# weibohuang0314/pixel_aware_gyro_aided_klt_feature_tracker

Hardware: AMD Instinct MI355X
Metric: tracked features/sec (21x21, 3-lvl, 30 iter) (higher is better)
Workload: dtype f32 sampling, f64 normal equations; 1 GPU; cfg1_euroc_752x480: 752x480 pair, 1000 keypoints (1000/GPU), gyro-predicted affine init, h=10, L=3, I=30 (synthetic stand-in for BASELINE configs[1]); mode=shard-weak, features_total=1000, features_active=1000, step_mode=graph

## Files before the change

### include/pagk.h

```cpp
#ifndef PAGK_H
#define PAGK_H

#include <stddef.h>
#include <stdint.h>

#ifdef __cplusplus
extern "C" {
#endif

#define PAGK_VERSION 303

#define PAGK_MAX_PYRAMIDS 8
#define PAGK_MAX_HALF_PATCH 15

enum {
    PAGK_OK = 0,
    PAGK_E_ARG = -1,
    PAGK_E_HIP = -2,
    PAGK_E_NOMEM = -3,
    PAGK_E_UNSUPPORTED = -4,
    PAGK_E_NODEVICE = -5,
    PAGK_E_NCCL = -6,
    PAGK_E_CAPACITY = -7
};
// ... 10 lines not shown
    int32_t iterations;
    int32_t pyramids;
    uint8_t has_gyro_predict_initial;
    uint8_t inverse;
    uint8_t consider_illumination;
    uint8_t consider_affine;
    uint8_t regularization_penalty;
    uint8_t calculate_ncc;
    uint8_t predict_method;
    uint8_t solver_variant;
    float lambda;
    float alpha;
    int32_t max_distance;
    float inv_log_max_dist;
    float fx, fy, cx, cy;
    float dist_coef[5];
    int32_t n_dist_coef;
} pagk_params;

typedef struct pagk_outputs {
    float *pt_un;
    float *pt_dist;
    uint8_t *status;
    double *pix_err;
    double *dist_pred;
    float *ncc;
    int32_t *iters;
} pagk_outputs;

typedef struct pagk_ctx pagk_ctx;

int pagk_version(void);
const char *pagk_strerror(int code);
const char *pagk_last_error(const pagk_ctx *ctx);

void pagk_params_default(pagk_params *p);
float pagk_inv_log_max_dist(float alpha, int32_t max_distance);

int pagk_create(pagk_ctx **out, int device);
void pagk_destroy(pagk_ctx *ctx);

int pagk_track(pagk_ctx *ctx, const pagk_params *params, const pagk_image *ref,
               const pagk_image *cur, int32_t n, const float *pt_ref_un,
               const float *pt_init_un, const float *affine, const uint8_t *status_in,
               const pagk_outputs *out);

int pagk_track_pyr(pagk_ctx *ctx, const pagk_params *params, int32_t n_levels,
                   const pagk_image *ref_levels, const pagk_image *cur_levels, int32_t n,
                   const float *pt_ref_un, const float *pt_init_un, const float *affine,
                   const uint8_t *status_in, const pagk_outputs *out);

int pagk_frame_upload(pagk_ctx *ctx, int32_t slot, const pagk_image *img, int32_t pyramids);
int pagk_frame_upload_pinned(pagk_ctx *ctx, int32_t slot, const pagk_image *img, int32_t pyramids);
int pagk_frame_set_device(pagk_ctx *ctx, int32_t slot, const void *d_data, int32_t width,
                          int32_t height, int64_t step, int32_t pyramids);
int pagk_frame_set_device_batch(pagk_ctx *const *ctxs, int32_t k, const int32_t *slot, const void *const *d_data,
                                const int32_t *width, const int32_t *height, const int64_t *step, int32_t pyramids);
int pagk_frame_download_level(pagk_ctx *ctx, int32_t slot, int32_t level, uint8_t *dst,
                              int32_t *width, int32_t *height);

int pagk_track_device(pagk_ctx *ctx, const pagk_params *params, int32_t slot_ref,
                      int32_t slot_cur, int32_t n, const float *d_pt_ref_un,
                      const float *d_pt_init_un, const float *d_affine,
                      const uint8_t *d_status_in, const pagk_outputs *d_out);
int pagk_track_device_fused(pagk_ctx *ctx, const pagk_params *params, int32_t slot_ref, int32_t slot_cur, int32_t n,
                            const float *d_pt_ref_un, const float *d_pt_init_un, const float *d_affine,
                            const uint8_t *d_status_in, const pagk_outputs *d_out, int32_t slot_next,
                            const void *d_next, int32_t width, int32_t height, int64_t step, int32_t pyramids);
int pagk_track_device_batch(pagk_ctx *const *ctxs, int32_t k, const pagk_params *params, const int32_t *slot_ref,
                            const int32_t *slot_cur, const int32_t *n, const float *const *d_pt_ref_un,
                            const float *const *d_pt_init_un, const float *const *d_affine,
                            const uint8_t *const *d_status_in, const pagk_outputs *d_out);
int pagk_sync(pagk_ctx *ctx);
int pagk_check_launch(pagk_ctx *ctx);
int pagk_set_stream(pagk_ctx *ctx, void *hip_stream);

int pagk_set_kernel(pagk_ctx *ctx, int32_t which);
int pagk_has_variant(int32_t which);
int pagk_last_variant(const pagk_ctx *ctx);

int pagk_last_handover(pagk_ctx *ctx);

int pagk_priority_threshold(pagk_ctx *ctx);

int pagk_set_concurrency(pagk_ctx *ctx, int32_t streams);

int pagk_last_kernel_ms(pagk_ctx *ctx, float *track_ms, float *pyramid_ms);

int pagk_gyro_predict_device(pagk_ctx *ctx, const pagk_params *params, int32_t width, int32_t height,
                             const float *KRKinv, const float *r3, int32_t n, const float *d_pt_ref_un,
                             float *d_pt_predict_un, float *d_pt_predict, uint8_t *d_status, float *d_affine);
int pagk_gyro_predict_device_rot(pagk_ctx *ctx, const pagk_params *params, int32_t width, int32_t height,
                                 const float *d_rot, int32_t n, const float *d_pt_ref_un, float *d_pt_predict_un,
                                 float *d_pt_predict, uint8_t *d_status, float *d_affine);

int pagk_post_filter(int32_t n, int32_t half_patch, const uint8_t *status_pm,
                     const double *pix_err, const double *dist_pred, const float *pt_pm,
                     const float *pt_pm_un, uint8_t *status_out, float *pt_predict,
                     float *pt_predict_un);
int pagk_post_filter_device(pagk_ctx *ctx, int32_t n, int32_t half_patch, const uint8_t *d_status_pm,
                            const double *d_pix_err, const double *d_dist_pred, const float *d_pt_pm,
                            const float *d_pt_pm_un, uint8_t *d_status_out, float *d_pt_predict,
                            float *d_pt_predict_un, int32_t *d_kept, double *d_thresholds );

int pagk_gyro_predict_device_live(pagk_ctx *ctx, const pagk_params *params, int32_t width, int32_t height,
                                  const float *d_rot, int32_t n, const float *d_pt_ref_un, const uint8_t *d_live,
                                  float *d_pt_predict_un, float *d_pt_predict, uint8_t *d_status, float *d_affine);

#define PAGK_HANDOVER_STATE_WORDS 8
int pagk_frame_handover_device(pagk_ctx *ctx, const pagk_params *params, int32_t width, int32_t height, int32_t cap,
                               int32_t target_n, double new_point_threshold, const uint8_t *d_status,
                               const float *d_pt_predict, const float *d_pt_predict_un, int32_t cand_cap,
                               const int32_t *d_n_cand, const float *d_cand_un, float *d_keys, float *d_keys_un,
                               float *d_keys_normal , int32_t *d_index_in_last, uint8_t *d_live,
                               uint8_t *d_mask , int32_t *d_state);
int pagk_frame_handover(pagk_ctx *ctx, const pagk_params *params, int32_t width, int32_t height, int32_t cap,
                        int32_t target_n, double new_point_threshold, const uint8_t *status, const float *pt_predict,
                        const float *pt_predict_un, int32_t cand_cap, const int32_t *n_cand, const float *cand_un,
                        float *keys, float *keys_un, float *keys_normal, int32_t *index_in_last, uint8_t *live,
                        uint8_t *mask, int32_t *state);

typedef struct pagk_detect_params {
    double quality_level;
    double min_distance;
    double harris_k;
    int32_t raw_cap;
} pagk_detect_params;
#define PAGK_DETECT_INFO_WORDS 8
void pagk_detect_params_default(pagk_detect_params *p);
int pagk_detect_corners_device(pagk_ctx *ctx, const pagk_detect_params *det, int32_t slot, const uint8_t *d_mask,
                               int32_t cap, const int32_t *d_max_corners, float *d_corners, int32_t *d_info);
int pagk_detect_corners(pagk_ctx *ctx, const pagk_detect_params *det, const pagk_image *img, const uint8_t *mask,
                        int32_t max_corners, float *corners, int32_t *info);
int pagk_frame_handover_detect_device(pagk_ctx *ctx, const pagk_params *params, int32_t width, int32_t height,
                                      int32_t cap, int32_t target_n, double new_point_threshold, const uint8_t *d_status,
                                      const float *d_pt_predict, const float *d_pt_predict_un,
                                      const pagk_detect_params *det, int32_t slot, float *d_keys, float *d_keys_un,
                                      float *d_keys_normal , int32_t *d_index_in_last, uint8_t *d_live,
                                      uint8_t *d_mask , int32_t *d_state, int32_t *d_info);
int pagk_frame_handover_detect(pagk_ctx *ctx, const pagk_params *params, int32_t width, int32_t height, int32_t cap,
                               int32_t target_n, double new_point_threshold, const uint8_t *status,
                               const float *pt_predict, const float *pt_predict_un, const pagk_detect_params *det,
                               const pagk_image *img, float *keys, float *keys_un, float *keys_normal,
                               int32_t *index_in_last, uint8_t *live, uint8_t *mask, int32_t *state, int32_t *info);
int pagk_selftest_corner_response(pagk_ctx *ctx, const pagk_image *img, float *R);

typedef struct pagk_fast_params {
    int32_t ini_threshold;
    int32_t min_threshold;
    int32_t n_features;
    int32_t n_levels;
} pagk_fast_params;
void pagk_fast_params_default(pagk_fast_params *p);
int pagk_fast_params_check(const pagk_fast_params *p);
int pagk_detect_fast_bounds(int32_t width, int32_t height, int32_t n_features, int32_t *raw_bound, int32_t *out_bound);
int pagk_detect_fast_device(pagk_ctx *ctx, const pagk_fast_params *params, int32_t slot, const uint8_t *d_mask, int32_t cap,
                            float *d_keypoints, float *d_response , int32_t *d_info);
int pagk_detect_fast(pagk_ctx *ctx, const pagk_fast_params *params, const pagk_image *img, const uint8_t *mask, int32_t cap,
                     float *keypoints, float *response, int32_t *info);
int pagk_frame_handover_fast_device(pagk_ctx *ctx, const pagk_params *params, int32_t width, int32_t height, int32_t cap,
                                    int32_t target_n, double new_point_threshold, const uint8_t *d_status,
                                    const float *d_pt_predict, const float *d_pt_predict_un, const pagk_fast_params *fast,
                                    int32_t slot, float *d_keys, float *d_keys_un, float *d_keys_normal ,
                                    int32_t *d_index_in_last, uint8_t *d_live, uint8_t *d_mask ,
                                    int32_t *d_state, int32_t *d_info);
int pagk_frame_handover_fast(pagk_ctx *ctx, const pagk_params *params, int32_t width, int32_t height, int32_t cap,
// ... 228 lines not shown
```

### pixel_aware_gyro_aided_klt_feature_tracker_amd/capi.py

```python
from __future__ import annotations

import ctypes as C
import os

import numpy as np

PKG_DIR = os.path.dirname(os.path.abspath(__file__))
LIB_PATH = os.environ.get("PAGK_LIB") or os.path.join(PKG_DIR, "libpagk_hip.so")

PAGK_OK = 0
PAGK_E_ARG = -1
PAGK_E_HIP = -2
PAGK_E_NOMEM = -3
PAGK_E_UNSUPPORTED = -4
PAGK_E_NODEVICE = -5
PAGK_E_NCCL = -6
PAGK_E_CAPACITY = -7


class Image(C.Structure):
    _fields_ = [("data", C.c_void_p), ("width", C.c_int32), ("height", C.c_int32), ("step", C.c_int64)]


class Params(C.Structure):
# ... 288 lines not shown
        lib.pagk_lk_params_check.argtypes = [_P(LkParams)]
        lib.pagk_lk_levels.restype = C.c_int
        lib.pagk_lk_levels.argtypes = [i32, i32, _P(LkParams)]
        lib.pagk_lk_pyramid_device.restype = C.c_int
        lib.pagk_lk_pyramid_device.argtypes = [vp, _P(LkParams), i32]
        lib.pagk_lk_track_device.restype = C.c_int
        lib.pagk_lk_track_device.argtypes = [vp, _P(LkParams), i32, i32, i32, vp, vp, vp, vp, vp, vp, vp, vp]
        lib.pagk_lk_track.restype = C.c_int
        lib.pagk_lk_track.argtypes = [vp, _P(LkParams), _P(Image), _P(Image), i32, vp, vp, vp, vp, vp, vp, vp]
        lib.pagk_selftest_lk_level.restype = C.c_int
        lib.pagk_selftest_lk_level.argtypes = [vp, i32, i32, vp, C.c_int64]
    f32 = C.c_float
    for name in ("pagk_graph_begin",):
        getattr(lib, name).restype = C.c_int
        getattr(lib, name).argtypes = [vp]
    lib.pagk_graph_end.restype = C.c_int
    lib.pagk_graph_end.argtypes = [vp, _P(i32)]
    lib.pagk_graph_launch.restype = C.c_int
    lib.pagk_graph_launch.argtypes = [vp, i32]
    lib.pagk_graph_destroy.restype = C.c_int
    lib.pagk_graph_destroy.argtypes = [vp, i32]
    lib.pagk_geometry_scores_device.restype = C.c_int
    lib.pagk_geometry_scores_device.argtypes = [vp, vp, vp, vp, i32, vp, vp, f32, vp, vp, vp]
    lib.pagk_geometry_scores.restype = C.c_int
    lib.pagk_geometry_scores.argtypes = [vp, vp, vp, vp, i32, vp, vp, f32, vp, vp, _P(f32), _P(f32)]
    lib.pagk_geometry_select.restype = C.c_int
    lib.pagk_geometry_select.argtypes = [f32, f32]
    lib.pagk_geometry_validation.restype = C.c_int
    lib.pagk_geometry_validation.argtypes = [vp, vp, vp, vp, i32, vp, vp, vp, f32, _P(f32)]
    if hasattr(lib, "pagk_search_klt_device"):
        ap, lp, f32_ = _P(AssocParams), _P(LkParams), C.c_float
        lib.pagk_assoc_params_default.restype = None
        lib.pagk_assoc_params_default.argtypes = [ap]
        lib.pagk_assoc_params_check.restype = C.c_int
        lib.pagk_assoc_params_check.argtypes = [ap]
        lib.pagk_match_features_device.restype = C.c_int
        lib.pagk_match_features_device.argtypes = [vp, ap, i32, i32, i32] + [vp] * 10
        lib.pagk_search_gyro_predict_device.restype = C.c_int
        lib.pagk_search_gyro_predict_device.argtypes = ([vp, ap, i32, i32, i32, i32, vp, vp, vp, vp, i32, vp, vp, vp, f32_, i32]
                                                        + [vp] * 11)
        lib.pagk_search_gyro_predict.restype = C.c_int
        lib.pagk_search_gyro_predict.argtypes = ([vp, ap, _P(Image), _P(Image), i32, i32, vp, vp, vp, vp, i32, vp, vp, f32_, i32]
                                                 + [vp] * 10)
        lib.pagk_search_klt_device.restype = C.c_int
        lib.pagk_search_klt_device.argtypes = [vp, lp, ap, i32, i32, i32, vp, vp, i32, vp, vp] + [vp] * 11
        lib.pagk_search_klt.restype = C.c_int
        lib.pagk_search_klt.argtypes = [vp, lp, ap, _P(Image), _P(Image), i32, vp, i32, vp] + [vp] * 10
    lib.pagk_fit_params_default.restype = None
    lib.pagk_fit_params_default.argtypes = [_P(FitParams)]
    lib.pagk_geometry_fit_device.restype = C.c_int
    lib.pagk_geometry_fit_device.argtypes = [vp, _P(FitParams), i32, vp, vp, vp, vp, vp, vp, vp, vp]
    lib.pagk_geometry_fit.restype = C.c_int
    lib.pagk_geometry_fit.argtypes = [vp, _P(FitParams), i32, vp, vp, vp, vp, vp, vp, vp, vp]
    lib.pagk_geometry_validation_device.restype = C.c_int
    lib.pagk_geometry_validation_device.argtypes = [vp, _P(FitParams), i32, vp, vp, vp, f32, vp, vp]
    lib.pagk_geometry_validation_fit.restype = C.c_int
    lib.pagk_geometry_validation_fit.argtypes = [vp, _P(FitParams), i32, vp, vp, vp, f32, _P(f32)]
    lib.pagk_selftest_fit_samples.restype = C.c_int
    lib.pagk_selftest_fit_samples.argtypes = [vp, C.c_uint64, i32, i32, i32, i32, vp]
    f64 = C.c_double
    lib.pagk_pose_params_default.restype = None
    lib.pagk_pose_params_default.argtypes = [_P(PoseParams)]
    lib.pagk_pose_params_check.restype = C.c_int
    lib.pagk_pose_params_check.argtypes = [_P(PoseParams)]
    lib.pagk_pose_2d2d_device.restype = C.c_int
    lib.pagk_pose_2d2d_device.argtypes = [vp, _P(PoseParams), f64, f64, f64, i32] + [vp] * 12
    lib.pagk_pose_from_matches_device.restype = C.c_int
    lib.pagk_pose_from_matches_device.argtypes = [vp, _P(PoseParams), f64, f64, f64, i32, vp, vp, i32] + [vp] * 12
    lib.pagk_pose_2d2d.restype = C.c_int
    lib.pagk_pose_2d2d.argtypes = [vp, _P(PoseParams), f64, f64, f64, i32] + [vp] * 12
    lib.pagk_near_neighbors_device.restype = C.c_int
    lib.pagk_near_neighbors_device.argtypes = [vp, i32, i32, i32, i32, vp, vp, vp, vp, i32, vp, vp, i32, f32, i32, i32,
                                               vp, vp, vp, vp]
    lib.pagk_find_near_neighbors.restype = C.c_int
    lib.pagk_find_near_neighbors.argtypes = [vp, _P(Image), _P(Image), i32, i32, vp, vp, vp, vp, i32, vp, vp, i32, f32,
                                             i32, i32, vp, vp, vp, vp]
    lib.pagk_ncc_free.restype = C.c_int
    lib.pagk_ncc_free.argtypes = [vp, _P(Image), _P(Image), i32, i32, vp, vp, vp, vp]
    if hasattr(lib, "pagk_selftest_divide"):
        lib.pagk_selftest_divide.restype = C.c_int
        lib.pagk_selftest_divide.argtypes = [vp, i32, vp, vp, vp, vp, vp, vp]
        lib.pagk_selftest_solve.restype = C.c_int
        lib.pagk_selftest_solve.argtypes = [vp, i32, vp, vp, C.c_uint32, vp, vp, vp, vp]
    if hasattr(lib, "pagk_priority_threshold"):
        lib.pagk_priority_threshold.restype = C.c_int
        lib.pagk_priority_threshold.argtypes = [vp]
    if hasattr(lib, "pagk_check_launch"):
        lib.pagk_check_launch.restype = C.c_int
        lib.pagk_check_launch.argtypes = [vp]
    if hasattr(lib, "pagk_selftest_repeat_sum"):
        lib.pagk_selftest_repeat_sum.restype = C.c_int
        lib.pagk_selftest_repeat_sum.argtypes = [vp, i32, vp, i32, vp, vp]
    if hasattr(lib, "pagk_selftest_sample"):
        lib.pagk_selftest_sample.restype = C.c_int
        lib.pagk_selftest_sample.argtypes = [vp, i32, i32, i32, i32, vp, vp]
    lib.pagk_match_features.restype = C.c_int
    lib.pagk_match_features.argtypes = [i32, i32, vp, vp, vp, vp, i32, vp, vp, vp, vp]
    lib.pagk_multi_create.restype = C.c_int
    lib.pagk_multi_create.argtypes = [_P(vp), _P(i32), i32]
    lib.pagk_multi_unique_id.restype = C.c_int
    lib.pagk_multi_unique_id.argtypes = [vp]
    lib.pagk_multi_create_rank.restype = C.c_int
    lib.pagk_multi_create_rank.argtypes = [_P(vp), vp, i32, i32, i32]
    lib.pagk_multi_destroy.restype = None
    lib.pagk_multi_destroy.argtypes = [vp]
    lib.pagk_multi_world.restype = i32
    lib.pagk_multi_world.argtypes = [vp]
    if hasattr(lib, "pagk_multi_comm_count"):
        lib.pagk_multi_comm_count.restype = i32
        lib.pagk_multi_comm_count.argtypes = [vp]
    lib.pagk_multi_local.restype = i32
    lib.pagk_multi_local.argtypes = [vp]
    lib.pagk_multi_ctx.restype = vp
    lib.pagk_multi_ctx.argtypes = [vp, i32]
    lib.pagk_multi_last_error.restype = C.c_char_p
    lib.pagk_multi_last_error.argtypes = [vp]
    lib.pagk_shard_range.restype = None
    lib.pagk_shard_range.argtypes = [i32, i32, i32, _P(i32), _P(i32)]
    lib.pagk_shard_layout.restype = C.c_size_t
    lib.pagk_shard_layout.argtypes = [i32, _P(C.c_size_t)]
    lib.pagk_multi_allgather.restype = C.c_int
    lib.pagk_multi_allgather.argtypes = [vp, _P(vp), _P(vp), C.c_size_t, _P(vp)]
    lib.pagk_track_sharded.restype = C.c_int
    lib.pagk_track_sharded.argtypes = [vp, _P(Params), _P(Image), _P(Image), i32, vp, vp, vp, vp, _P(Outputs)]


EXPORTED_SYMBOLS = [
    "pagk_version", "pagk_strerror", "pagk_last_error", "pagk_params_default", "pagk_inv_log_max_dist",
    "pagk_create", "pagk_destroy", "pagk_track", "pagk_track_pyr", "pagk_frame_upload", "pagk_frame_upload_pinned",
    "pagk_frame_set_device", "pagk_frame_download_level", "pagk_track_device", "pagk_track_device_fused", "pagk_sync",
    "pagk_set_stream", "pagk_set_kernel", "pagk_last_variant", "pagk_set_concurrency", "pagk_last_handover", "pagk_last_kernel_ms", "pagk_post_filter", "pagk_gyro_predict_device",
    "pagk_gyro_predict_device_rot",
    "pagk_geometry_scores_device", "pagk_geometry_scores", "pagk_geometry_select", "pagk_geometry_validation",
    "pagk_graph_begin", "pagk_graph_end", "pagk_graph_launch", "pagk_graph_destroy",
    "pagk_near_neighbors_device", "pagk_find_near_neighbors", "pagk_ncc_free", "pagk_match_features",
    "pagk_multi_create", "pagk_multi_unique_id", "pagk_multi_create_rank", "pagk_multi_destroy", "pagk_multi_world",
    "pagk_multi_local", "pagk_multi_ctx", "pagk_multi_last_error", "pagk_shard_range", "pagk_shard_layout",
    "pagk_multi_allgather", "pagk_track_sharded", "pagk_selftest_divide", "pagk_selftest_solve",
    "pagk_selftest_repeat_sum", "pagk_check_launch", "pagk_track_device_batch", "pagk_frame_set_device_batch", "pagk_priority_threshold",
    "pagk_multi_comm_count", "pagk_has_variant",
    "pagk_fit_params_default", "pagk_geometry_fit_device", "pagk_geometry_fit", "pagk_geometry_validation_device",
    "pagk_geometry_validation_fit", "pagk_selftest_fit_samples",
    "pagk_pose_params_default", "pagk_pose_params_check", "pagk_pose_2d2d_device", "pagk_pose_from_matches_device",
    "pagk_pose_2d2d",
    "pagk_post_filter_device", "pagk_gyro_predict_device_live", "pagk_frame_handover_device", "pagk_frame_handover",
    "pagk_detect_params_default", "pagk_detect_corners_device", "pagk_detect_corners",
    "pagk_frame_handover_detect_device", "pagk_frame_handover_detect", "pagk_selftest_corner_response",
    "pagk_fast_params_default", "pagk_fast_params_check", "pagk_detect_fast_bounds", "pagk_detect_fast_device",
    "pagk_detect_fast", "pagk_frame_handover_fast_device", "pagk_frame_handover_fast", "pagk_selftest_fast_cells",
    "pagk_rectify_params_default", "pagk_rectify_params_check", "pagk_rectify_set_maps", "pagk_frame_rectify_device",
    "pagk_frame_rectify_pinned", "pagk_rectify", "pagk_undistort_maps",
    "pagk_orb_params_default", "pagk_orb_params_check", "pagk_orb_pattern_check", "pagk_orb_set_pattern",
    "pagk_orb_describe_device", "pagk_orb_describe", "pagk_orb_match_device", "pagk_orb_match",
    "pagk_selftest_sample",
    "pagk_lk_params_default", "pagk_lk_params_check", "pagk_lk_levels", "pagk_lk_pyramid_device", "pagk_lk_track_device",
    "pagk_lk_track", "pagk_selftest_lk_level",
    "pagk_assoc_params_default", "pagk_assoc_params_check", "pagk_match_features_device", "pagk_search_gyro_predict_device",
    "pagk_search_gyro_predict", "pagk_search_klt_device", "pagk_search_klt",
]

HANDOVER_STATE_WORDS = 8
HANDOVER_STATE_FIELDS = ("total", "reach_flag", "survivors", "added", "rejected")


def fit_params_default(**overrides) -> FitParams:
    p = FitParams()
    load().pagk_fit_params_default(C.byref(p))
    for k, v in overrides.items():
        if k not in dict(FitParams._fields_):
            raise TypeError(f"pagk_fit_params has no field {k}")
        setattr(p, k, v)
    return p


def pose_params_default(**overrides) -> PoseParams:
    p = PoseParams()
    load().pagk_pose_params_default(C.byref(p))
    for k, v in overrides.items():
        if k not in dict(PoseParams._fields_):
            raise TypeError(f"pagk_pose_params has no field {k}")
        setattr(p, k, v)
    return p


def pose_params_check(p: PoseParams) -> int:
    return load().pagk_pose_params_check(C.byref(p))


def detect_params_default(**overrides) -> DetectParams:
    p = DetectParams()
    load().pagk_detect_params_default(C.byref(p))
    for k, v in overrides.items():
        if k not in dict(DetectParams._fields_):
            raise TypeError(f"pagk_detect_params has no field {k}")
        setattr(p, k, v)
    return p


def fast_params_default(**overrides) -> FastParams:
    p = FastParams()
    load().pagk_fast_params_default(C.byref(p))
    for k, v in overrides.items():
        if k not in dict(FastParams._fields_):
            raise TypeError(f"pagk_fast_params has no field {k}")
        setattr(p, k, v)
    return p


def fast_params_check(p: FastParams) -> int:
    return int(load().pagk_fast_params_check(C.byref(p)))


def detect_fast_bounds(width: int, height: int, n_features: int):
    raw, out = C.c_int32(0), C.c_int32(0)
    rc = load().pagk_detect_fast_bounds(int(width), int(height), int(n_features), C.byref(raw), C.byref(out))
    if rc != 0:
        raise PagkError(rc, "pagk_detect_fast_bounds")
    return raw.value, out.value


def orb_params_default(**overrides) -> OrbParams:
    p = OrbParams()
    load().pagk_orb_params_default(C.byref(p))
# ... 787 lines not shown
        info = np.zeros(ASSOC_INFO_WORDS, np.int32)
        ru = float(2 * half_patch) if radius_unit is None else float(radius_unit)
        rc = self.lib.pagk_search_gyro_predict(self.h, C.byref(ap), C.byref(ir), C.byref(ic), half_patch, n, _ptr(keys_ref),
                                               _ptr(pt_predict_un), _ptr(status), _ptr(affine), m, _ptr(keys_cur),
                                               _ptr(keys_cur_un), ru, cap, _ptr(count), _ptr(idx), _ptr(dist), _ptr(ncc),
                                               _ptr(q), _ptr(t), _ptr(md), _ptr(mc), _ptr(flows), _ptr(info))
        if rc < 0 and rc != PAGK_E_CAPACITY:
            self._check(rc, "pagk_search_gyro_predict")
        k = int(info[4])
        out = dict(rc=rc, n_matches=k, query=q[:k], train=t[:k], dist=md[:k], ncc=mc[:k], flows_err=flows[:n], count=count[:n],
                   idx=idx[:n], dist_lists=dist[:n], ncc_lists=ncc[:n], info=info)
        out.update(zip(ASSOC_MATCH_INFO_FIELDS, (int(v) for v in info[:6])))
        return out

    def search_klt_device(self, lk: LkParams, ap: AssocParams, slot_ref: int, slot_cur: int, cap: int, d_keys_ref, d_n, m: int,
                          d_keys_cur, d_m, d_pt_out, d_status, d_err, d_match_query, d_match_train, d_match_dist, d_disparity,
                          d_n_matches, d_stats, d_info, d_lk_info):
        self._check(self.lib.pagk_search_klt_device(
            self.h, C.byref(lk), C.byref(ap), slot_ref, slot_cur, cap, _ptr(d_keys_ref), _ptr(d_n), m, _ptr(d_keys_cur), _ptr(d_m),
            _ptr(d_pt_out), _ptr(d_status), _ptr(d_err), _ptr(d_match_query), _ptr(d_match_train), _ptr(d_match_dist),
            _ptr(d_disparity), _ptr(d_n_matches), _ptr(d_stats), _ptr(d_info), _ptr(d_lk_info)), "pagk_search_klt_device")

    def search_klt(self, img_ref, img_cur, keys_ref, keys_cur, lk: LkParams | None = None, ap: AssocParams | None = None) -> dict:
        lk = lk if lk is not None else lk_params_default()
        ap = ap if ap is not None else assoc_params_default()
        kr = np.ascontiguousarray(keys_ref, np.float32).reshape(-1, 2)
        kc = np.ascontiguousarray(keys_cur, np.float32).reshape(-1, 2)
        n, m = int(kr.shape[0]), int(kc.shape[0])
        nn = max(n, 1)
        ir, ic = image_view(img_ref), image_view(img_cur)
        pt_out, status, err = np.zeros((nn, 2), np.float32), np.zeros(nn, np.uint8), np.zeros(nn, np.float32)
        q, t = np.full(nn, -1, np.int32), np.full(nn, -1, np.int32)
        md, disp = np.zeros(nn, np.float32), np.zeros(nn, np.float64)
        stats = np.zeros(ASSOC_STATS_WORDS, np.float64)
        info, lk_info = np.zeros(ASSOC_INFO_WORDS, np.int32), np.zeros(LK_INFO_WORDS, np.int32)
        k = self.lib.pagk_search_klt(self.h, C.byref(lk), C.byref(ap), C.byref(ir), C.byref(ic), n, _ptr(kr) if n else None, m,
                                     _ptr(kc) if m else None, _ptr(pt_out), _ptr(status), _ptr(err), _ptr(q), _ptr(t), _ptr(md),
                                     _ptr(disp), _ptr(stats), _ptr(info), _ptr(lk_info))
        self._check(min(k, 0), "pagk_search_klt")
        out = dict(n_matches=k, query=q[:k], train=t[:k], dist=md[:k], disparity=disp[:k], pt_out=pt_out[:n], status=status[:n],
                   err=err[:n], stats=stats, info=info, lk_info=lk_info)
        out.update(zip(ASSOC_KLT_INFO_FIELDS, (int(v) for v in info)))
        out.update(zip(ASSOC_STATS_FIELDS, (float(v) for v in stats[:7])))
        return out

    def graph_begin(self):
        self._check(self.lib.pagk_graph_begin(self.h), "pagk_graph_begin")

    def graph_end(self) -> int:
        gid = C.c_int32(-1)
        self._check(self.lib.pagk_graph_end(self.h, C.byref(gid)), "pagk_graph_end")
        return gid.value

    def graph_launch(self, graph_id: int):
        self._check(self.lib.pagk_graph_launch(self.h, graph_id), "pagk_graph_launch")

    def graph_destroy(self, graph_id: int):
        self._check(self.lib.pagk_graph_destroy(self.h, graph_id), "pagk_graph_destroy")

    def sync(self):
        self._check(self.lib.pagk_sync(self.h), "pagk_sync")

    def check_launch(self):
        self._check(self.lib.pagk_check_launch(self.h), "pagk_check_launch")

    def set_stream(self, stream_ptr: int | None):
        self._check(self.lib.pagk_set_stream(self.h, stream_ptr), "pagk_set_stream")

    def set_kernel(self, which: int):
        self._check(self.lib.pagk_set_kernel(self.h, which), "pagk_set_kernel")

    VARIANT_NAMES = {0: "4-wave workgroup per feature, DPP row chains", 1: "one thread per feature (cross-check)",
                     2: "2-wave workgroup per feature, f64 MFMA chain", 3: "one wave per feature, f64 MFMA chain",
                     4: "relaxed order (experiment)", 5: "four features per wave, f64 MFMA blocks",
                     6: "four independent rows per wave + work queue",
                     7: "four features per wave, one pyramid level per wave"}

    def priority_threshold(self) -> int:
        rc = int(self.lib.pagk_priority_threshold(self.h))
        if rc < 0:
            self._check(rc, "pagk_priority_threshold")
        return rc

    def last_variant(self) -> int:
        return int(self.lib.pagk_last_variant(self.h))

    def last_handover(self) -> int:
        rc = int(self.lib.pagk_last_handover(self.h))
        if rc < 0:
            self._check(rc, "pagk_last_handover")
        return rc

    def set_concurrency(self, streams: int):
        self._check(self.lib.pagk_set_concurrency(self.h, streams), "pagk_set_concurrency")

    def last_kernel_ms(self):
        t, p = C.c_float(0), C.c_float(0)
        self._check(self.lib.pagk_last_kernel_ms(self.h, C.byref(t), C.byref(p)), "pagk_last_kernel_ms")
        return t.value, p.value


def post_filter(half_patch: int, status_pm, pix_err, dist_pred, pt_pm, pt_pm_un):
    lib = load()
    n = int(status_pm.shape[0])
    status = np.zeros(max(n, 1), np.uint8)
    pp = np.zeros((max(n, 1), 2), np.float32)
    ppu = np.zeros((max(n, 1), 2), np.float32)
    rc = lib.pagk_post_filter(n, half_patch, _ptr(status_pm), _ptr(pix_err), _ptr(dist_pred), _ptr(pt_pm),
                              _ptr(pt_pm_un), _ptr(status), _ptr(pp), _ptr(ppu))
    if rc < 0:
        raise PagkError(rc, "pagk_post_filter")
    return rc, status[:n], pp[:n], ppu[:n]


def geometry_select(score_H: float, score_F: float) -> bool:
    return bool(load().pagk_geometry_select(float(score_H), float(score_F)))


def match_features(count, idx, dist, ncc, use_ncc=True):
    n = int(count.shape[0])
    cap = int(idx.shape[1])
    q, t = np.zeros(max(n, 1), np.int32), np.zeros(max(n, 1), np.int32)
    d, c = np.zeros(max(n, 1), np.float32), np.zeros(max(n, 1), np.float32)
    count = np.ascontiguousarray(count, np.int32)
    idx, dist, ncc = np.ascontiguousarray(idx), np.ascontiguousarray(dist), np.ascontiguousarray(ncc)
    k = load().pagk_match_features(n, cap, _ptr(count), _ptr(idx), _ptr(dist), _ptr(ncc), int(use_ncc), _ptr(q), _ptr(t),
                                   _ptr(d), _ptr(c))
    if k < 0:
        raise PagkError(k, "pagk_match_features")
    return q[:k], t[:k], d[:k], c[:k]


def shard_range(n: int, rank: int, world: int) -> tuple[int, int]:
    lo, hi = C.c_int32(0), C.c_int32(0)
    load().pagk_shard_range(n, rank, world, C.byref(lo), C.byref(hi))
    return lo.value, hi.value


def shard_layout(m: int) -> tuple[list[int], int]:
    offs = (C.c_size_t * 7)()
    total = load().pagk_shard_layout(m, offs)
    return [int(v) for v in offs], int(total)


class Multi:

    def __init__(self, devices=None, *, uid: bytes | None = None, rank: int = 0, world: int = 1, device: int = 0):
        self.lib = load()
        self._lent = []
        h = C.c_void_p()
        if uid is None:
            if devices is None or len(devices) == 0 or any(int(d) < 0 for d in devices):
                raise ValueError("Multi(devices=[...]) needs a non-empty list of device indices (or uid=, rank=, world=)")
            devs = (C.c_int32 * len(devices))(*devices)
            rc = self.lib.pagk_multi_create(C.byref(h), devs, len(devices))
            where = "pagk_multi_create"
        else:
            if len(uid) != 128:
                raise ValueError("the RCCL unique id is 128 bytes")
            buf = (C.c_uint8 * 128).from_buffer_copy(uid)
            rc = self.lib.pagk_multi_create_rank(C.byref(h), buf, rank, world, device)
            where = "pagk_multi_create_rank"
        if rc != PAGK_OK:
            raise PagkError(rc, where)
        self.h = h
        self.world = self.lib.pagk_multi_world(h)
# ... 60 lines not shown
```

### pixel_aware_gyro_aided_klt_feature_tracker_amd/csrc/pagk_device.h

```cpp
#pragma once
#include <hip/hip_runtime.h>
#include <stdint.h>

namespace pagk {

constexpr int kMaxLevels = 8;

struct DevLevel {
    const uint32_t *quad;
    int cols, rows;
    float fcols, frows;
    float fcols_m1, frows_m1;
};

__device__ __forceinline__ int ld_agent(const int *p) { return __hip_atomic_load(p, __ATOMIC_RELAXED, __HIP_MEMORY_SCOPE_AGENT); }
__device__ __forceinline__ void st_agent(int *p, int v) { __hip_atomic_store(p, v, __ATOMIC_RELAXED, __HIP_MEMORY_SCOPE_AGENT); }

struct SuspState {
    int level;
    int iter;
    float dx, dy, dg, db, lastCost;
    int iters;
};

struct BatchStream {
    DevLevel l1[kMaxLevels], l2[kMaxLevels];
    const float *pt_ref, *pt_init, *affine;
    const uint8_t *status_in;
    float *pt_un, *pt_dist;
    uint8_t *status;
    double *pix_err, *dist_pred;
    float *ncc;
    int *iters;
    int n;
    int quad_base;
};

struct TrackArgs {
    DevLevel l1[kMaxLevels], l2[kMaxLevels];
    float scales[kMaxLevels];
    int n_levels;
    int n;
    const float *pt_ref;
    const float *pt_init;
    const float *affine;
    const uint8_t *status_in;
    float *pt_un;
    float *pt_dist;
    uint8_t *status;
    double *pix_err;
    double *dist_pred;
    float *ncc;
    int *iters;
    unsigned long long *dbg;
    float *ws;
    int iter_budget;
    int *susp_count;
    int *susp_list;
    SuspState *susp_state;
    int susp_lone;
    int susp_waves;
    int susp_polls;
    int *queue;
    int *lv_ready;
    float *lv_state;
    int *lv_error;
    int lv_shift;
    int lv_polls;
    const BatchStream *batch;
    int batch_k;
    int half, iterations;
    int prio_k;
    unsigned long long *prio_stats;
    const int *prio_kbuf;
    int has_gyro, illum, use_affine, penalty, calc_ncc;
    uint32_t solver;
    float lam_invlog;
    float lam_invlog_alpha;
    float alpha;
    double win_size_inv;
    int distort_on;
    float fx, fy, cx, cy, fx_inv, fy_inv, k1, k2, p1, p2, k3;
};

__device__ __forceinline__ DevLevel pin_level(const DevLevel &src) { return src; }

struct Coord {
    int i;
    float f;
    float omf;
};

template <bool CLAMP>
__device__ __forceinline__ Coord prep_coord(float x, float fmax, float fmax_m1)
{
    if (CLAMP) {
        x = fmaxf(x, 0.0f);
        x = (x >= fmax) ? fmax_m1 : x;
    }
    Coord c;
    c.i = (int)x;
    c.f = __builtin_amdgcn_fractf(x);
    c.omf = 1.0f - c.f;
    return c;
}

__device__ __forceinline__ float bilerp(uint32_t q, const Coord &cx, const Coord &cy)
{
    float d0 = (float)(q & 0xffu);
    float d1 = (float)((q >> 8) & 0xffu);
    float d2 = (float)((q >> 16) & 0xffu);
    float d3 = (float)(q >> 24);
    float top = cx.omf * d0 + cx.f * d1;
    float bot = cx.omf * d2 + cx.f * d3;
    return cy.omf * top + cy.f * bot;
}

#if !defined(PAGK_CLASSIC_SAMPLER)
#ifndef PAGK_PK_BILERP
#define PAGK_PK_BILERP
#endif
#ifndef PAGK_TYPED_TAPS
#define PAGK_TYPED_TAPS
#endif
#endif
typedef float pagk_f32x4 __attribute__((ext_vector_type(4)));
typedef float pagk_f32x2 __attribute__((ext_vector_type(2)));
typedef int pagk_i32x4 __attribute__((ext_vector_type(4)));

#ifdef PAGK_TYPED_TAPS
__device__ pagk_f32x4 pagk_buffer_load_format_xyzw(pagk_i32x4 rsrc, int vindex, int voffset, int soffset, int aux)
    __asm("llvm.amdgcn.struct.buffer.load.format.v4f32");

struct TapSrc {
    pagk_i32x4 rs;
};
__device__ __forceinline__ TapSrc tap_src(const DevLevel &L)
{
    const uint64_t base = (uint64_t)(uintptr_t)L.quad;
    TapSrc t;
    t.rs.x = (int)(uint32_t)base;
    t.rs.y = (int)((uint32_t)(base >> 32) & 0xffffu) | (4 << 16);
    t.rs.z = L.cols * L.rows;
    t.rs.w = 4 | (6 << 3) | (5 << 6) | (7 << 9) | (2 << 12) | (10 << 15);
    return t;
}
typedef pagk_f32x4 Taps;
__device__ __forceinline__ Taps load_taps(const TapSrc &t, int idx) { return pagk_buffer_load_format_xyzw(t.rs, idx, 0, 0, 0); }
__device__ __forceinline__ pagk_f32x4 taps_f32(Taps q) { return q; }
#else
struct TapSrc {
    const uint32_t *quad;
};
__device__ __forceinline__ TapSrc tap_src(const DevLevel &L) { return TapSrc{L.quad}; }
typedef uint32_t Taps;
__device__ __forceinline__ Taps load_taps(const TapSrc &t, int idx) { return t.quad[(uint32_t)idx]; }
__device__ __forceinline__ pagk_f32x4 taps_f32(Taps q)
// ... 607 lines not shown
```

### pixel_aware_gyro_aided_klt_feature_tracker_amd/csrc/pagk_handover_kernel.h

```cpp
#pragma once

#include <hip/hip_runtime.h>
#include <stdint.h>

namespace pagk {

constexpr int kHandoverStateWords = 8;
constexpr int kHandoverHalf = 7;

constexpr int kPfRound = 2048;

__device__ __forceinline__ double pf_chain256(double s, const double2 *b)
{
    double2 A[8], B[8];
#pragma unroll
    for (int j = 0; j < 8; j++) A[j] = b[j];
    for (int k = 0; k < 128; k += 16) {
#pragma unroll
        for (int j = 0; j < 8; j++) B[j] = b[k + 8 + j];
        __builtin_amdgcn_sched_barrier(0);
#pragma unroll
        for (int j = 0; j < 8; j++) {
            s = s + A[j].x;
            s = s + A[j].y;
// ... 10 lines not shown
        __builtin_amdgcn_sched_barrier(0);
    }
    return s;
}

__global__ void __launch_bounds__(1024) k_post_filter(int32_t n, int32_t half_patch, const uint8_t *status_pm,
                                                      const double *pix_err, const double *dist_pred, const float *pt_pm,
                                                      const float *pt_pm_un, uint8_t *status_out, float *pt_predict,
                                                      float *pt_predict_un, int32_t *kept_out, double *thresholds)
{
    __shared__ double s_sum;
    __shared__ __align__(16) double s_stage[2][kPfRound];
    __shared__ int32_t s_cnt[16], s_kept[16];
    const int tid = threadIdx.x, lane = tid & 63, wave = tid >> 6;
    int32_t cnt = 0;
    double s = 0.0;
    auto load = [&](int i, int32_t &c) -> double {
        if (i >= n) return 0.0;
        const double v = pix_err[i];
        const bool on = status_pm[i] != 0;
        c += on ? 1 : 0;
        return on ? v : 0.0;
    };
    double v0 = load(tid, cnt), v1 = load(1024 + tid, cnt);
    s_stage[0][tid] = v0, s_stage[0][1024 + tid] = v1;
    __syncthreads();
    for (int r0 = 0, g = 0; r0 < n; r0 += kPfRound, g ^= 1) {
        v0 = load(r0 + kPfRound + tid, cnt), v1 = load(r0 + kPfRound + 1024 + tid, cnt);
        if (wave == 0) {
            const int left = n - r0;
            const int groups = left >= kPfRound ? kPfRound / 256 : (left + 255) / 256;
            for (int q = 0; q < groups; q++) s = pf_chain256(s, reinterpret_cast<const double2 *>(&s_stage[g][q * 256]));
        }
        s_stage[g ^ 1][tid] = v0, s_stage[g ^ 1][1024 + tid] = v1;
        __syncthreads();
    }
    if (tid == 0) s_sum = s;
    for (int off = 32; off >= 1; off >>= 1) cnt += __shfl_down(cnt, off, 64);
    if (lane == 0) s_cnt[wave] = cnt;
    __syncthreads();
    int32_t total = 0;
    for (int w = 0; w < 16; w++) total += s_cnt[w];
    const double avg = s_sum / (double)total;
    const double th_pix = 4.0 * avg > (double)half_patch ? 4.0 * avg : (double)half_patch;
    const double th_dist = (double)half_patch * 4.0;
    int32_t kept = 0;
    for (int c0 = 0; c0 < n; c0 += 1024) {
        const int i = c0 + tid;
        if (i < n) {
            const bool ok = status_pm[i] && pix_err[i] < th_pix && dist_pred[i] < th_dist;
            status_out[i] = ok ? 1 : 0;
            if (ok) {
                if (pt_predict && pt_pm) pt_predict[2 * i] = pt_pm[2 * i], pt_predict[2 * i + 1] = pt_pm[2 * i + 1];
                if (pt_predict_un && pt_pm_un)
                    pt_predict_un[2 * i] = pt_pm_un[2 * i], pt_predict_un[2 * i + 1] = pt_pm_un[2 * i + 1];
                kept++;
            }
        }
    }
    for (int off = 32; off >= 1; off >>= 1) kept += __shfl_down(kept, off, 64);
    if (lane == 0) s_kept[wave] = kept;
    __syncthreads();
    if (tid == 0) {
        int32_t k = 0;
        for (int w = 0; w < 16; w++) k += s_kept[w];
        *kept_out = k;
        if (thresholds) thresholds[0] = th_pix, thresholds[1] = th_dist;
    }
}

struct HandoverArgs {
    int32_t cap, cand_cap, width, height, target_n;
    double new_point_threshold;
    float fx, fy, cx, cy, fx_inv, fy_inv, k1, k2, p1, p2, k3;
    int32_t distort_on;
    const uint8_t *status;
    const float *pt_predict, *pt_predict_un;
    const int32_t *n_cand;
    const float *cand_un;
    float *keys, *keys_un, *keys_normal;
    int32_t *index_in_last;
    uint8_t *live, *mask;
    int32_t *state;
};

__global__ void __launch_bounds__(256) k_handover_fill(uint8_t *mask, int64_t bytes)
{
    const int64_t t = (int64_t)blockIdx.x * 256 + threadIdx.x, o = t * 16;
    if (o + 16 <= bytes) {
        if ((reinterpret_cast<uintptr_t>(mask) & 15) == 0) {
            *reinterpret_cast<uint4 *>(mask + o) = make_uint4(0x01010101u, 0x01010101u, 0x01010101u, 0x01010101u);
        } else {
            for (int k = 0; k < 16; k++) mask[o + k] = 1;
        }
    } else {
        for (int64_t k = o; k < bytes; k++) mask[k] = 1;
    }
}

__device__ __forceinline__ int handover_hole_origin(float x, int extent)
{
    const int a = (int)x - kHandoverHalf;
    const int b = a > 0 ? a : 0;
    const int hi = extent - 2 * kHandoverHalf;
    return b < hi ? b : hi;
}

__global__ void __launch_bounds__(256) k_handover_holes(int32_t cap, int32_t width, int32_t height, const uint8_t *status,
                                                        const float *pt_predict_un, uint8_t *mask)
{
    const int t = blockIdx.x * 256 + threadIdx.x;
    const int i = t / (2 * kHandoverHalf), r = t - i * (2 * kHandoverHalf);
    if (i >= cap || !status[i]) return;
    const int x0 = handover_hole_origin(pt_predict_un[2 * i], width);
    const int y0 = handover_hole_origin(pt_predict_un[2 * i + 1], height);
    uint8_t *row = mask + (int64_t)(y0 + r) * width + x0;
    for (int k = 0; k < 2 * kHandoverHalf; k++) row[k] = 0;
}

__device__ __forceinline__ int32_t handover_scan(bool take, int32_t *wtot, int lane, int wave, int32_t &tot)
{
    const unsigned long long bal = __ballot(take);
    if (lane == 0) wtot[wave] = __popcll(bal);
    __syncthreads();
    int32_t off = 0;
    tot = 0;
    for (int w = 0; w < 16; w++) {
        off += w < wave ? wtot[w] : 0;
        tot += wtot[w];
    }
    __syncthreads();
    return off + __popcll(bal & ((1ull << lane) - 1ull));
}

__device__ __forceinline__ bool handover_accepts(const HandoverArgs &a, float x, float y)
{
    if (!(x > -1.0f && x < (float)a.width && y > -1.0f && y < (float)a.height)) return false;
    return a.mask[(int64_t)(int)y * a.width + (int)x] != 0;
}

__global__ void __launch_bounds__(1024) k_handover_keys(HandoverArgs a)
{
    __shared__ int32_t wtot[16];
    const int tid = threadIdx.x, lane = tid & 63, wave = tid >> 6;
    int32_t m = 0;
    for (int c0 = 0; c0 < a.cap; c0 += 1024) {
        const int i = c0 + tid;
        const bool take = i < a.cap && a.status[i] != 0;
        int32_t tot;
        const int32_t o = m + handover_scan(take, wtot, lane, wave, tot);
        if (take) {
            const float xu = a.pt_predict_un[2 * i], yu = a.pt_predict_un[2 * i + 1];
            a.keys[2 * o] = a.pt_predict[2 * i], a.keys[2 * o + 1] = a.pt_predict[2 * i + 1];
            a.keys_un[2 * o] = xu, a.keys_un[2 * o + 1] = yu;
            if (a.keys_normal) a.keys_normal[2 * o] = (xu - a.cx) * a.fx_inv, a.keys_normal[2 * o + 1] = (yu - a.cy) * a.fy_inv;
            a.index_in_last[o] = i;
        }
        m += tot;
    }
    const int32_t reach = a.state[1];
    int32_t n_cand = *a.n_cand;
    n_cand = n_cand < 0 ? 0 : (n_cand > a.cand_cap ? a.cand_cap : n_cand);
    __syncthreads();
    const int32_t n_new = a.target_n - m;
    const bool topup = ((double)m < a.new_point_threshold || !reach) && n_new > 0;
    int32_t seen = 0;
    for (int c0 = 0; c0 < n_cand; c0 += 1024) {
        const int j = c0 + tid;
        float x = 0.0f, y = 0.0f;
        if (j < n_cand) x = a.cand_un[2 * j], y = a.cand_un[2 * j + 1];
        const bool ok = j < n_cand && handover_accepts(a, x, y);
        int32_t tot;
        const int32_t r = seen + handover_scan(ok, wtot, lane, wave, tot);
        if (topup && ok && r < n_new) {
            const int32_t q = m + r;
            a.keys_un[2 * q] = x, a.keys_un[2 * q + 1] = y;
            const float xn = (x - a.cx) * a.fx_inv, yn = (y - a.cy) * a.fy_inv;
            if (a.keys_normal) a.keys_normal[2 * q] = xn, a.keys_normal[2 * q + 1] = yn;
            float ox = x, oy = y;
            if (a.distort_on) {
                const float r2 = xn * xn + yn * yn;
                const float r4 = r2 * r2;
                const float r6 = r4 * r2;
                const float xd = xn * (1 + a.k1 * r2 + a.k2 * r4 + a.k3 * r6) + 2 * a.p1 * xn * yn + a.p2 * (r2 + 2 * xn * xn);
                const float yd = yn * (1 + a.k1 * r2 + a.k2 * r4 + a.k3 * r6) + a.p1 * (r2 + 2 * yn * yn) + 2 * a.p2 * xn * yn;
                ox = a.fx * xd + a.cx;
                oy = a.fy * yd + a.cy;
            }
            a.keys[2 * q] = ox, a.keys[2 * q + 1] = oy;
            a.index_in_last[q] = -1;
        }
        seen += tot;
    }
    const int32_t added = topup ? (seen < n_new ? seen : n_new) : 0;
    const int32_t total = m + added;
    for (int i = tid; i < a.cap; i += 1024) {
        a.live[i] = i < total ? 1 : 0;
        if (i >= total) {
            a.keys[2 * i] = a.keys[2 * i + 1] = 0.0f;
            a.keys_un[2 * i] = a.keys_un[2 * i + 1] = 0.0f;
            if (a.keys_normal) a.keys_normal[2 * i] = a.keys_normal[2 * i + 1] = 0.0f;
            a.index_in_last[i] = -1;
        }
    }
    if (tid == 0) {
        a.state[0] = total;
        a.state[1] = topup ? (total == a.target_n ? 1 : 0) : reach;
        a.state[2] = m;
        a.state[3] = added;
        a.state[4] = n_cand - seen;
        a.state[5] = a.state[6] = a.state[7] = 0;
    }
}

}
```

### pixel_aware_gyro_aided_klt_feature_tracker_amd/csrc/pagk_hip.hip

```cpp
#include <hip/hip_runtime.h>

#include <algorithm>
#include <array>
#include <cmath>
#include <cstdio>
#include <cstdlib>
#include <cstring>
#include <new>
#include <utility>
#include <vector>

#include "../../include/pagk.h"
#include "pagk_kernels.h"
#include "pagk_associate_kernel.h"
#include "pagk_pose_kernel.h"
#include "pagk_layout.h"
#include "pagk_select.h"

using namespace pagk;

namespace {

constexpr int kSlots = 6;
constexpr int kUserSlots = 4;

struct DevBuf {
    void *ptr = nullptr;
    size_t bytes = 0;
    void *host = nullptr;
    bool mirrored = false;
};

struct FrameSlot {
    int w = 0, h = 0, L = 0;
    int wrap0 = 1;
    int pad0 = 0;
    uint8_t *u8[kMaxLevels] = {};
    uint32_t *quad[kMaxLevels] = {};
    const uint8_t *img0 = nullptr;
    int64_t pitch0 = 0;
    DevBuf block;
    bool valid = false;
};

}

struct pagk_ctx {
    int device = 0;
    hipStream_t own_stream = nullptr;
    hipStream_t stream = nullptr;
    FrameSlot slots[kSlots];
    enum Buf {
        FEAT,
        SCORE,
        FIT,
        FITIO,
        HAND,
        HANDIO,
        DET,
        FAST,
        RECT_ENTRIES,
        RECT_STAGE,
        ORB_PATTERN,
        ORB_BLUR,
        ORB_KEYS,
        LK_PYR,
        LK_PYR_LAST = LK_PYR + kSlots - 1,
        ASSOC,
        POSE,
        POSEIO,
        QUAD_WS,
        SUSP,
        LV,
        kBufs
    };
    DevBuf buf[kBufs];
    int fit_n = 0, fit_iters = 0;
    int pose_n = 0, pose_iters = 0;
    int rect_w = 0, rect_h = 0, rect_wp = 0;
    bool orb_pattern_set = false;
    struct LkPyr { int w = 0, h = 0, top = -1; } lk_pyr[kSlots];
    void *queue = nullptr;
    int quad_capacity[PAGK_MAX_HALF_PATCH + 1] = {};
    int rows_capacity[PAGK_MAX_HALF_PATCH + 1] = {};
    int rows_waves_cap = 0;
    int *susp_count_dev = nullptr;
    struct BatchDesc {
        void *host = nullptr, *dev = nullptr;
        hipEvent_t used = nullptr;
        bool recorded = false;
    };
    static constexpr int kBatchRing = 6, kBatchPerCapture = 4, kBatchMaxStreams = 64;
    BatchDesc batch_ring[kBatchRing];
    int batch_turn = 0;
    bool batch_seen = false;
    std::vector<BatchDesc> cap_batch;
    int cap_batch_used = 0;
    hipEvent_t ev_batch = nullptr;
    int *lv_error = nullptr;
    int *lv_error_dev = nullptr;
    hipStream_t aux_stream = nullptr;
    hipEvent_t ev_fork = nullptr, ev_join = nullptr;
    int susp_lone = 1;
    int finisher_wgs = 16;
    int finisher_polls = 20000;
    int level_polls = 300000;
    int quad_budget = -1;
    int cus = 0;
    bool capturing = false;
    static constexpr int kGraphs = 8;
    hipGraph_t graphs[kGraphs] = {};
    hipGraphExec_t graph_execs[kGraphs] = {};
    struct GraphSeg {
        enum Kind { GRAPH, FINISHER, JOIN } kind = GRAPH;
        hipGraph_t g = nullptr;
        hipGraphExec_t ex = nullptr;
        const void *fn = nullptr;
        TrackArgs args;
        int grid = 0;
        size_t lds = 0;
    };
    std::vector<GraphSeg> pre_segs[kGraphs];
    std::vector<BatchDesc> graph_batch[kGraphs];
    std::vector<GraphSeg> cap_segs;
    hipEvent_t ev_trk[2] = {}, ev_pyr[2] = {};
    bool trk_timed = false, pyr_timed = false;
    int kernel = 0;
    bool last_handover = false;
    int concurrency = 1;
    int last_variant = -1;
    int mfma_min_features = 0x7fffffff;
    int wave_min_features = 6000;
    int quad_min_features = 7000;
    int block5_min_features = 2500;
    int prio_k = 4;
    unsigned long long *prio_stats = nullptr;
    bool block5_window = true;
    int levels_min_features = 6000;
    int levels_shift = 0;
    bool levels_shared = false;
    bool unfused_pyramid = false;
    char err[256] = {0};
};

namespace {

#define HIPCHK(ctx, call)                                                                              \
    do {                                                                                               \
        hipError_t e_ = (call);                                                                        \
        if (e_ != hipSuccess) {                                                                        \
            snprintf((ctx)->err, sizeof((ctx)->err), "%s:%d %s -> %s", __FILE__, __LINE__, #call,     \
                     hipGetErrorString(e_));                                                           \
            return e_ == hipErrorOutOfMemory ? PAGK_E_NOMEM : PAGK_E_HIP;                              \
        }                                                                                              \
    } while (0)

#define NOT_WHILE_CAPTURING(ctx, what)                                                                 \
    do {                                                                                               \
        if ((ctx)->capturing) {                                                                        \
            snprintf((ctx)->err, sizeof((ctx)->err), "%s is not capturable: use the *_device entry points between pagk_graph_begin and pagk_graph_end", what); \
            return PAGK_E_ARG;                                                                         \
        }                                                                                              \
    } while (0)

int level_dims(int w, int h, int L, int *lw, int *lh)
{
    lw[0] = w;
    lh[0] = h;
    for (int l = 1; l < L; l++) {
        lw[l] = (int)(lw[l - 1] * 0.5);
        lh[l] = (int)(lh[l - 1] * 0.5);
        if (lw[l] < 1 || lh[l] < 1) return PAGK_E_ARG;
    }
    return PAGK_OK;
}

bool in_capture(pagk_ctx *ctx)
{
    if (ctx->capturing) return true;
    hipStreamCaptureStatus st = hipStreamCaptureStatusNone;
    return hipStreamIsCapturing(ctx->stream, &st) != hipSuccess || st != hipStreamCaptureStatusNone;
}

int no_live_graphs(pagk_ctx *ctx, const char *what, const char *hint)
{
    for (int k = 0; k < pagk_ctx::kGraphs; k++)
        if (ctx->graph_execs[k]) {
            snprintf(ctx->err, sizeof(ctx->err), "%s would have to grow while graph %d of this context is alive (its nodes hold the old "
                     "pointers): destroy the graph first, or %s", what, k, hint);
            return PAGK_E_ARG;
        }
    return PAGK_OK;
}

enum GrowPolicy {
    GROW_FREELY = 0,
    NOT_IN_CAPTURE = 1,
    NOT_UNDER_GRAPH = 2,
    NOT_IN_CAPTURE_NOR_UNDER_GRAPH = NOT_IN_CAPTURE | NOT_UNDER_GRAPH,
};

int release(pagk_ctx *ctx, DevBuf &b)
{
    if (b.ptr) HIPCHK(ctx, hipFree(b.ptr));
    if (b.host) HIPCHK(ctx, hipHostFree(b.host));
    b.ptr = b.host = nullptr;
    b.bytes = 0;
    return PAGK_OK;
}

int reserve(pagk_ctx *ctx, DevBuf &b, size_t bytes, GrowPolicy policy, const char *what, const char *hint = "")
{
    if (bytes <= b.bytes) return PAGK_OK;
    if ((policy & NOT_IN_CAPTURE) && in_capture(ctx)) {
        snprintf(ctx->err, sizeof(ctx->err), "%s would have to grow inside a graph capture: %s", what, hint);
        return PAGK_E_ARG;
    }
    int rc = (policy & NOT_UNDER_GRAPH) ? no_live_graphs(ctx, what, hint) : PAGK_OK;
    if (rc || (rc = release(ctx, b))) return rc;
// ... 479 lines not shown
            a.susp_list = reinterpret_cast<int *>(lb + lvl.susp_list);
            a.susp_state = reinterpret_cast<SuspState *>(lb + lvl.susp_state);
        } else {
            const size_t sizes[3] = {kSuspCountBytes, (size_t)n * 4, (size_t)n * sizeof(SuspState)};
            const Layout<3> lay(sizes);
            DevBuf &susp = ctx->buf[pagk_ctx::SUSP];
            if (int gr = reserve(ctx, susp, lay.total, NOT_IN_CAPTURE_NOR_UNDER_GRAPH, "the continuation buffers",
                                 kLargestLaunchFirst)) return gr;
            a.susp_count = lay.at<int>(susp.ptr, 0);
            a.susp_list = lay.at<int>(susp.ptr, 1);
            a.susp_state = lay.at<SuspState>(susp.ptr, 2);
        }
        a.iter_budget = budget;
        a.susp_waves = nq;
        a.susp_lone = ctx->susp_lone;
        ctx->susp_count_dev = a.susp_count;
    }
    if (use_levels)
        HIPCHK(ctx, hipMemsetAsync(lb, 0, handover ? lvl.susp_list + (size_t)n * 4 : lvl.susp_count, ctx->stream));
    else if (handover)
        HIPCHK(ctx, hipMemsetAsync(a.susp_count, 0, kSuspCountBytes + (size_t)n * 4, ctx->stream));
    const bool live = handover && live_ok && ctx->finisher_wgs > 0 && ctx->aux_stream;
    const bool segmented = live && ctx->capturing && !getenv("PAGK_GRAPH_BRANCH");
    int fin_seg = -1;
    if (segmented) {
        if (int sr = capture_split(ctx)) return sr;
        ctx->cap_segs.emplace_back();
        ctx->cap_segs.back().kind = pagk_ctx::GraphSeg::FINISHER;
        fin_seg = (int)ctx->cap_segs.size() - 1;
    } else if (live) {
        HIPCHK(ctx, hipEventRecord(ctx->ev_fork, ctx->stream));
        HIPCHK(ctx, hipStreamWaitEvent(ctx->aux_stream, ctx->ev_fork, 0));
    }
    HIPCHK(ctx, launch(use_levels ? k.levels[lean] : k.quad[lean], waves, 64, 0, ctx->stream, a));
    TrackArgs af = a;
#ifdef PAGK_STAMPS
    if (af.dbg) af.dbg += (size_t)16 * (waves - nq);
#endif
    const size_t lds = track_block_lds_bytes(a.half);
    if (live) {
        if (segmented) {
            pagk_ctx::GraphSeg &fs = ctx->cap_segs[(size_t)fin_seg];
            fs.fn = reinterpret_cast<const void *>(k.resume_live[lean]);
            fs.args = af;
            fs.grid = ctx->finisher_wgs;
            fs.lds = lds;
            if (int sr = capture_split(ctx)) return sr;
            ctx->cap_segs.emplace_back();
            ctx->cap_segs.back().kind = pagk_ctx::GraphSeg::JOIN;
        } else {
            HIPCHK(ctx, launch(k.resume_live[lean], ctx->finisher_wgs, kBlock, lds, ctx->aux_stream, af));
            HIPCHK(ctx, hipEventRecord(ctx->ev_join, ctx->aux_stream));
            HIPCHK(ctx, hipStreamWaitEvent(ctx->stream, ctx->ev_join, 0));
        }
    }
    if (handover) HIPCHK(ctx, launch(k.resume[lean], live ? 64 : (n < 1024 ? n : 1024), kBlock, lds, ctx->stream, af));
    return PAGK_OK;
}

int launch_block(pagk_ctx *ctx, const TrackKernels &k, bool lean, int n, const TrackArgs &a, const PyrArgs *pyr,
                 int pyr_blocks, bool *pyr_done)
{
    const size_t lds = track_block_lds_bytes(a.half);
    if (pyr && pyr_blocks > 0 && k.block_pyr[lean] && lds <= 48 * 1024) {
        hipLaunchKernelGGL(k.block_pyr[lean], dim3(n + pyr_blocks), dim3(kBlock), lds, ctx->stream, a, *pyr);
        HIPCHK(ctx, hipGetLastError());
        if (pyr_done) *pyr_done = true;
        return PAGK_OK;
    }
    const bool five = lean && k.block5 && select_block5(n, ctx->block5_min_features, ctx->block5_window, ctx->cus);
    const TrackFn kern = five ? k.block5 : k.block[lean];
    if (lds > 48 * 1024) {
        static thread_local bool configured[PAGK_MAX_HALF_PATCH + 1][2][16] = {};
        bool &done = configured[a.half][lean][ctx->device & 15];
        if (!done) {
            HIPCHK(ctx, hipFuncSetAttribute(reinterpret_cast<const void *>(kern), hipFuncAttributeMaxDynamicSharedMemorySize, (int)lds));
            done = true;
        }
    }
    HIPCHK(ctx, launch(kern, n, kBlock, lds, ctx->stream, a));
    return PAGK_OK;
}

int launch_track(pagk_ctx *ctx, const pagk_params *p, const FrameSlot &sr, const FrameSlot &sc, int n,
                 const float *d_pt_ref, const float *d_pt_init, const float *d_affine, const uint8_t *d_status,
                 const pagk_outputs *o, const PyrArgs *pyr = nullptr, int pyr_blocks = 0, bool *pyr_done = nullptr)
{
    if (pyr_done) *pyr_done = false;
    TrackArgs a;
    memset(&a, 0, sizeof a);
    a.n_levels = p->pyramids;
    for (int l = 0; l < p->pyramids; l++) {
        fill_level(a.l1[l], sr, l);
        fill_level(a.l2[l], sc, l);
        a.scales[l] = l == 0 ? 1.0f : (float)((double)a.scales[l - 1] * 0.5);
    }
    a.n = n;
    a.pt_ref = d_pt_ref;
    a.pt_init = d_pt_init;
    a.affine = d_affine;
    a.status_in = d_status;
    a.pt_un = o->pt_un;
    a.pt_dist = o->pt_dist;
    a.status = o->status;
    a.pix_err = o->pix_err;
    a.dist_pred = o->dist_pred;
    a.ncc = o->ncc;
    a.iters = o->iters;
#if defined(PAGK_STAMPS) || defined(PAGK_COUNT_REDO) || defined(PAGK_TIC)
    a.dbg = reinterpret_cast<unsigned long long *>(getenv("PAGK_DBG_PTR") ? strtoull(getenv("PAGK_DBG_PTR"), nullptr, 0) : 0ull);
#endif
    fill_param_args(a, p);
    a.prio_k = ctx->prio_k;
    a.prio_stats = ctx->prio_stats;
    a.prio_kbuf = ctx->prio_stats ? reinterpret_cast<const int *>(ctx->prio_stats + 2) : nullptr;
    a.lv_error = ctx->lv_error_dev;

    if (ctx->ev_trk[0] && !in_capture(ctx)) HIPCHK(ctx, hipEventRecord(ctx->ev_trk[0], ctx->stream));
    if (n > 0) {
        ctx->last_handover = false;
        const bool lean = !a.penalty && a.solver == 0;
        const TrackKernels &k = track_kernels_of(a.half);
        const int variant = ctx->last_variant = select_variant(select_in(ctx, p, n));
        int rc = PAGK_OK;
        hipError_t e = hipSuccess;
        switch (variant) {
            case 1: e = launch(k_track_thread, (n + 63) / 64, 64, 0, ctx->stream, a); break;
            case 2: e = launch(k.mfma[lean], n, 128, track_mfma_lds_bytes(a.half), ctx->stream, a); break;
            case 3: e = launch(k.wave[lean], n, 64, track_wave_lds_bytes(a.half), ctx->stream, a); break;
            case 4: e = launch(k.relaxed, n, kBlock, track_block_lds_bytes(a.half), ctx->stream, a); break;
            case 5:
            case 7: rc = launch_quad(ctx, p, k, lean, variant == 7, n, a); break;
            case 6: rc = launch_rows(ctx, k, n, a); break;
            default: rc = launch_block(ctx, k, lean, n, a, pyr, pyr_blocks, pyr_done); break;
        }
        if (rc) return rc;
        HIPCHK(ctx, e);
        HIPCHK(ctx, hipGetLastError());
    }
    if (ctx->ev_trk[1] && !in_capture(ctx)) HIPCHK(ctx, hipEventRecord(ctx->ev_trk[1], ctx->stream));
    if (!in_capture(ctx)) ctx->trk_timed = true;
    return PAGK_OK;
}

struct FeatPtrs {
    float *pt_ref, *pt_init, *affine;
    uint8_t *status_in;
    pagk_outputs out;
    Layout<11> lay;
    size_t in_bytes;
};

int feat_reserve(pagk_ctx *ctx, int n, FeatPtrs *fp)
{
    int cap = n < 1 ? 1 : n;
    size_t sizes[11] = {8, 8, 16, 1, 8, 8, 1, 8, 8, 4, 4};
    for (size_t &sz : sizes) sz *= (size_t)cap;
    const Layout<11> lay(sizes);
    int rc = reserve(ctx, ctx->buf[pagk_ctx::FEAT], lay.total, GROW_FREELY, "the feature arrays");
    if (rc) return rc;
    void *b = ctx->buf[pagk_ctx::FEAT].ptr;
    fp->lay = lay;
    fp->in_bytes = lay.off[4];
    fp->pt_ref = lay.at<float>(b, 0);
    fp->pt_init = lay.at<float>(b, 1);
    fp->affine = lay.at<float>(b, 2);
    fp->status_in = lay.at<uint8_t>(b, 3);
    fp->out = {lay.at<float>(b, 4), lay.at<float>(b, 5), lay.at<uint8_t>(b, 6), lay.at<double>(b, 7),
               lay.at<double>(b, 8), lay.at<float>(b, 9), lay.at<int32_t>(b, 10)};
    return PAGK_OK;
}

int upload_level0(pagk_ctx *ctx, FrameSlot &s, const pagk_image *img)
{
    HIPCHK(ctx, hipMemcpy2DAsync(s.u8[0], (size_t)s.w, img->data, (size_t)img->step, (size_t)s.w, (size_t)s.h,
                                 hipMemcpyHostToDevice, ctx->stream));
    return PAGK_OK;
}

int check_image(const pagk_image *im)
{
    if (!im || !im->data || im->width < 1 || im->height < 1 || im->step < im->width) return PAGK_E_ARG;
    if (im->width >= (1 << 24) || im->height >= (1 << 24) || (int64_t)im->width * im->height >= (1ll << 31)) return PAGK_E_ARG;
    return PAGK_OK;
}

int track_host_common(pagk_ctx *ctx, const pagk_params *p, int n, const float *pt_ref, const float *pt_init,
                      const float *affine, const uint8_t *status_in, const pagk_outputs *out, FrameSlot &sr,
                      FrameSlot &sc)
{
    if (n < 0 || !out || !out->pt_un || !out->status) return PAGK_E_ARG;
    if (n > 0 && (!pt_ref || !status_in)) return PAGK_E_ARG;
    if (n > 0 && p->has_gyro_predict_initial && !pt_init) return PAGK_E_ARG;
    if (n > 0 && p->consider_affine && !affine) return PAGK_E_ARG;
    FeatPtrs fp;
    int rc = feat_reserve(ctx, n, &fp);
    if (rc) return rc;
    const size_t *offs = fp.lay.off;
    uint8_t *hb = static_cast<uint8_t *>(ctx->buf[pagk_ctx::FEAT].host), *db = static_cast<uint8_t *>(ctx->buf[pagk_ctx::FEAT].ptr);
    if (n > 0) {
        size_t nn = (size_t)n;
        memcpy(hb + offs[0], pt_ref, nn * 8);
        if (pt_init) memcpy(hb + offs[1], pt_init, nn * 8);
        if (affine) memcpy(hb + offs[2], affine, nn * 16);
        memcpy(hb + offs[3], status_in, nn);
        HIPCHK(ctx, hipMemcpyAsync(db, hb, fp.in_bytes, hipMemcpyHostToDevice, ctx->stream));
    }
    pagk_outputs dout = fp.out;
    if (!out->pt_dist) dout.pt_dist = nullptr;
    if (!out->pix_err) dout.pix_err = nullptr;
    if (!out->dist_pred) dout.dist_pred = nullptr;
    if (!out->ncc) dout.ncc = nullptr;
    if (!out->iters) dout.iters = nullptr;
    rc = launch_track(ctx, p, sr, sc, n, fp.pt_ref, pt_init ? fp.pt_init : nullptr, affine ? fp.affine : nullptr,
                      fp.status_in, &dout);
    if (rc) return rc;
    if (n > 0)
        HIPCHK(ctx, hipMemcpyAsync(hb + fp.in_bytes, db + fp.in_bytes, fp.lay.total - fp.in_bytes, hipMemcpyDeviceToHost,
                                   ctx->stream));
    HIPCHK(ctx, hipStreamSynchronize(ctx->stream));
    if (int lr = lv_check(ctx)) return lr;
    if (n > 0) {
        size_t nn = (size_t)n;
        memcpy(out->pt_un, hb + offs[4], nn * 8);
        if (out->pt_dist) memcpy(out->pt_dist, hb + offs[5], nn * 8);
        memcpy(out->status, hb + offs[6], nn);
        if (out->pix_err) memcpy(out->pix_err, hb + offs[7], nn * 8);
        if (out->dist_pred) memcpy(out->dist_pred, hb + offs[8], nn * 8);
        if (out->ncc) memcpy(out->ncc, hb + offs[9], nn * 4);
        if (out->iters) memcpy(out->iters, hb + offs[10], nn * 4);
    }
    return PAGK_OK;
}

}

extern "C" {

int pagk_version(void) { return PAGK_VERSION; }

const char *pagk_strerror(int code)
{
    switch (code) {
        case PAGK_OK: return "ok";
        case PAGK_E_ARG: return "invalid argument";
        case PAGK_E_HIP: return "HIP runtime error";
        case PAGK_E_NOMEM: return "out of memory";
        case PAGK_E_UNSUPPORTED: return "unsupported mode";
        case PAGK_E_NODEVICE: return "no HIP device";
        case PAGK_E_NCCL: return "RCCL error";
        case PAGK_E_CAPACITY: return "output capacity too small";
        default: return "unknown error";
    }
}

const char *pagk_last_error(const pagk_ctx *ctx) { return ctx ? ctx->err : ""; }

void pagk_params_default(pagk_params *p)
{
    if (!p) return;
    memset(p, 0, sizeof *p);
    p->half_patch = 5;
    p->iterations = 10;
    p->pyramids = 3;
    p->has_gyro_predict_initial = 1;
    p->inverse = 0;
    p->consider_illumination = 1;
    p->consider_affine = 1;
    p->regularization_penalty = 0;
    p->calculate_ncc = 0;
    p->lambda = 1.0f;
    p->alpha = 0.5f;
    p->max_distance = 25;
    p->inv_log_max_dist = 0.0f;
    p->fx = p->fy = 1.0f;
    p->n_dist_coef = 4;
}

float pagk_inv_log_max_dist(float alpha, int32_t max_distance)
{
    float arg = alpha * (float)max_distance + 1;
    float lg = std::log(arg);
    return (float)(1.0 / (double)lg);
}

int pagk_create(pagk_ctx **out, int device)
{
    if (!out) return PAGK_E_ARG;
    *out = nullptr;
    int ndev = 0;
    if (hipGetDeviceCount(&ndev) != hipSuccess || ndev <= 0) return PAGK_E_NODEVICE;
    if (device < 0 || device >= ndev) return PAGK_E_ARG;
    pagk_ctx *ctx = new (std::nothrow) pagk_ctx();
    if (!ctx) return PAGK_E_NOMEM;
    ctx->device = device;
    if (hipSetDevice(device) != hipSuccess || hipStreamCreateWithFlags(&ctx->own_stream, hipStreamNonBlocking) != hipSuccess) {
        delete ctx;
        return PAGK_E_HIP;
    }
    ctx->stream = ctx->own_stream;
    ctx->buf[pagk_ctx::FEAT].mirrored = true;
    if (hipDeviceGetAttribute(&ctx->cus, hipDeviceAttributeMultiprocessorCount, device) != hipSuccess) ctx->cus = 0;
    if (hipMalloc(&ctx->queue, 256) != hipSuccess) {
        pagk_destroy(ctx);
        return PAGK_E_NOMEM;
    }
    {
        void *hp = nullptr;
        void *dp = nullptr;
        if (hipHostMalloc(&hp, 64, hipHostMallocMapped) == hipSuccess) {
            memset(hp, 0, 64);
            if (hipHostGetDevicePointer(&dp, hp, 0) == hipSuccess && dp) {
                ctx->lv_error = static_cast<int *>(hp);
                ctx->lv_error_dev = static_cast<int *>(dp);
            } else {
                (void)hipHostFree(hp);
            }
        }
    }
    if (ctx->cus > 0 && ctx->cus != 256) {
        auto scaled = [&](int v) { return v >= 0x7fffffff / 2 ? v : (int)((long long)v * ctx->cus / 256); };
        ctx->wave_min_features = scaled(ctx->wave_min_features);
        ctx->quad_min_features = scaled(ctx->quad_min_features);
        ctx->levels_min_features = scaled(ctx->levels_min_features);
        ctx->block5_min_features = scaled(ctx->block5_min_features);
    }
    ctx->unfused_pyramid = getenv("PAGK_UNFUSED_PYRAMID") != nullptr;
    if (getenv("PAGK_MFMA_MIN")) ctx->mfma_min_features = atoi(getenv("PAGK_MFMA_MIN"));
    if (getenv("PAGK_WAVE_MIN")) ctx->wave_min_features = atoi(getenv("PAGK_WAVE_MIN"));
    if (getenv("PAGK_QUAD_MIN")) ctx->quad_min_features = atoi(getenv("PAGK_QUAD_MIN"));
    if (getenv("PAGK_BLOCK5_MIN")) ctx->block5_min_features = atoi(getenv("PAGK_BLOCK5_MIN")), ctx->block5_window = false;
    if (getenv("PAGK_LEVELS_MIN")) ctx->levels_min_features = atoi(getenv("PAGK_LEVELS_MIN"));
    if (getenv("PAGK_PRIO_K") && strcmp(getenv("PAGK_PRIO_K"), "auto") == 0) {
        struct { unsigned long long st[2]; int k, pad; } seed = {{3500ull, 1000ull}, ctx->prio_k, 0};
        if (hipMalloc(reinterpret_cast<void **>(&ctx->prio_stats), sizeof seed) != hipSuccess ||
            hipMemcpy(ctx->prio_stats, &seed, sizeof seed, hipMemcpyHostToDevice) != hipSuccess) {
            if (ctx->prio_stats) (void)hipFree(ctx->prio_stats);
            ctx->prio_stats = nullptr;
            (void)hipGetLastError();
        }
    } else if (getenv("PAGK_PRIO_K")) {
        ctx->prio_k = atoi(getenv("PAGK_PRIO_K")) < 0 ? 0 : atoi(getenv("PAGK_PRIO_K"));
    }
    if (getenv("PAGK_LEVELS_XCD_SHIFT")) ctx->levels_shift = atoi(getenv("PAGK_LEVELS_XCD_SHIFT")) & 7;
    if (getenv("PAGK_LEVELS_SHARED")) ctx->levels_shared = atoi(getenv("PAGK_LEVELS_SHARED")) != 0;
    if (getenv("PAGK_QUAD_BUDGET")) ctx->quad_budget = atoi(getenv("PAGK_QUAD_BUDGET"));
    if (getenv("PAGK_ROWS_WAVES")) ctx->rows_waves_cap = atoi(getenv("PAGK_ROWS_WAVES"));
    if (getenv("PAGK_FINISHER_WGS")) ctx->finisher_wgs = atoi(getenv("PAGK_FINISHER_WGS"));
    if (getenv("PAGK_SUSPEND_LONE")) ctx->susp_lone = atoi(getenv("PAGK_SUSPEND_LONE"));
    if (getenv("PAGK_FINISHER_POLLS")) ctx->finisher_polls = atoi(getenv("PAGK_FINISHER_POLLS"));
    if (getenv("PAGK_LEVEL_POLLS")) ctx->level_polls = atoi(getenv("PAGK_LEVEL_POLLS"));
    if (hipStreamCreateWithFlags(&ctx->aux_stream, hipStreamNonBlocking) != hipSuccess ||
        hipEventCreateWithFlags(&ctx->ev_fork, hipEventDisableTiming) != hipSuccess ||
        hipEventCreateWithFlags(&ctx->ev_join, hipEventDisableTiming) != hipSuccess ||
        hipEventCreateWithFlags(&ctx->ev_batch, hipEventDisableTiming) != hipSuccess) {
        pagk_destroy(ctx);
        return PAGK_E_HIP;
    }
    for (int k = 0; k < 2; k++) {
        if (hipEventCreate(&ctx->ev_trk[k]) != hipSuccess || hipEventCreate(&ctx->ev_pyr[k]) != hipSuccess) {
            pagk_destroy(ctx);
            return PAGK_E_HIP;
        }
    }
    *out = ctx;
    return PAGK_OK;
}

void pagk_destroy(pagk_ctx *ctx)
{
    if (!ctx) return;
    (void)hipSetDevice(ctx->device);
    if (ctx->own_stream) (void)hipStreamSynchronize(ctx->own_stream);
    if (ctx->aux_stream) {
        (void)hipStreamSynchronize(ctx->aux_stream);
        (void)hipStreamDestroy(ctx->aux_stream);
    }
    if (ctx->ev_fork) (void)hipEventDestroy(ctx->ev_fork);
    if (ctx->ev_join) (void)hipEventDestroy(ctx->ev_join);
    for (int k = 0; k < pagk_ctx::kGraphs; k++) {
        if (ctx->graph_execs[k]) {
            (void)hipGraphExecDestroy(ctx->graph_execs[k]);
            (void)hipGraphDestroy(ctx->graphs[k]);
        }
        destroy_segs(ctx->pre_segs[k]);
    }
    destroy_segs(ctx->cap_segs);
    for (auto &s : ctx->slots) (void)release(ctx, s.block);
    for (auto &b : ctx->buf) (void)release(ctx, b);
    if (ctx->queue) (void)hipFree(ctx->queue);
    if (ctx->prio_stats) (void)hipFree(ctx->prio_stats);
    for (auto &d : ctx->batch_ring) batch_desc_free(d);
    batch_desc_free(ctx->cap_batch);
    for (int k = 0; k < pagk_ctx::kGraphs; k++) batch_desc_free(ctx->graph_batch[k]);
    if (ctx->ev_batch) (void)hipEventDestroy(ctx->ev_batch);
    if (ctx->lv_error) (void)hipHostFree(ctx->lv_error);
    for (int k = 0; k < 2; k++) {
        if (ctx->ev_trk[k]) (void)hipEventDestroy(ctx->ev_trk[k]);
        if (ctx->ev_pyr[k]) (void)hipEventDestroy(ctx->ev_pyr[k]);
    }
    if (ctx->own_stream) (void)hipStreamDestroy(ctx->own_stream);
    delete ctx;
}

int pagk_set_stream(pagk_ctx *ctx, void *hip_stream)
{
    if (!ctx) return PAGK_E_ARG;
    ctx->stream = hip_stream ? static_cast<hipStream_t>(hip_stream) : ctx->own_stream;
    return PAGK_OK;
}

int pagk_has_variant(int32_t which)
{
    return which >= 0 && which <= 7 && (kAllVariants || (which != 2 && which != 6));
}

int pagk_set_kernel(pagk_ctx *ctx, int32_t which)
{
    if (!ctx || which < 0 || which > 7) return PAGK_E_ARG;
    if (!pagk_has_variant(which)) {
        snprintf(ctx->err, sizeof(ctx->err), "variant %d is not in this build of libpagk_hip.so (compile with -DPAGK_ALL_VARIANTS)", which);
        return PAGK_E_UNSUPPORTED;
    }
    ctx->kernel = which;
    return PAGK_OK;
}

int pagk_last_variant(const pagk_ctx *ctx) { return ctx ? ctx->last_variant : PAGK_E_ARG; }

int pagk_last_handover(pagk_ctx *ctx)
{
    if (!ctx) return PAGK_E_ARG;
    if (!ctx->last_handover || !ctx->susp_count_dev) return 0;
    HIPCHK(ctx, hipSetDevice(ctx->device));
    int count = 0;
    HIPCHK(ctx, hipMemcpyAsync(&count, ctx->susp_count_dev, sizeof count, hipMemcpyDeviceToHost, ctx->stream));
    HIPCHK(ctx, hipStreamSynchronize(ctx->stream));
    if (int lr = lv_check(ctx)) return lr;
    return count;
}

int pagk_priority_threshold(pagk_ctx *ctx)
{
    if (!ctx) return PAGK_E_ARG;
    if (!ctx->prio_stats) return ctx->prio_k;
    HIPCHK(ctx, hipSetDevice(ctx->device));
    int k = 0;
    HIPCHK(ctx, hipMemcpyAsync(&k, ctx->prio_stats + 2, sizeof k, hipMemcpyDeviceToHost, ctx->stream));
    HIPCHK(ctx, hipStreamSynchronize(ctx->stream));
    if (int lr = lv_check(ctx)) return lr;
    return k;
}

int pagk_check_launch(pagk_ctx *ctx)
{
    if (!ctx) return PAGK_E_ARG;
    return lv_check(ctx);
}

int pagk_set_concurrency(pagk_ctx *ctx, int32_t streams)
{
    if (!ctx || streams < 1 || streams > 64) return PAGK_E_ARG;
    ctx->concurrency = streams;
    return PAGK_OK;
}

int pagk_sync(pagk_ctx *ctx)
{
    if (!ctx) return PAGK_E_ARG;
    NOT_WHILE_CAPTURING(ctx, "pagk_sync");
    HIPCHK(ctx, hipStreamSynchronize(ctx->stream));
    return lv_check(ctx);
}

int pagk_last_kernel_ms(pagk_ctx *ctx, float *track_ms, float *pyramid_ms)
{
    if (!ctx) return PAGK_E_ARG;
    NOT_WHILE_CAPTURING(ctx, "pagk_last_kernel_ms");
    if (track_ms) {
        *track_ms = 0.0f;
        if (ctx->trk_timed) {
            HIPCHK(ctx, hipEventSynchronize(ctx->ev_trk[1]));
            HIPCHK(ctx, hipEventElapsedTime(track_ms, ctx->ev_trk[0], ctx->ev_trk[1]));
        }
    }
    if (pyramid_ms) {
        *pyramid_ms = 0.0f;
        if (ctx->pyr_timed) {
            HIPCHK(ctx, hipEventSynchronize(ctx->ev_pyr[1]));
            HIPCHK(ctx, hipEventElapsedTime(pyramid_ms, ctx->ev_pyr[0], ctx->ev_pyr[1]));
        }
    }
    return PAGK_OK;
}

static int frame_upload_any(pagk_ctx *ctx, int32_t slot, const pagk_image *img, int32_t pyramids);

int pagk_frame_upload(pagk_ctx *ctx, int32_t slot, const pagk_image *img, int32_t pyramids)
{
    if (!ctx || slot < 0 || slot >= kUserSlots) return PAGK_E_ARG;
    NOT_WHILE_CAPTURING(ctx, "pagk_frame_upload");
    int rc = frame_upload_any(ctx, slot, img, pyramids);
    if (rc) return rc;
    HIPCHK(ctx, hipStreamSynchronize(ctx->stream));
    return PAGK_OK;
}

int pagk_frame_upload_pinned(pagk_ctx *ctx, int32_t slot, const pagk_image *img, int32_t pyramids)
{
    if (!ctx || slot < 0 || slot >= kUserSlots) return PAGK_E_ARG;
    return frame_upload_any(ctx, slot, img, pyramids);
}

static int frame_upload_any(pagk_ctx *ctx, int32_t slot, const pagk_image *img, int32_t pyramids)
{
    if (!ctx || slot < 0 || slot >= kSlots || pyramids < 1 || pyramids > PAGK_MAX_PYRAMIDS) return PAGK_E_ARG;
    int rc = check_image(img);
    if (rc) return rc;
    HIPCHK(ctx, hipSetDevice(ctx->device));
    FrameSlot &s = ctx->slots[slot];
    s.valid = false;
    if ((rc = slot_reserve(ctx, s, img->width, img->height, pyramids))) return rc;
    if ((rc = upload_level0(ctx, s, img))) return rc;
    rc = slot_build(ctx, s, s.u8[0], s.w, img->step == img->width);
    s.pad0 = (int)(img->step - img->width > 2 ? 2 : img->step - img->width);
    return rc;
}

int pagk_frame_set_device(pagk_ctx *ctx, int32_t slot, const void *d_data, int32_t width, int32_t height,
                          int64_t step, int32_t pyramids)
{
    if (!ctx || slot < 0 || slot >= kUserSlots || pyramids < 1 || pyramids > PAGK_MAX_PYRAMIDS) return PAGK_E_ARG;
    if (!d_data || width < 1 || height < 1 || step < width) return PAGK_E_ARG;
    if (width >= (1 << 24) || height >= (1 << 24) || (int64_t)width * height >= (1ll << 31)) return PAGK_E_ARG;
// ... 600 lines not shown
int pagk_gyro_predict_device(pagk_ctx *ctx, const pagk_params *params, int32_t width, int32_t height,
                             const float *KRKinv, const float *r3, int32_t n, const float *d_pt_ref_un,
                             float *d_pt_predict_un, float *d_pt_predict, uint8_t *d_status, float *d_affine)
{
    return gyro_predict_any(ctx, params, width, height, KRKinv, r3, nullptr, n, d_pt_ref_un, d_pt_predict_un,
                            d_pt_predict, d_status, d_affine);
}

int pagk_gyro_predict_device_rot(pagk_ctx *ctx, const pagk_params *params, int32_t width, int32_t height,
                                 const float *d_rot, int32_t n, const float *d_pt_ref_un, float *d_pt_predict_un,
                                 float *d_pt_predict, uint8_t *d_status, float *d_affine)
{
    if (!d_rot) return PAGK_E_ARG;
    return gyro_predict_any(ctx, params, width, height, nullptr, nullptr, d_rot, n, d_pt_ref_un, d_pt_predict_un,
                            d_pt_predict, d_status, d_affine);
}

int pagk_gyro_predict_device_live(pagk_ctx *ctx, const pagk_params *params, int32_t width, int32_t height,
                                  const float *d_rot, int32_t n, const float *d_pt_ref_un, const uint8_t *d_live,
                                  float *d_pt_predict_un, float *d_pt_predict, uint8_t *d_status, float *d_affine)
{
    if (!d_rot || (n > 0 && !d_live)) return PAGK_E_ARG;
    return gyro_predict_any(ctx, params, width, height, nullptr, nullptr, d_rot, n, d_pt_ref_un, d_pt_predict_un,
                            d_pt_predict, d_status, d_affine, d_live);
}

int pagk_post_filter(int32_t n, int32_t half_patch, const uint8_t *status_pm, const double *pix_err,
                     const double *dist_pred, const float *pt_pm, const float *pt_pm_un, uint8_t *status_out,
                     float *pt_predict, float *pt_predict_un)
{
    if (n < 0 || (n > 0 && (!status_pm || !pix_err || !dist_pred || !status_out))) return PAGK_E_ARG;
    double sum = 0;
    int cnt = 0;
    for (int i = 0; i < n; ++i)
        if (status_pm[i]) {
            sum += pix_err[i];
            cnt++;
        }
    const double avg = sum / cnt;
    const double th_pix = 4.0 * avg > half_patch ? 4.0 * avg : half_patch;
    const double th_dist = half_patch * 4.0;
    int kept = 0;
    for (int i = 0; i < n; i++) {
        const bool ok = status_pm[i] && pix_err[i] < th_pix && dist_pred[i] < th_dist;
        status_out[i] = ok ? 1 : 0;
        if (!ok) continue;
        if (pt_predict && pt_pm) {
            pt_predict[2 * i] = pt_pm[2 * i];
            pt_predict[2 * i + 1] = pt_pm[2 * i + 1];
        }
        if (pt_predict_un && pt_pm_un) {
            pt_predict_un[2 * i] = pt_pm_un[2 * i];
            pt_predict_un[2 * i + 1] = pt_pm_un[2 * i + 1];
        }
        kept++;
    }
    return kept;
}


int pagk_post_filter_device(pagk_ctx *ctx, int32_t n, int32_t half_patch, const uint8_t *d_status_pm,
                            const double *d_pix_err, const double *d_dist_pred, const float *d_pt_pm,
                            const float *d_pt_pm_un, uint8_t *d_status_out, float *d_pt_predict,
                            float *d_pt_predict_un, int32_t *d_kept, double *d_thresholds)
{
    if (!ctx || n < 0 || !d_kept) return PAGK_E_ARG;
    if (n > 0 && (!d_status_pm || !d_pix_err || !d_dist_pred || !d_status_out)) return PAGK_E_ARG;
    HIPCHK(ctx, hipSetDevice(ctx->device));
    hipLaunchKernelGGL(k_post_filter, dim3(1), dim3(1024), 0, ctx->stream, n, half_patch, d_status_pm, d_pix_err,
                       d_dist_pred, d_pt_pm, d_pt_pm_un, d_status_out, d_pt_predict, d_pt_predict_un, d_kept, d_thresholds);
    HIPCHK(ctx, hipGetLastError());
    return PAGK_OK;
}

namespace {

bool handover_args_ok(const pagk_params *params, int32_t width, int32_t height, int32_t cap, int32_t target_n,
                      double new_point_threshold, int32_t cand_cap)
{
    return params && width >= 14 && height >= 14 && (int64_t)width * height <= 0x7fffffff && cap >= 1 && target_n >= 0 &&
           cap >= target_n && cand_cap >= 0 && !std::isnan(new_point_threshold);
}

void handover_fill_args(HandoverArgs *out, const pagk_params *params, int32_t width, int32_t height, int32_t cap,
                        int32_t target_n, double new_point_threshold)
{
    HandoverArgs a;
    memset(&a, 0, sizeof a);
    a.cap = cap, a.width = width, a.height = height, a.target_n = target_n;
    a.new_point_threshold = new_point_threshold;
    a.fx = params->fx, a.fy = params->fy, a.cx = params->cx, a.cy = params->cy;
    a.fx_inv = (float)(1.0 / (double)params->fx);
    a.fy_inv = (float)(1.0 / (double)params->fy);
    a.k1 = params->dist_coef[0], a.k2 = params->dist_coef[1], a.p1 = params->dist_coef[2], a.p2 = params->dist_coef[3];
    a.k3 = params->n_dist_coef == 5 ? params->dist_coef[4] : 0.0f;
    a.distort_on = params->dist_coef[0] != 0.0f;
    *out = a;
}

int handover_launch(pagk_ctx *ctx, const pagk_params *params, int32_t width, int32_t height, int32_t cap, int32_t target_n,
                    double new_point_threshold, const uint8_t *d_status, const float *d_pt_predict,
                    const float *d_pt_predict_un, int32_t cand_cap, const int32_t *d_n_cand, const float *d_cand_un,
                    float *d_keys, float *d_keys_un, float *d_keys_normal, int32_t *d_index_in_last, uint8_t *d_live,
                    uint8_t *d_mask, int32_t *d_state, const pagk_detect_params *det = nullptr,
                    const FrameSlot *s = nullptr, int32_t *d_info = nullptr);

int handover_host(pagk_ctx *ctx, const pagk_params *params, int32_t width, int32_t height, int32_t cap, int32_t target_n,
                  double new_point_threshold, const uint8_t *status, const float *pt_predict, const float *pt_predict_un,
                  int32_t cand_cap, const int32_t *n_cand, const float *cand_un, const pagk_detect_params *det,
                  const pagk_fast_params *fast, float *keys, float *keys_un, float *keys_normal, int32_t *index_in_last,
                  uint8_t *live, uint8_t *mask, int32_t *state, int32_t *info);

}

int pagk_frame_handover_device(pagk_ctx *ctx, const pagk_params *params, int32_t width, int32_t height, int32_t cap,
                               int32_t target_n, double new_point_threshold, const uint8_t *d_status,
                               const float *d_pt_predict, const float *d_pt_predict_un, int32_t cand_cap,
                               const int32_t *d_n_cand, const float *d_cand_un, float *d_keys, float *d_keys_un,
                               float *d_keys_normal, int32_t *d_index_in_last, uint8_t *d_live, uint8_t *d_mask,
                               int32_t *d_state)
{
    if (!ctx || !handover_args_ok(params, width, height, cap, target_n, new_point_threshold, cand_cap)) return PAGK_E_ARG;
    if (!d_status || !d_pt_predict || !d_pt_predict_un || !d_n_cand || (cand_cap > 0 && !d_cand_un) || !d_keys ||
        !d_keys_un || !d_index_in_last || !d_live || !d_state)
        return PAGK_E_ARG;
    if (d_keys == d_pt_predict || d_keys_un == d_pt_predict_un) return PAGK_E_ARG;
    return handover_launch(ctx, params, width, height, cap, target_n, new_point_threshold, d_status, d_pt_predict,
                           d_pt_predict_un, cand_cap, d_n_cand, d_cand_un, d_keys, d_keys_un, d_keys_normal, d_index_in_last,
                           d_live, d_mask, d_state);
}

int pagk_frame_handover(pagk_ctx *ctx, const pagk_params *params, int32_t width, int32_t height, int32_t cap,
                        int32_t target_n, double new_point_threshold, const uint8_t *status, const float *pt_predict,
                        const float *pt_predict_un, int32_t cand_cap, const int32_t *n_cand, const float *cand_un,
                        float *keys, float *keys_un, float *keys_normal, int32_t *index_in_last, uint8_t *live,
                        uint8_t *mask, int32_t *state)
{
    if (!ctx || !handover_args_ok(params, width, height, cap, target_n, new_point_threshold, cand_cap)) return PAGK_E_ARG;
    NOT_WHILE_CAPTURING(ctx, "pagk_frame_handover");
    if (!status || !pt_predict || !pt_predict_un || !n_cand || (cand_cap > 0 && !cand_un) || !keys || !keys_un ||
        !index_in_last || !live || !state)
        return PAGK_E_ARG;
    HIPCHK(ctx, hipSetDevice(ctx->device));
    return handover_host(ctx, params, width, height, cap, target_n, new_point_threshold, status, pt_predict, pt_predict_un,
                         cand_cap, n_cand, cand_un, nullptr, nullptr, keys, keys_un, keys_normal, index_in_last, live, mask, state,
                         nullptr);
}

namespace {

bool detect_params_ok(const pagk_detect_params *d)
{
    return d && std::isfinite(d->quality_level) && d->quality_level >= 0.0 && std::isfinite(d->min_distance) &&
           d->min_distance >= 0.0 && std::isfinite(d->harris_k) && d->raw_cap >= 0;
}

int64_t detect_raw_bound(int w, int h) { return (int64_t)((w - 2 + 1) / 2) * ((h - 2 + 1) / 2); }

struct DetectWs {
    int32_t *ctl = nullptr, *grid = nullptr;
    float *R = nullptr, *cand = nullptr;
    uint64_t *keys = nullptr;
    uint32_t key_slots = 0;
    int32_t raw_cap = 0, cell = 1, grid_w = 1, grid_h = 1, reach = 1;
};

// ... 35 lines not shown
{
    hipLaunchKernelGGL(k_detect_response, dim3((s.w + kDetTileW - 1) / kDetTileW, (s.h + kDetTileH - 1) / kDetTileH), dim3(256),
                       0, ctx->stream, s.img0, s.pitch0, s.w, s.h, d_mask, harris_k, ws.R, ws.ctl, d_skip);
    HIPCHK(ctx, hipGetLastError());
    return PAGK_OK;
}

int detect_launch(pagk_ctx *ctx, const pagk_detect_params *det, const FrameSlot &s, const uint8_t *d_mask, int32_t cap,
                  const int32_t *d_max_corners, const int32_t *d_skip, float *d_corners, int32_t *d_info, const DetectWs &ws)
{
    HIPCHK(ctx, hipMemsetAsync(ws.ctl, 0, 8, ctx->stream));
    int rc = detect_response_launch(ctx, s, d_mask, det->harris_k, ws, d_skip);
    if (rc) return rc;
    hipLaunchKernelGGL(k_detect_nms, dim3((s.w + 63) / 64, (s.h + 3) / 4), dim3(256), 0, ctx->stream, ws.R, s.w, s.h, d_mask,
                       det->quality_level, ws.ctl, ws.keys, ws.raw_cap, d_skip);
    HIPCHK(ctx, hipGetLastError());
    const uint32_t N = ws.key_slots;
    const size_t sort_lds = (size_t)kDetSortBlock * sizeof(uint64_t);
    if (!in_capture(ctx))
        HIPCHK(ctx, hipFuncSetAttribute(reinterpret_cast<const void *>(k_detect_sort_local),
                                        hipFuncAttributeMaxDynamicSharedMemorySize, (int)sort_lds));
    hipLaunchKernelGGL(k_detect_sort_local, dim3(N / kDetSortBlock), dim3(1024), sort_lds, ctx->stream, ws.keys, ws.ctl,
                       ws.raw_cap, 0u, d_skip);
    for (uint32_t k = 2 * kDetSortBlock; k <= N; k <<= 1) {
        for (uint32_t j = k >> 1; j >= (uint32_t)kDetSortBlock; j >>= 1)
            hipLaunchKernelGGL(k_detect_sort_step, dim3(N / 2 / 256), dim3(256), 0, ctx->stream, ws.keys, ws.ctl, ws.raw_cap, k, j,
                               d_skip);
        hipLaunchKernelGGL(k_detect_sort_local, dim3(N / kDetSortBlock), dim3(1024), sort_lds, ctx->stream, ws.keys, ws.ctl,
                           ws.raw_cap, k, d_skip);
    }
    HIPCHK(ctx, hipGetLastError());
    DetectWalkArgs a;
    memset(&a, 0, sizeof a);
    a.keys = ws.keys, a.ctl = ws.ctl, a.max_corners = d_max_corners, a.skip = d_skip;
    a.raw_cap = ws.raw_cap, a.cap = cap, a.width = s.w, a.height = s.h;
    a.min_distance = det->min_distance;
    a.cell = ws.cell, a.grid_w = ws.grid_w, a.grid_h = ws.grid_h, a.reach = ws.reach, a.grid = ws.grid;
    a.corners = d_corners, a.info = d_info;
    hipLaunchKernelGGL(k_detect_walk, dim3(1), dim3(1024), 0, ctx->stream, a);
    HIPCHK(ctx, hipGetLastError());
    return PAGK_OK;
}

bool detect_slot_ok(const FrameSlot &s) { return s.valid && s.img0 && s.w >= 14 && s.h >= 14; }

int detect_corners_slot(pagk_ctx *ctx, const pagk_detect_params *det, int32_t slot, const uint8_t *d_mask, int32_t cap,
                        const int32_t *d_max_corners, float *d_corners, int32_t *d_info)
{
    const FrameSlot &s = ctx->slots[slot];
    if (!detect_slot_ok(s)) return PAGK_E_ARG;
    HIPCHK(ctx, hipSetDevice(ctx->device));
    DetectWs ws;
    int rc = detect_workspace(ctx, det, s.w, s.h, cap, &ws);
    if (rc) return rc;
    return detect_launch(ctx, det, s, d_mask, cap, d_max_corners, nullptr, d_corners, d_info, ws);
}

int handover_launch(pagk_ctx *ctx, const pagk_params *params, int32_t width, int32_t height, int32_t cap, int32_t target_n,
                    double new_point_threshold, const uint8_t *d_status, const float *d_pt_predict,
                    const float *d_pt_predict_un, int32_t cand_cap, const int32_t *d_n_cand, const float *d_cand_un,
                    float *d_keys, float *d_keys_un, float *d_keys_normal, int32_t *d_index_in_last, uint8_t *d_live,
                    uint8_t *d_mask, int32_t *d_state, const pagk_detect_params *det, const FrameSlot *s, int32_t *d_info)
{
    HIPCHK(ctx, hipSetDevice(ctx->device));
    const int64_t bytes = (int64_t)width * height;
    DevBuf &hand = ctx->buf[pagk_ctx::HAND];
    int rc = d_mask ? PAGK_OK
                    : reserve(ctx, hand, align_up((size_t)bytes, kPartAlign), NOT_IN_CAPTURE_NOR_UNDER_GRAPH, "the hand-over's mask",
                              "run the call once with this image size before capturing, or pass d_mask");
    if (rc) return rc;
    uint8_t *mask = d_mask ? d_mask : static_cast<uint8_t *>(hand.ptr);
    DetectWs ws;
    if (det) {
        if ((rc = detect_workspace(ctx, det, width, height, cap, &ws))) return rc;
        cand_cap = cap, d_n_cand = d_info, d_cand_un = ws.cand;
    }
    HandoverArgs a;
    handover_fill_args(&a, params, width, height, cap, target_n, new_point_threshold);
    a.cand_cap = cand_cap;
    a.status = d_status, a.pt_predict = d_pt_predict, a.pt_predict_un = d_pt_predict_un;
    a.n_cand = d_n_cand, a.cand_un = d_cand_un;
    a.keys = d_keys, a.keys_un = d_keys_un, a.keys_normal = d_keys_normal;
    a.index_in_last = d_index_in_last, a.live = d_live, a.mask = mask, a.state = d_state;
    hipLaunchKernelGGL(k_handover_fill, dim3((unsigned)((bytes + 4095) / 4096)), dim3(256), 0, ctx->stream, mask, bytes);
    HIPCHK(ctx, hipGetLastError());
    hipLaunchKernelGGL(k_handover_holes, dim3((unsigned)(((int64_t)cap * 14 + 255) / 256)), dim3(256), 0, ctx->stream, cap,
                       width, height, d_status, d_pt_predict_un, mask);
    HIPCHK(ctx, hipGetLastError());
    if (det) {
        hipLaunchKernelGGL(k_handover_plan, dim3(1), dim3(1024), 0, ctx->stream, cap, target_n, new_point_threshold, d_status,
                           (const int32_t *)d_state, ws.ctl);
        HIPCHK(ctx, hipGetLastError());
        if ((rc = detect_launch(ctx, det, *s, mask, cap, ws.ctl + kDetCtlLimit, ws.ctl + kDetCtlSkip, ws.cand, d_info, ws)))
            return rc;
    }
    hipLaunchKernelGGL(k_handover_keys, dim3(1), dim3(1024), 0, ctx->stream, a);
    HIPCHK(ctx, hipGetLastError());
    return PAGK_OK;
}

}

void pagk_detect_params_default(pagk_detect_params *p)
{
    if (!p) return;
    p->quality_level = 0.005;
    p->min_distance = 20.0;
    p->harris_k = 0.04;
    p->raw_cap = 0;
}

int pagk_detect_corners_device(pagk_ctx *ctx, const pagk_detect_params *det, int32_t slot, const uint8_t *d_mask,
                               int32_t cap, const int32_t *d_max_corners, float *d_corners, int32_t *d_info)
{
    if (!ctx || !detect_params_ok(det) || slot < 0 || slot >= kUserSlots || cap < 1 || !d_corners || !d_info) return PAGK_E_ARG;
    return detect_corners_slot(ctx, det, slot, d_mask, cap, d_max_corners, d_corners, d_info);
}

int pagk_detect_corners(pagk_ctx *ctx, const pagk_detect_params *det, const pagk_image *img, const uint8_t *mask,
                        int32_t max_corners, float *corners, int32_t *info)
{
    if (!ctx || !detect_params_ok(det) || !img || max_corners < 0 || (max_corners > 0 && !corners)) return PAGK_E_ARG;
    NOT_WHILE_CAPTURING(ctx, "pagk_detect_corners");
    if (img->width < 14 || img->height < 14) return PAGK_E_ARG;
    int rc = frame_upload_any(ctx, 4, img, 1);
    if (rc) return rc;
    const size_t px = (size_t)img->width * img->height, cap = (size_t)(max_corners > 0 ? max_corners : 1);
    const size_t sizes[4] = {px, cap * 8, 256, 256};
    Staged<4> s(ctx, sizes);
    if ((rc = s.open(nullptr, nullptr)) || (rc = s.in(0, mask, px)) || (rc = s.in(3, &max_corners, 4))) return rc;
    rc = detect_corners_slot(ctx, det, 4, mask ? s.at<uint8_t>(0) : nullptr, (int32_t)cap, s.at<int32_t>(3), s.at<float>(1),
                             s.at<int32_t>(2));
    if (rc || (rc = s.out(1, corners, (size_t)max_corners * 8)) || (rc = s.out(2, info, kDetectInfoWords * 4))) return rc;
    return s.finish();
}

int pagk_selftest_corner_response(pagk_ctx *ctx, const pagk_image *img, float *R)
{
    if (!ctx || !img || !R) return PAGK_E_ARG;
    NOT_WHILE_CAPTURING(ctx, "pagk_selftest_corner_response");
    if (img->width < 14 || img->height < 14) return PAGK_E_ARG;
    int rc = frame_upload_any(ctx, 4, img, 1);
    if (rc) return rc;
    pagk_detect_params det;
    pagk_detect_params_default(&det);
    DetectWs ws;
    if ((rc = detect_workspace(ctx, &det, img->width, img->height, 1, &ws))) return rc;
    HIPCHK(ctx, hipMemsetAsync(ws.ctl, 0, 8, ctx->stream));
    if ((rc = detect_response_launch(ctx, ctx->slots[4], nullptr, det.harris_k, ws, nullptr))) return rc;
    HIPCHK(ctx, hipMemcpyAsync(R, ws.R, (size_t)img->width * img->height * 4, hipMemcpyDeviceToHost, ctx->stream));
    HIPCHK(ctx, hipStreamSynchronize(ctx->stream));
    return PAGK_OK;
}

int pagk_frame_handover_detect_device(pagk_ctx *ctx, const pagk_params *params, int32_t width, int32_t height,
                                      int32_t cap, int32_t target_n, double new_point_threshold, const uint8_t *d_status,
                                      const float *d_pt_predict, const float *d_pt_predict_un,
                                      const pagk_detect_params *det, int32_t slot, float *d_keys, float *d_keys_un,
                                      float *d_keys_normal, int32_t *d_index_in_last, uint8_t *d_live, uint8_t *d_mask,
                                      int32_t *d_state, int32_t *d_info)
{
    if (!ctx || !handover_args_ok(params, width, height, cap, target_n, new_point_threshold, 0) || !detect_params_ok(det) ||
        slot < 0 || slot >= kUserSlots)
        return PAGK_E_ARG;
    if (!d_status || !d_pt_predict || !d_pt_predict_un || !d_keys || !d_keys_un || !d_index_in_last || !d_live || !d_state ||
        !d_info)
// ... 76 lines not shown
    int rc = reserve(ctx, ctx->buf[pagk_ctx::FAST], lay.total, NOT_IN_CAPTURE_NOR_UNDER_GRAPH, "the FAST detector's workspace",
                     "run the call once with this image size and n_features before capturing");
    if (rc) return rc;
    void *b = ctx->buf[pagk_ctx::FAST].ptr;
    ws->ctl = lay.at<int32_t>(b, 0), ws->cell_cnt = lay.at<int32_t>(b, 1), ws->cell_off = lay.at<int32_t>(b, 2);
    ws->seg_xy = lay.at<uint32_t>(b, 3), ws->seg_score = lay.at<int32_t>(b, 4);
    ws->kxy = lay.at<uint32_t>(b, 5), ws->kscore = lay.at<int32_t>(b, 6), ws->knode = lay.at<int32_t>(b, 7);
    ws->box[0] = lay.at<int4>(b, 8), ws->box[1] = lay.at<int4>(b, 9);
    ws->ncnt[0] = lay.at<int32_t>(b, 10), ws->ncnt[1] = lay.at<int32_t>(b, 11);
    ws->ncand[0] = lay.at<int32_t>(b, 12), ws->ncand[1] = lay.at<int32_t>(b, 13);
    ws->cnt4 = lay.at<int32_t>(b, 14), ws->cbase = lay.at<int32_t>(b, 15), ws->split = lay.at<int32_t>(b, 16);
    ws->sortk = lay.at<unsigned long long>(b, 17), ws->best = lay.at<unsigned long long>(b, 18);
    ws->cand = lay.at<float>(b, 19);
    ws->sort_slots = slots, ws->raw_bound = (int32_t)rb, ws->out_bound = (int32_t)ob, ws->n_cells = (int32_t)nc;
    return PAGK_OK;
}

int fast_cells_launch(pagk_ctx *ctx, const pagk_fast_params *fp, const FrameSlot &s, const FastGrid &g, const FastWs &ws,
                      const int32_t *d_skip)
{
    FastCellArgs c;
    memset(&c, 0, sizeof c);
    c.img = s.img0, c.pitch = s.pitch0, c.g = g, c.t_ini = fp->ini_threshold, c.t_min = fp->min_threshold;
    c.seg_xy = ws.seg_xy, c.seg_score = ws.seg_score, c.cell_cnt = ws.cell_cnt, c.skip = d_skip;
    hipLaunchKernelGGL(k_fast_cells, dim3(ws.n_cells), dim3(256), 0, ctx->stream, c);
    HIPCHK(ctx, hipGetLastError());
    hipLaunchKernelGGL(k_fast_offsets, dim3(1), dim3(1024), 0, ctx->stream, ws.n_cells, (const int32_t *)ws.cell_cnt, ws.cell_off,
                       ws.ctl, d_skip);
    HIPCHK(ctx, hipGetLastError());
    hipLaunchKernelGGL(k_fast_gather, dim3(ws.n_cells), dim3(256), 0, ctx->stream, g.seg, (const int32_t *)ws.cell_cnt,
                       (const int32_t *)ws.cell_off, (const uint32_t *)ws.seg_xy, (const int32_t *)ws.seg_score, ws.kxy, ws.kscore,
                       d_skip);
    HIPCHK(ctx, hipGetLastError());
    return PAGK_OK;
}

int fast_launch(pagk_ctx *ctx, const pagk_fast_params *fp, int32_t n_features, const FrameSlot &s, const FastGrid &g,
                const uint8_t *d_mask, int32_t cap, float *d_keypoints, float *d_response, int32_t *d_info,
                const int32_t *d_skip, const FastWs &ws)
{
    int rc = fast_cells_launch(ctx, fp, s, g, ws, d_skip);
    if (rc) return rc;
    FastTreeArgs t;
    memset(&t, 0, sizeof t);
    t.g = g, t.n_features = n_features, t.cap = cap, t.out_bound = ws.out_bound, t.raw_bound = ws.raw_bound;
    t.sort_slots = ws.sort_slots, t.ctl = ws.ctl, t.kxy = ws.kxy, t.kscore = ws.kscore, t.knode = ws.knode;
    for (int k = 0; k < 2; k++) t.box[k] = ws.box[k], t.ncnt[k] = ws.ncnt[k], t.ncand[k] = ws.ncand[k];
    t.cnt4 = ws.cnt4, t.cbase = ws.cbase, t.split = ws.split, t.sortk = ws.sortk, t.best = ws.best;
    t.mask = d_mask, t.out_xy = d_keypoints, t.out_resp = d_response, t.info = d_info, t.skip = d_skip;
    hipLaunchKernelGGL(k_fast_tree, dim3(1), dim3(1024), 0, ctx->stream, t);
    HIPCHK(ctx, hipGetLastError());
    return PAGK_OK;
}

bool fast_slot_ok(const FrameSlot &s) { return s.valid && s.img0; }

int handover_fast_launch(pagk_ctx *ctx, const pagk_params *params, int32_t width, int32_t height, int32_t cap,
                         int32_t target_n, double new_point_threshold, const uint8_t *d_status, const float *d_pt_predict,
                         const float *d_pt_predict_un, const pagk_fast_params *fp, const FrameSlot &s, float *d_keys,
                         float *d_keys_un, float *d_keys_normal, int32_t *d_index_in_last, uint8_t *d_live, uint8_t *d_mask,
                         int32_t *d_state, int32_t *d_info)
{
    HIPCHK(ctx, hipSetDevice(ctx->device));
    FastGrid g;
    if (!fast_grid(width, height, &g)) return PAGK_E_ARG;
    const int32_t n_features = fp->n_features ? fp->n_features : target_n;
    if (n_features < 1) return PAGK_E_ARG;
    const int64_t bytes = (int64_t)width * height;
    DevBuf &hand = ctx->buf[pagk_ctx::HAND];
    int rc = d_mask ? PAGK_OK
                    : reserve(ctx, hand, align_up((size_t)bytes, kPartAlign), NOT_IN_CAPTURE_NOR_UNDER_GRAPH, "the hand-over's mask",
                              "run the call once with this image size before capturing, or pass d_mask");
    if (rc) return rc;
    uint8_t *mask = d_mask ? d_mask : static_cast<uint8_t *>(hand.ptr);
    FastWs ws;
    if ((rc = fast_workspace(ctx, g, n_features, &ws))) return rc;
    HandoverArgs a;
    handover_fill_args(&a, params, width, height, cap, target_n, new_point_threshold);
    a.cand_cap = ws.out_bound;
    a.status = d_status, a.pt_predict = d_pt_predict, a.pt_predict_un = d_pt_predict_un;
    a.n_cand = d_info, a.cand_un = ws.cand;
    a.keys = d_keys, a.keys_un = d_keys_un, a.keys_normal = d_keys_normal;
    a.index_in_last = d_index_in_last, a.live = d_live, a.mask = mask, a.state = d_state;
    hipLaunchKernelGGL(k_handover_fill, dim3((unsigned)((bytes + 4095) / 4096)), dim3(256), 0, ctx->stream, mask, bytes);
    HIPCHK(ctx, hipGetLastError());
    hipLaunchKernelGGL(k_handover_holes, dim3((unsigned)(((int64_t)cap * 14 + 255) / 256)), dim3(256), 0, ctx->stream, cap,
                       width, height, d_status, d_pt_predict_un, mask);
    HIPCHK(ctx, hipGetLastError());
    hipLaunchKernelGGL(k_handover_plan, dim3(1), dim3(1024), 0, ctx->stream, cap, target_n, new_point_threshold, d_status,
                       (const int32_t *)d_state, ws.ctl);
    HIPCHK(ctx, hipGetLastError());
    if ((rc = fast_launch(ctx, fp, n_features, s, g, nullptr, ws.out_bound, ws.cand, nullptr, d_info, ws.ctl + kFastCtlSkip, ws)))
        return rc;
    hipLaunchKernelGGL(k_handover_keys, dim3(1), dim3(1024), 0, ctx->stream, a);
    HIPCHK(ctx, hipGetLastError());
    return PAGK_OK;
}

}

void pagk_fast_params_default(pagk_fast_params *p)
{
    if (!p) return;
    p->ini_threshold = 20;
    p->min_threshold = 7;
    p->n_features = 0;
    p->n_levels = 1;
}

int pagk_fast_params_check(const pagk_fast_params *p) { return fast_params_check(p); }

int pagk_detect_fast_bounds(int32_t width, int32_t height, int32_t n_features, int32_t *raw_bound, int32_t *out_bound)
{
    FastGrid g;
    if (n_features < 1 || n_features > (1 << 24) || !fast_grid(width, height, &g) || fast_raw_bound(g) > (1 << 30)) return PAGK_E_ARG;
    if (raw_bound) *raw_bound = (int32_t)fast_raw_bound(g);
    if (out_bound) *out_bound = fast_out_bound(g, n_features);
    return PAGK_OK;
}

static int detect_fast_slot(pagk_ctx *ctx, const pagk_fast_params *params, int32_t slot, const uint8_t *d_mask, int32_t cap,
                            float *d_keypoints, float *d_response, int32_t *d_info)
{
    if (!ctx) return PAGK_E_ARG;
    int rc = fast_params_check(params);
    if (rc) return rc;
    if (params->n_features < 1 || slot < 0 || slot >= kSlots || !d_keypoints || !d_info) return PAGK_E_ARG;
    const FrameSlot &s = ctx->slots[slot];
    FastGrid g;
    if (!fast_slot_ok(s) || !fast_grid(s.w, s.h, &g) || cap < fast_out_bound(g, params->n_features)) return PAGK_E_ARG;
    HIPCHK(ctx, hipSetDevice(ctx->device));
    FastWs ws;
    if ((rc = fast_workspace(ctx, g, params->n_features, &ws))) return rc;
    return fast_launch(ctx, params, params->n_features, s, g, d_mask, cap, d_keypoints, d_response, d_info, nullptr, ws);
}

int pagk_detect_fast_device(pagk_ctx *ctx, const pagk_fast_params *params, int32_t slot, const uint8_t *d_mask, int32_t cap,
                            float *d_keypoints, float *d_response, int32_t *d_info)
{
    if (slot < 0 || slot >= kUserSlots) return PAGK_E_ARG;
    return detect_fast_slot(ctx, params, slot, d_mask, cap, d_keypoints, d_response, d_info);
}

int pagk_detect_fast(pagk_ctx *ctx, const pagk_fast_params *params, const pagk_image *img, const uint8_t *mask, int32_t cap,
                     float *keypoints, float *response, int32_t *info)
{
    if (!ctx || !img) return PAGK_E_ARG;
    int rc = fast_params_check(params);
    if (rc) return rc;
    NOT_WHILE_CAPTURING(ctx, "pagk_detect_fast");
    FastGrid g;
    if (params->n_features < 1 || !keypoints || !fast_grid(img->width, img->height, &g) ||
        cap < fast_out_bound(g, params->n_features))
        return PAGK_E_ARG;
    if ((rc = frame_upload_any(ctx, 4, img, 1))) return rc;
    const size_t px = (size_t)img->width * img->height, nc = (size_t)cap;
    const size_t sizes[4] = {px, nc * 8, nc * 4, 256};
    Staged<4> s(ctx, sizes);
    if ((rc = s.open(nullptr, nullptr)) || (rc = s.in(0, mask, px))) return rc;
    rc = detect_fast_slot(ctx, params, 4, mask ? s.at<uint8_t>(0) : nullptr, cap, s.at<float>(1), s.at<float>(2), s.at<int32_t>(3));
    if (rc || (rc = s.out(1, keypoints, nc * 8)) || (rc = s.out(2, response, nc * 4)) || (rc = s.out(3, info, kDetectInfoWords * 4)))
        return rc;
    return s.finish();
}

int pagk_selftest_fast_cells(pagk_ctx *ctx, const pagk_fast_params *params, const pagk_image *img, float *raw_xy,
// ... 1572 lines not shown
```

### pixel_aware_gyro_aided_klt_feature_tracker_amd/csrc/pagk_kernels.h

```cpp
#pragma once
#include <type_traits>
#include "pagk_device.h"
#include "pagk_chain_asm.h"
#include "pagk_prio.h"

namespace pagk {

__global__ void k_pyr_down(const uint8_t *__restrict__ src, int64_t pitch, int dw, int dh,
                           uint8_t *__restrict__ dst)
{
    int x = blockIdx.x * blockDim.x + threadIdx.x;
    int y = blockIdx.y * blockDim.y + threadIdx.y;
    if (x >= dw || y >= dh) return;
    const uint8_t *r0 = src + (int64_t)(2 * y) * pitch + 2 * x;
    const uint8_t *r1 = r0 + pitch;
    dst[(int64_t)y * dw + x] = (uint8_t)((r0[0] + r0[1] + r1[0] + r1[1] + 2) >> 2);
}

__global__ void k_pyr_down_linear(const uint8_t *__restrict__ src, int64_t pitch, int w, int h, int dw, int dh,
                                  double scale_x, double scale_y, uint8_t *__restrict__ dst)
{
    const int dx = blockIdx.x * blockDim.x + threadIdx.x;
    const int dy = blockIdx.y * blockDim.y + threadIdx.y;
    if (dx >= dw || dy >= dh) return;
// ... 383 lines not shown
template <int N>
__device__ __forceinline__ double row_shr_f64(double v)
{
    int lo = __double2loint(v), hi = __double2hiint(v);
    lo = __builtin_amdgcn_update_dpp(0, lo, 0x110 + N, 0xf, 0xf, false);
    hi = __builtin_amdgcn_update_dpp(0, hi, 0x110 + N, 0xf, 0xf, false);
    return __hiloint2double(hi, lo);
}
template <int N>
__device__ __forceinline__ float row_shr_f32(float v)
{
    return __int_as_float(__builtin_amdgcn_update_dpp(0, __float_as_int(v), 0x110 + N, 0xf, 0xf, false));
}
__device__ __forceinline__ double relaxed_row_f64(const double *arr, int P, int lr, double s1)
{
    double s0 = 0.0, s1a = 0.0, s2 = 0.0, s3 = 0.0;
    int k = lr;
    for (; k + 48 < P; k += 64) {
        s0 = __builtin_fma(arr[k], s1, s0);
        s1a = __builtin_fma(arr[k + 16], s1, s1a);
        s2 = __builtin_fma(arr[k + 32], s1, s2);
        s3 = __builtin_fma(arr[k + 48], s1, s3);
    }
    for (; k < P; k += 16) s0 = __builtin_fma(arr[k], s1, s0);
    double s = (s0 + s1a) + (s2 + s3);
    s += row_shr_f64<8>(s);
    s += row_shr_f64<4>(s);
    s += row_shr_f64<2>(s);
    s += row_shr_f64<1>(s);
    return s;
}
__device__ __forceinline__ float relaxed_row_f32(const float *arr, int P, int lr)
{
    float s0 = 0.0f, s1 = 0.0f;
    int k = lr;
    for (; k + 16 < P; k += 32) {
        s0 += arr[k];
        s1 += arr[k + 16];
    }
    for (; k < P; k += 16) s0 += arr[k];
    float s = s0 + s1;
    s += row_shr_f32<8>(s);
    s += row_shr_f32<4>(s);
    s += row_shr_f32<2>(s);
    s += row_shr_f32<1>(s);
    return s;
}

template <int NR, int TAIL, int WAVES = 4, bool MFMA = false, bool RELAXED = false, bool LEAN = false, bool PIPE = true>
__device__ __forceinline__ void track_block_body(const TrackArgs &a, const int i, const SuspState *resume = nullptr)
{
    static_assert(MFMA ? WAVES == 2 : WAVES == 4, "DPP rows need 4 waves; the MFMA variant is 2 waves");
    static_assert(!(MFMA && RELAXED), "the relaxed-order experiment exists for the 4-wave kernel only");
    constexpr int kBlock = WAVES * 64;
    constexpr int kStreams = MFMA ? 3 : 8;
    constexpr int kAcc = MFMA ? 24 : 16;
    constexpr int HC = (NR == 2 && !MFMA) ? (TAIL == 1 ? 8 : (TAIL == 9 ? 9 : 10)) : 0;
#ifndef PAGK_NO_PIPE
    if constexpr (HC != 0 && !RELAXED && PIPE) {
        track_pipe_body<HC, LEAN>(a, i, resume);
        return;
    }
#endif
    extern __shared__ __attribute__((aligned(16))) unsigned char lds_raw[];
    const int tid = threadIdx.x;
    const int wave = tid >> 6, lane = tid & 63;
    const int h = HC ? HC : a.half, Wd = 2 * h + 1, P = Wd * Wd, PP = track_block_pp(h);
    const int nfull = P / 32;

    const int PS = MFMA ? PP + 8 : PP + 1;
    double *stream = reinterpret_cast<double *>(lds_raw);
    double *cst = stream + (size_t)kStreams * PS;
    float *esq = reinterpret_cast<float *>(cst + (MFMA ? 16 : 0));
    double *cslot = reinterpret_cast<double *>(esq + PP);
    double *acc = cslot + 2;
    double *sh_upd = acc + kAcc;
    float *sh_cost = reinterpret_cast<float *>(sh_upd + 5);
#ifdef PAGK_EXPERIMENT_LDS_WINDOW
    uint32_t *win = reinterpret_cast<uint32_t *>(sh_cost + 2);
#endif

    const float *init = a.has_gyro ? a.pt_init : a.pt_ref;
    float p2x = init[2 * i], p2y = init[2 * i + 1];
    if (!a.status_in[i]) {
        if (tid == 0) write_outputs(a, i, p2x, p2y, 0, 0.0f, 0, 0.0f, 0);
        return;
    }
    float A00 = 1, A01 = 0, A10 = 0, A11 = 1;
    if (a.use_affine) {
        A00 = a.affine[4 * i], A01 = a.affine[4 * i + 1], A10 = a.affine[4 * i + 2], A11 = a.affine[4 * i + 3];
    }
    const float refx = a.pt_ref[2 * i], refy = a.pt_ref[2 * i + 1];

    float px[NR], py[NR], wx[NR], wy[NR];
#pragma unroll
    for (int r = 0; r < NR; r++) {
        int p = tid + kBlock * r;
        p = p < P ? p : P - 1;
        int yy = p / Wd, xx = p - yy * Wd;
        int x = xx - h, y = yy - h;
        px[r] = (float)x;
        py[r] = (float)y;
        if (a.use_affine) {
            wx[r] = A00 * (float)x + A01 * (float)y;
            wy[r] = A10 * (float)x + A11 * (float)y;
        } else {
            wx[r] = (float)x;
            wy[r] = (float)y;
        }
    }
    const float fh = (float)h;
    const float ext_x = fabsf(A00) * fh + fabsf(A01) * fh + 2.0f;
    const float ext_y = fabsf(A10) * fh + fabsf(A11) * fh + 2.0f;

    const int lr = lane & 15;
    const int cid = wave * 4 + (lane >> 4);
    const int stream_of[12] = {0, 1, 2, 3, 4, 5, 6, 5, 6, 7, 7, 0};
    uint32_t row_addr, row_inc;
    if constexpr (RELAXED || MFMA) {
        if (MFMA || cid >= 12) {
            row_addr = lds_off(esq) + 8u * lr;
            row_inc = 128u;
        } else if (cid < 11) {
            row_addr = lds_off(stream + (size_t)stream_of[cid] * PS) + 16u * lr;
            row_inc = 256u;
        } else {
            row_addr = lds_off(cslot);
            row_inc = 0u;
        }
    } else {
        if (cid < 8) {
            row_addr = lds_off(stream + (size_t)cid * PS) + 16u * lr;
            row_inc = 256u;
        } else if (cid < 12) {
            row_addr = lds_off(esq) + 8u * lr;
            row_inc = 128u;
        } else {
            row_addr = lds_off(cslot);
            row_inc = 0u;
        }
    }
    const int mk = lane >> 4, mq = (lane >> 2) & 3, mi = lane & 3;
    const double *j_src = mi < 2 ? stream + (size_t)mi * PS + mk : cst + (mi == 2 ? 0 : 4) + mk;
    const int j_step = mi < 2 ? 4 : 0;
    const double *a_src = mq < 2 ? j_src : cst + 8 + mk;
    const int a_step = mq < 2 ? j_step : 0;
    const double *b_src = mq == 0 ? j_src : ((mq == 1 && mi == 0) ? stream + (size_t)2 * PS + mk : cst + 8 + mk);
    const int b_step = mq == 0 ? j_step : ((mq == 1 && mi == 0) ? 4 : 0);
    if constexpr (MFMA) {
        if (tid < 4) {
            cst[4 + tid] = 1.0;
            cst[8 + tid] = 0.0;
        }
    }

    int succ = 1, iters = 0;
    [[maybe_unused]] constexpr bool kPrioByWork = NR > 1;
    PAGK_PRIO_DECL
    float lastCost = 0.0f;
#ifdef PAGK_STAMPS
    unsigned long long st[14] = {0, 0, 0, 0, 0, 0, 0, 0, 0, 0, 0, 0, 0, 0};
    unsigned long long t_begin = __builtin_amdgcn_s_memtime(), t0, t1;
    const unsigned long long rt_begin = __builtin_amdgcn_s_memrealtime();
#define STAMP(k)                                  \
    t1 = __builtin_amdgcn_s_memtime();            \
    st[k] += t1 - t0;                             \
    t0 = t1;
#else
#define STAMP(k)
#endif

    const int level_first = resume ? resume->level : a.n_levels - 1;
    for (int level = level_first; level >= 0; level--) {
#ifdef PAGK_STAMPS
        t0 = __builtin_amdgcn_s_memtime();
#endif
        const DevLevel &L1 = a.l1[level];
        const DevLevel L2 = pin_level(a.l2[level]);
        const float ptx = refx * a.scales[level], pty = refy * a.scales[level];
        float nx, ny;
        if (level == a.n_levels - 1) {
            nx = p2x * a.scales[level];
            ny = p2y * a.scales[level];
        } else {
            nx = (float)((double)(p2x * 1.0f) / 0.5);
            ny = (float)((double)(p2y * 1.0f) / 0.5);
        }
        float dx = nx - ptx, dy = ny - pty, dg = 0.0f, db = 0.0f;
        lastCost = 0.0f;
        succ = 1;
        int iter_first = 0;
        if (resume && level == level_first) {
            dx = resume->dx, dy = resume->dy, dg = resume->dg, db = resume->db;
            lastCost = resume->lastCost;
            iters = resume->iters;
            iter_first = resume->iter;
        }

        const float cneg = -sample<true>(L1, ptx, pty);
        const double cd = (double)cneg;
        float s1[NR];
#pragma unroll
        for (int r = 0; r < NR; r++) s1[r] = sample<true>(L1, ptx + px[r], pty + py[r]);
        double row_s1;
        if constexpr (RELAXED) {
            switch (cid) {
                case 3: case 4: case 10: row_s1 = -1.0; break;
                case 5: case 6: case 11: row_s1 = cd; break;
                case 9: row_s1 = -cd; break;
                default: row_s1 = 1.0; break;
            }
        } else {
            switch (cid) {
                case 3: case 4: row_s1 = -1.0; break;
                case 5: case 6: row_s1 = lr == 0 ? cd : 1.0; break;
                case 7: row_s1 = lr == 0 ? -cd : -1.0; break;
                default: row_s1 = cid >= 12 ? cd : 1.0; break;
            }
        }
        if (tid == 0) {
            cslot[0] = cd;
            cslot[1] = cd;
        }
        if constexpr (MFMA) {
            if (tid < 4) cst[tid] = cd;
        }

        STAMP(0)
        for (int iter = iter_first; iter < a.iterations; iter++) {
            iters++;
            PAGK_PRIO_TIER
            const float bx = ptx + dx, by = pty + dy;
            const float gain = 1.0f + dg;
            const bool interior = (bx - ext_x >= 0.0f) & (bx + ext_x < L2.fcols_m1) &
                                  (by - ext_y >= 0.0f) & (by + ext_y < L2.frows_m1);
            auto sampling = [&](auto mode_tag, auto rounds_tag) {
            constexpr int NRX = decltype(rounds_tag)::value;
            constexpr int G = NRX < 2 ? NRX : 2;
            constexpr int MODE = decltype(mode_tag)::value;
#pragma unroll
            for (int r0 = 0; r0 < NRX; r0 += G) {
// ... 246 lines not shown
                }
            }
            __syncthreads();
            PRIO(PAGK_PRIO_N_REST)
            STAMP(3)
            const double u0 = sh_upd[0], u1 = sh_upd[1], u2 = sh_upd[2], u3 = sh_upd[3], unorm = sh_upd[4];
            const float cost = sh_cost[1];
            if (u0 != u0) {
                succ = 0;
                break;
            }
            if (iter > 0 && cost > lastCost) break;
            dx = (float)((double)dx + u0);
            dy = (float)((double)dy + u1);
            if (a.illum) {
                dg = (float)((double)dg + u2);
                db = (float)((double)db + u3);
            }
            lastCost = cost;
            succ = 1;
            if (unorm < kNormSqConverged) break;
#ifdef PAGK_STAMPS
            asm volatile("" : "+v"(dx), "+v"(dy), "+v"(dg), "+v"(db));
            STAMP(12)
#endif
        }
        p2x = ptx + dx;
        p2y = pty + dy;
    }
    PAGK_PRIO_RESET
    float ncc = 1.0f;
    if (a.calc_ncc) {
        float *vref = reinterpret_cast<float *>(stream), *vcur = vref + PP;
        float *tnum = vcur + PP, *td1 = tnum + PP, *td2 = td1 + PP;
        const DevLevel &R0 = a.l1[0], &C0 = a.l2[0];
        float vr[NR], vc[NR];
        __syncthreads();
#pragma unroll
        for (int r = 0; r < NR; r++) {
            int k = tid + kBlock * r;
            k = k < P ? k : P - 1;
            int xi = k / Wd - h, yi = k - (k / Wd) * Wd - h;
            vr[r] = sample<true>(R0, refx + xi, refy + yi);
            if (a.use_affine) {
                float wxx = A00 * xi + A01 * yi, wyy = A10 * xi + A11 * yi;
                vc[r] = sample<true>(C0, p2x + wxx, p2y + wyy);
            } else {
                vc[r] = sample<true>(C0, p2x + xi, p2y + yi);
            }
            if (tid + kBlock * r < P) {
                vref[tid + kBlock * r] = vr[r];
                vcur[tid + kBlock * r] = vc[r];
            }
        }
        __syncthreads();
        const int row = lane >> 4;
        float *sh_f = reinterpret_cast<float *>(acc);
        if (wave == 0) {
            float m = chain_rows_f32<TAIL>(lds_off(row == 1 ? vcur : vref) + 8u * lr, 128u, nfull);
            if (lr == 0 && row < 2) sh_f[row] = m;
        }
        __syncthreads();
        const float mean_ref = sh_f[0] / (float)P, mean_cur = sh_f[1] / (float)P;
#pragma unroll
        for (int r = 0; r < NR; r++) {
            int k = tid + kBlock * r;
            if (k < P) {
                float dr = vr[r] - mean_ref, dc = vc[r] - mean_cur;
                tnum[k] = dr * dc;
                td1[k] = dr * dr;
                td2[k] = dc * dc;
            }
        }
        __syncthreads();
        if (wave == 0) {
            const float *src = row == 0 ? tnum : (row == 1 ? td1 : td2);
            float v = chain_rows_f32<TAIL>(lds_off(src) + 8u * lr, 128u, nfull);
            if (lr == 0 && row < 3) sh_f[2 + row] = v;
        }
        __syncthreads();
        ncc = (float)((double)sh_f[2] / sqrt((double)(sh_f[3] * sh_f[4]) + 1e-10));
    }
    if (tid == 0) write_outputs(a, i, p2x, p2y, succ, lastCost, 1, ncc, iters);
    if (tid == 0 && kPrioByWork && !resume) prio_account(a, i, iters, a.n_levels);
#ifdef PAGK_STAMPS
    if (tid == 0 && a.dbg) {
        unsigned long long *dbgp = a.dbg + (resume ? (size_t)16 * (a.susp_waves > 0 ? a.susp_waves : (a.n + 3) / 4) : 0);
        st[5] = __builtin_amdgcn_s_memtime() - t_begin;
        for (int k = 0; k < 6; k++) dbgp[(size_t)i * 16 + k] = st[k];
        dbgp[(size_t)i * 16 + 6] = (unsigned long long)iters;
        dbgp[(size_t)i * 16 + 7] = rt_begin;
        for (int k = 8; k < 11; k++) dbgp[(size_t)i * 16 + k] = st[k];
        dbgp[(size_t)i * 16 + 11] = __builtin_amdgcn_s_memrealtime();
        dbgp[(size_t)i * 16 + 12] = st[12];
        dbgp[(size_t)i * 16 + 13] = st[13];
    }
#endif
#undef STAMP
}

template <int NR, int TAIL, int WAVES = 4, bool MFMA = false, bool RELAXED = false, bool LEAN = false>
__global__ void __launch_bounds__(WAVES * 64, 4) k_track_block(TrackArgs a)
{
    track_block_body<NR, TAIL, WAVES, MFMA, RELAXED, LEAN>(a, (int)blockIdx.x);
}

template <int NR, int TAIL, bool LEAN = false>
__global__ void __launch_bounds__(256, 5) k_track_block5(TrackArgs a)
{
    track_block_body<NR, TAIL, 4, false, false, LEAN, false>(a, (int)blockIdx.x);
}

__device__ __forceinline__ SuspState load_susp_state(const TrackArgs &a, int i)
{
    const int *p = reinterpret_cast<const int *>(&a.susp_state[i]);
    SuspState st;
    st.level = ld_agent(p + 0), st.iter = ld_agent(p + 1);
    st.dx = __int_as_float(ld_agent(p + 2)), st.dy = __int_as_float(ld_agent(p + 3));
    st.dg = __int_as_float(ld_agent(p + 4)), st.db = __int_as_float(ld_agent(p + 5));
    st.lastCost = __int_as_float(ld_agent(p + 6)), st.iters = ld_agent(p + 7);
    return st;
}

template <int NR, int TAIL, bool LEAN = false>
__global__ void __launch_bounds__(256, 4) k_track_resume_live(TrackArgs a)
{
    __shared__ int s_entry;
    const int tid = threadIdx.x;
    int polls = 0;
    for (;;) {
        if (tid == 0) {
            int entry = 0;
            const int ticket = atomicAdd(a.susp_count + 1, 1);
            if (ticket < a.n) {
                for (;;) {
                    entry = __hip_atomic_load(a.susp_list + ticket, __ATOMIC_ACQUIRE, __HIP_MEMORY_SCOPE_AGENT);
                    if (entry != 0) break;
                    if (ld_agent(a.susp_count + 2) >= a.susp_waves) {
                        entry = __hip_atomic_load(a.susp_list + ticket, __ATOMIC_ACQUIRE, __HIP_MEMORY_SCOPE_AGENT);
                        break;
                    }
                    if (++polls > a.susp_polls) break;
                    __builtin_amdgcn_s_sleep(64);
                }
            }
            s_entry = entry > 0 ? ticket + 1 : 0;
        }
        __syncthreads();
        const int slot = s_entry - 1;
        if (slot < 0) return;
        const int i = ld_agent(a.susp_list + slot) - 1;
        const SuspState st = load_susp_state(a, i);
        track_block_body<NR, TAIL, 4, false, false, LEAN>(a, i, &st);
        __syncthreads();
        if (tid == 0) st_agent(a.susp_list + slot, -(i + 1));
    }
}

template <int NR, int TAIL, bool LEAN = false>
__global__ void __launch_bounds__(256, 4) k_track_resume(TrackArgs a)
{
    const int count = *a.susp_count;
    for (int b = (int)blockIdx.x; b < count; b += (int)gridDim.x) {
        const int entry = a.susp_list[b];
        if (entry <= 0) continue;
        const int i = entry - 1;
// ... 34 lines not shown
```

### pixel_aware_gyro_aided_klt_feature_tracker_amd/csrc/pagk_multi.h

```cpp
#pragma once
#include <dlfcn.h>

#include <mutex>

namespace {

struct Id128 {
    char internal[128];
};
struct Rccl {
    void *lib = nullptr;
    int (*GetUniqueId)(void *) = nullptr;
    int (*CommInitAll)(void **, int, const int *) = nullptr;
    int (*CommInitRank)(void **, int, Id128 , int) = nullptr;
    int (*CommDestroy)(void *) = nullptr;
    int (*AllGather)(const void *, void *, size_t, int, void *, hipStream_t) = nullptr;
    int (*GroupStart)() = nullptr;
    int (*GroupEnd)() = nullptr;
    const char *(*GetErrorString)(int) = nullptr;
    int (*CommCount)(void *, int *) = nullptr;
};

void rccl_load_once(Rccl &r, char *err, size_t errn)
{
// ... 243 lines not shown
            snprintf((pm)->err, sizeof((pm)->err), "%s:%d %s -> %s", __FILE__, __LINE__, #call,     \
                     hipGetErrorString(e_));                                                         \
            return e_ == hipErrorOutOfMemory ? PAGK_E_NOMEM : PAGK_E_HIP;                            \
        }                                                                                            \
    } while (0)

int pagk_track_sharded(pagk_multi *pm, const pagk_params *params, const pagk_image *ref, const pagk_image *cur,
                       int32_t n, const float *pt_ref_un, const float *pt_init_un, const float *affine,
                       const uint8_t *status_in, const pagk_outputs *out)
{
    if (!pm || pm->n_local != pm->world) return PAGK_E_ARG;
    int rc = check_params(params);
    if (rc) return rc;
    if ((rc = check_image(ref)) || (rc = check_image(cur))) return rc;
    if (ref->width != cur->width || ref->height != cur->height) return PAGK_E_ARG;
    if (n < 0 || !out || !out->pt_un || !out->status) return PAGK_E_ARG;
    if (n > 0 && (!pt_ref_un || !status_in)) return PAGK_E_ARG;
    if (n > 0 && params->has_gyro_predict_initial && !pt_init_un) return PAGK_E_ARG;
    if (n > 0 && params->consider_affine && !affine) return PAGK_E_ARG;
    const int G = pm->world, m = (n + G - 1) / G;
    size_t off[7];
    const size_t slice = pagk_shard_layout(m, off);
    const size_t mm = (size_t)(m < 1 ? 1 : m);
    const size_t in_off[4] = {0, mm * 8, mm * 16, mm * 32};
    const size_t in_bytes = mm * 33;
    auto drain = [&](int upto) {
        for (int j = 0; j < upto && j < G; j++) {
            (void)hipSetDevice(pm->ctx[j]->device);
            (void)hipStreamSynchronize(pm->ctx[j]->stream);
        }
    };
    for (int k = 0; k < G; k++) {
        pagk_ctx *c = pm->ctx[k];
        pagk_multi::Stage &s = pm->stage[k];
        MHIPCHK(pm, hipSetDevice(c->device));
        if (s.in_bytes < in_bytes) {
            if (s.d_in) MHIPCHK(pm, hipFree(s.d_in));
            if (s.h_in) MHIPCHK(pm, hipHostFree(s.h_in));
            s.d_in = s.h_in = nullptr, s.in_bytes = 0;
            MHIPCHK(pm, hipMalloc(&s.d_in, in_bytes));
            MHIPCHK(pm, hipHostMalloc(&s.h_in, in_bytes, hipHostMallocDefault));
            s.in_bytes = in_bytes;
        }
        if (s.slice_bytes < slice) {
            if (s.d_slice) MHIPCHK(pm, hipFree(s.d_slice));
            s.d_slice = nullptr, s.slice_bytes = 0;
            MHIPCHK(pm, hipMalloc(&s.d_slice, slice));
            MHIPCHK(pm, hipMemset(s.d_slice, 0, slice));
            s.slice_bytes = slice;
        }
        if (s.all_bytes < slice * G) {
            if (s.d_all) MHIPCHK(pm, hipFree(s.d_all));
            if (s.h_all) MHIPCHK(pm, hipHostFree(s.h_all));
            s.d_all = s.h_all = nullptr, s.all_bytes = 0;
            MHIPCHK(pm, hipMalloc(&s.d_all, slice * G));
            if (k == 0) MHIPCHK(pm, hipHostMalloc(&s.h_all, slice * G, hipHostMallocDefault));
            s.all_bytes = slice * G;
        }
        if ((rc = frame_upload_any(c, 4, ref, params->pyramids)) || (rc = frame_upload_any(c, 5, cur, params->pyramids))) {
            snprintf(pm->err, sizeof pm->err, "rank %d: %s", k, c->err);
            drain(k);
            return rc;
        }
        int lo, hi;
        pagk_shard_range(n, k, G, &lo, &hi);
        const int nk = hi - lo;
        uint8_t *hb = static_cast<uint8_t *>(s.h_in), *db = static_cast<uint8_t *>(s.d_in);
        if (nk > 0) {
            memcpy(hb + in_off[0], pt_ref_un + 2 * (size_t)lo, (size_t)nk * 8);
            if (pt_init_un) memcpy(hb + in_off[1], pt_init_un + 2 * (size_t)lo, (size_t)nk * 8);
            if (affine) memcpy(hb + in_off[2], affine + 4 * (size_t)lo, (size_t)nk * 16);
            memcpy(hb + in_off[3], status_in + lo, (size_t)nk);
            MHIPCHK(pm, hipMemcpyAsync(db, hb, in_bytes, hipMemcpyHostToDevice, c->stream));
        }
        uint8_t *sl = static_cast<uint8_t *>(s.d_slice);
        pagk_outputs o;
        o.pt_un = reinterpret_cast<float *>(sl + off[0]);
        o.pt_dist = reinterpret_cast<float *>(sl + off[1]);
        o.status = sl + off[2];
        o.pix_err = reinterpret_cast<double *>(sl + off[3]);
        o.dist_pred = reinterpret_cast<double *>(sl + off[4]);
        o.ncc = reinterpret_cast<float *>(sl + off[5]);
        o.iters = reinterpret_cast<int32_t *>(sl + off[6]);
        rc = launch_track(c, params, c->slots[4], c->slots[5], nk, reinterpret_cast<float *>(db + in_off[0]),
                          pt_init_un ? reinterpret_cast<float *>(db + in_off[1]) : nullptr,
                          affine ? reinterpret_cast<float *>(db + in_off[2]) : nullptr, db + in_off[3], &o);
        if (rc) {
            snprintf(pm->err, sizeof pm->err, "rank %d: %s", k, c->err);
            drain(k);
            return rc;
        }
    }
    std::vector<const void *> snd((size_t)G);
    std::vector<void *> rcv((size_t)G);
    for (int k = 0; k < G; k++) snd[(size_t)k] = pm->stage[k].d_slice, rcv[(size_t)k] = pm->stage[k].d_all;
    if ((rc = pagk_multi_allgather(pm, snd.data(), rcv.data(), slice, nullptr))) {
        drain(G);
        return rc;
    }
    MHIPCHK(pm, hipSetDevice(pm->ctx[0]->device));
    MHIPCHK(pm, hipMemcpyAsync(pm->stage[0].h_all, pm->stage[0].d_all, slice * G, hipMemcpyDeviceToHost, pm->ctx[0]->stream));
    int lv_rc = PAGK_OK;
    for (int k = 0; k < G; k++) {
        MHIPCHK(pm, hipSetDevice(pm->ctx[k]->device));
        MHIPCHK(pm, hipStreamSynchronize(pm->ctx[k]->stream));
        if (int r = lv_check(pm->ctx[k])) {
            snprintf(pm->err, sizeof pm->err, "rank %d: %s", k, pm->ctx[k]->err);
            lv_rc = r;
        }
    }
    if (lv_rc) return lv_rc;
    const uint8_t *all = static_cast<const uint8_t *>(pm->stage[0].h_all);
    for (int k = 0; k < G; k++) {
        int lo, hi;
        pagk_shard_range(n, k, G, &lo, &hi);
        const size_t nk = (size_t)(hi - lo);
        if (!nk) continue;
        const uint8_t *sl = all + (size_t)k * slice;
        memcpy(out->pt_un + 2 * (size_t)lo, sl + off[0], nk * 8);
        if (out->pt_dist) memcpy(out->pt_dist + 2 * (size_t)lo, sl + off[1], nk * 8);
        memcpy(out->status + lo, sl + off[2], nk);
        if (out->pix_err) memcpy(out->pix_err + lo, sl + off[3], nk * 8);
        if (out->dist_pred) memcpy(out->dist_pred + lo, sl + off[4], nk * 8);
        if (out->ncc) memcpy(out->ncc + lo, sl + off[5], nk * 4);
        if (out->iters) memcpy(out->iters + lo, sl + off[6], nk * 4);
    }
    return PAGK_OK;
}

}
```

### pixel_aware_gyro_aided_klt_feature_tracker_amd/csrc/pagk_pipe_kernel.h

```cpp
#pragma once

namespace pagk {


__device__ __forceinline__ void lds_write_b32(uint32_t addr, int v)
{
    asm volatile("ds_write_b32 %0, %1" ::"v"(addr), "v"(v) : "memory");
}

template <int H, bool LEAN>
__device__ __forceinline__ void track_pipe_body(const TrackArgs &a, const int i, const SuspState *resume = nullptr)
{
    static_assert(H >= 8 && H <= 10, "two-round patches only");
    constexpr int kBlock = 256;
    constexpr int Wd = 2 * H + 1, P = Wd * Wd, PP = (P + 31) / 32 * 32, PS = PP + 1;
    constexpr int TAIL = P % 32;
    constexpr bool HAS_B = P > 320, HAS_C = P > 384;
    extern __shared__ __attribute__((aligned(16))) unsigned char lds_raw[];
    const int tid = threadIdx.x;
    const int wave = __builtin_amdgcn_readfirstlane(tid >> 6), lane = tid & 63;

    double *stream = reinterpret_cast<double *>(lds_raw);
    float *esq = reinterpret_cast<float *>(stream + (size_t)8 * PS);
    double *cslot = reinterpret_cast<double *>(esq + PP);
    double *acc = cslot + 2;
    double *sh_upd = acc + 16;
    float *sh_cost = reinterpret_cast<float *>(sh_upd + 5);
    int *flags = reinterpret_cast<int *>(sh_cost + 2 + 2);
    double *h22 = reinterpret_cast<double *>(flags + 4);
    double *sh_pen = h22 + 2;

    const float *init = a.has_gyro ? a.pt_init : a.pt_ref;
    float p2x = init[2 * i], p2y = init[2 * i + 1];
    if (!a.status_in[i]) {
        if (tid == 0) write_outputs(a, i, p2x, p2y, 0, 0.0f, 0, 0.0f, 0);
        return;
    }
    float A00 = 1, A01 = 0, A10 = 0, A11 = 1;
    if (a.use_affine) {
        A00 = a.affine[4 * i], A01 = a.affine[4 * i + 1], A10 = a.affine[4 * i + 2], A11 = a.affine[4 * i + 3];
    }
    const float refx = a.pt_ref[2 * i], refy = a.pt_ref[2 * i + 1];
    if (tid < 4) flags[tid] = 0;

    int pix[3];
    pix[0] = tid;
    pix[1] = (wave == 3 ? 320 : 256) + lane;
    pix[2] = 384 + lane;
    float px[3], py[3], wx[3], wy[3];
#pragma unroll
    for (int r = 0; r < 3; r++) {
        const int p = pix[r] < P ? pix[r] : P - 1;
        const int yy = p / Wd, xx = p - yy * Wd;
        const int x = xx - H, y = yy - H;
        px[r] = (float)x;
        py[r] = (float)y;
        if (a.use_affine) {
            wx[r] = A00 * (float)x + A01 * (float)y;
            wy[r] = A10 * (float)x + A11 * (float)y;
        } else {
            wx[r] = (float)x;
            wy[r] = (float)y;
        }
    }
    const float fh = (float)H;
    const float ext_x = fabsf(A00) * fh + fabsf(A01) * fh + 2.0f;
    const float ext_y = fabsf(A10) * fh + fabsf(A11) * fh + 2.0f;

    const int lr = lane & 15;
    const int cid = wave * 4 + (lane >> 4);
    const int row_stream = (0x76423510 >> (4 * cid)) & 15;
    const uint32_t row_addr = wave < 2 ? lds_off(stream + (size_t)row_stream * PS) + 16u * lr : lds_off(esq) + 8u * lr;
    const uint32_t flag_addr = lds_off(flags);
    const int acc_slot = wave == 1 ? (lr == 0 ? (cid == 7 ? 4 : cid - 4) : ((lr == 1 && cid >= 6) ? 2 * cid - 9 : -1)) : -1;

    int succ = 1, iters = 0, seq = 0;
    [[maybe_unused]] constexpr bool kPrioByWork = true;
    PAGK_PRIO_DECL
    float lastCost = 0.0f;
#ifdef PAGK_STAMPS
    unsigned long long st[14] = {0, 0, 0, 0, 0, 0, 0, 0, 0, 0, 0, 0, 0, 0};
    unsigned long long t_begin = __builtin_amdgcn_s_memtime(), t0, t1;
    const unsigned long long rt_begin = __builtin_amdgcn_s_memrealtime();
#define STAMP(k)                                  \
    t1 = __builtin_amdgcn_s_memtime();            \
    st[k] += t1 - t0;                             \
    t0 = t1;
#else
#define STAMP(k)
#endif
#if defined(PAGK_TIC) && defined(PAGK_TOC)
    unsigned long long pt_t0 = 0, pt_sum = 0;
#define POINT(k)                                                                   \
    if (wave == 0) {                                                               \
        if ((k) == PAGK_TIC) pt_t0 = __builtin_amdgcn_s_memtime();                 \
        if ((k) == PAGK_TOC) pt_sum += __builtin_amdgcn_s_memtime() - pt_t0;       \
    }
#else
#define POINT(k)
#endif

    const int level_first = resume ? resume->level : a.n_levels - 1;
    for (int level = level_first; level >= 0; level--) {
#ifdef PAGK_STAMPS
        t0 = __builtin_amdgcn_s_memtime();
#endif
        const DevLevel &L1 = a.l1[level];
        const DevLevel L2 = pin_level(a.l2[level]);
        const float ptx = refx * a.scales[level], pty = refy * a.scales[level];
        float nx, ny;
        if (level == a.n_levels - 1) {
            nx = p2x * a.scales[level];
            ny = p2y * a.scales[level];
        } else {
            nx = (float)((double)(p2x * 1.0f) / 0.5);
            ny = (float)((double)(p2y * 1.0f) / 0.5);
        }
        float dx = nx - ptx, dy = ny - pty, dg = 0.0f, db = 0.0f;
        lastCost = 0.0f;
        succ = 1;
        int iter_first = 0;
        if (resume && level == level_first) {
            dx = resume->dx, dy = resume->dy, dg = resume->dg, db = resume->db;
            lastCost = resume->lastCost;
            iters = resume->iters;
            iter_first = resume->iter;
        }

        const float cneg = -sample<true>(L1, ptx, pty);
        const double cd = (double)cneg;
        float s1[3];
        s1[0] = sample<true>(L1, ptx + px[0], pty + py[0]);
        s1[1] = s1[2] = 0.0f;
        if (wave >= 2) {
            s1[1] = sample<true>(L1, ptx + px[1], pty + py[1]);
            if (HAS_C && wave == 2) s1[2] = sample<true>(L1, ptx + px[2], pty + py[2]);
        }
        double row_s1 = 1.0;
        switch (cid) {
            case 3: case 5: row_s1 = -1.0; break;
            case 2: case 6: row_s1 = lr == 0 ? cd : 1.0; break;
            case 7: row_s1 = lr == 0 ? -cd : -1.0; break;
            default: break;
        }
        if (level == level_first && wave == 1) {
            const double s = repeat_sum_f64(cd * cd, P);
            if (lane == 0) h22[level & 1] = s;
        }

        STAMP(0)
        for (int iter = iter_first; iter < a.iterations; iter++) {
            iters++;
            seq++;
            PAGK_PRIO_TIER
            POINT(0)
            const float bx = ptx + dx, by = pty + dy;
            const float gain = 1.0f + dg;
            const bool interior = (bx - ext_x >= 0.0f) & (bx + ext_x < L2.fcols_m1) &
                                  (by - ext_y >= 0.0f) & (by + ext_y < L2.frows_m1);
            auto emit = [&](const FiveTaps &t, int p, float s1v) {
                const Five s = sample5_finish(t);
// ... 196 lines not shown
                if (a.penalty) cost = (float)((double)cost + sh_pen[0]);
            }
            if (u0 != u0) {
                succ = 0;
                break;
            }
            if (iter > 0 && cost > lastCost) break;
            dx = (float)((double)dx + u0);
            dy = (float)((double)dy + u1);
            if (a.illum) {
                dg = (float)((double)dg + u2);
                db = (float)((double)db + u3);
            }
            lastCost = cost;
            succ = 1;
            if (unorm < kNormSqConverged) break;
#ifdef PAGK_STAMPS
            asm volatile("" : "+v"(dx), "+v"(dy), "+v"(dg), "+v"(db));
            STAMP(12)
#endif
#if defined(PAGK_TIC) && defined(PAGK_TOC)
            asm volatile("" : "+v"(dx), "+v"(dy), "+v"(dg), "+v"(db));
            POINT(5)
#endif
        }
        p2x = ptx + dx;
        p2y = pty + dy;
    }
    PAGK_PRIO_RESET
    float ncc = 1.0f;
    if (a.calc_ncc) {
        float *vref = reinterpret_cast<float *>(stream), *vcur = vref + PP;
        float *tnum = vcur + PP, *td1 = tnum + PP, *td2 = td1 + PP;
        const DevLevel &R0 = a.l1[0], &C0 = a.l2[0];
        constexpr int nfull = P / 32;
        float vr[2], vc[2];
        __syncthreads();
#pragma unroll
        for (int r = 0; r < 2; r++) {
            int k = tid + kBlock * r;
            k = k < P ? k : P - 1;
            int xi = k / Wd - H, yi = k - (k / Wd) * Wd - H;
            vr[r] = sample<true>(R0, refx + xi, refy + yi);
            if (a.use_affine) {
                float wxx = A00 * xi + A01 * yi, wyy = A10 * xi + A11 * yi;
                vc[r] = sample<true>(C0, p2x + wxx, p2y + wyy);
            } else {
                vc[r] = sample<true>(C0, p2x + xi, p2y + yi);
            }
            if (tid + kBlock * r < P) {
                vref[tid + kBlock * r] = vr[r];
                vcur[tid + kBlock * r] = vc[r];
            }
        }
        __syncthreads();
        const int row = lane >> 4;
        float *sh_f = reinterpret_cast<float *>(acc);
        if (wave == 0) {
            float m = chain_rows_f32<TAIL>(lds_off(row == 1 ? vcur : vref) + 8u * lr, 128u, nfull);
            if (lr == 0 && row < 2) sh_f[row] = m;
        }
        __syncthreads();
        const float mean_ref = sh_f[0] / (float)P, mean_cur = sh_f[1] / (float)P;
#pragma unroll
        for (int r = 0; r < 2; r++) {
            int k = tid + kBlock * r;
            if (k < P) {
                float dr = vr[r] - mean_ref, dc = vc[r] - mean_cur;
                tnum[k] = dr * dc;
                td1[k] = dr * dr;
                td2[k] = dc * dc;
            }
        }
        __syncthreads();
        if (wave == 0) {
            const float *src = row == 0 ? tnum : (row == 1 ? td1 : td2);
            float v = chain_rows_f32<TAIL>(lds_off(src) + 8u * lr, 128u, nfull);
            if (lr == 0 && row < 3) sh_f[2 + row] = v;
        }
        __syncthreads();
        ncc = (float)((double)sh_f[2] / sqrt((double)(sh_f[3] * sh_f[4]) + 1e-10));
    }
    if (tid == 0) write_outputs(a, i, p2x, p2y, succ, lastCost, 1, ncc, iters);
    if (tid == 0 && kPrioByWork && !resume) prio_account(a, i, iters, a.n_levels);
#ifdef PAGK_STAMPS
    if (lane == 0 && a.dbg) {
        unsigned long long *dbgp = a.dbg + (resume ? (size_t)16 * (a.susp_waves > 0 ? a.susp_waves : (a.n + 3) / 4) : 0);
        if (wave == 0) {
            st[5] = __builtin_amdgcn_s_memtime() - t_begin;
            for (int k = 0; k < 4; k++) dbgp[(size_t)i * 16 + k] = st[k];
            dbgp[(size_t)i * 16 + 5] = st[5];
            dbgp[(size_t)i * 16 + 6] = (unsigned long long)iters;
            dbgp[(size_t)i * 16 + 7] = rt_begin;
            dbgp[(size_t)i * 16 + 11] = __builtin_amdgcn_s_memrealtime();
            dbgp[(size_t)i * 16 + 12] = st[12];
        } else if (wave == 1) {
            dbgp[(size_t)i * 16 + 4] = st[4];
        } else if (wave == 2) {
            dbgp[(size_t)i * 16 + 8] = st[8];
            dbgp[(size_t)i * 16 + 9] = st[9];
        } else {
            dbgp[(size_t)i * 16 + 10] = st[10];
            dbgp[(size_t)i * 16 + 13] = st[13];
        }
    }
#endif
#if defined(PAGK_TIC) && defined(PAGK_TOC)
    if (tid == 0 && a.dbg) {
        a.dbg[(size_t)i * 2] = pt_sum;
        a.dbg[(size_t)i * 2 + 1] = (unsigned long long)iters;
    }
#endif
#undef STAMP
#undef POINT
}

}
```

### pixel_aware_gyro_aided_klt_feature_tracker_amd/csrc/pagk_prio.h

```cpp
#pragma once

#ifndef PAGK_PRIO_MODE
#define PAGK_PRIO_MODE 1
#endif

namespace pagk {
__device__ __forceinline__ void prio_account(const TrackArgs &a, int i, int iters, int levels)
{
    if (a.prio_stats && (i & 7) == 0) {
        __hip_atomic_fetch_add(a.prio_stats + 0, (unsigned long long)iters, __ATOMIC_RELAXED, __HIP_MEMORY_SCOPE_AGENT);
        __hip_atomic_fetch_add(a.prio_stats + 1, (unsigned long long)levels, __ATOMIC_RELAXED, __HIP_MEMORY_SCOPE_AGENT);
        if ((i & 63) == 0 && iters <= 4 * levels) {
            const unsigned long long it = __hip_atomic_load(a.prio_stats + 0, __ATOMIC_RELAXED, __HIP_MEMORY_SCOPE_AGENT);
            const unsigned long long lv = __hip_atomic_load(a.prio_stats + 1, __ATOMIC_RELAXED, __HIP_MEMORY_SCOPE_AGENT);
            if (lv > 0) {
                int k = (int)ceilf((float)it / (float)lv);
                k = k < 3 ? 3 : (k > 12 ? 12 : k);
                __hip_atomic_store(const_cast<int *>(a.prio_kbuf), k, __ATOMIC_RELAXED, __HIP_MEMORY_SCOPE_AGENT);
            }
        }
    }
}
}
#if PAGK_PRIO_MODE == 0
#define PAGK_PRIO_DECL
#define PAGK_PRIO_TIER
#define PAGK_PRIO_RESET
#define PRIO(n) __builtin_amdgcn_s_setprio(n);
#define PAGK_PRIO_N_CHAIN 3
#define PAGK_PRIO_N_SAMP 2
#define PAGK_PRIO_N_COST 1
#define PAGK_PRIO_N_REST 0
#else
#define PAGK_PRIO_DECL   \
    int tier_now = 0;    \
    const int prio_kv = !kPrioByWork ? 0 : (a.prio_kbuf ? __builtin_amdgcn_readfirstlane(*a.prio_kbuf) : a.prio_k);
#define PAGK_STR2(x) #x
#define PAGK_STR(x) PAGK_STR2(x)
#define PAGK_PRIO_TIER                                                                                              \
    {                                                                                                               \
        const int tier = (prio_kv > 0 && __builtin_amdgcn_readfirstlane(iters - prio_kv * (a.n_levels - level)) > 0) ? 3 : 0; \
        asm volatile("s_cmp_eq_u32 %0, %1\n\t"                                                                      \
                     "s_cbranch_scc1 2f\n\t"                                                                        \
                     "s_cmp_eq_u32 %1, 0\n\t"                                                                       \
                     "s_cbranch_scc1 1f\n\t"                                                                        \
                     "s_setprio 3\n\t"                                                                              \
                     "s_branch 2f\n"                                                                                \
                     "1:\n\t"                                                                                       \
                     "s_setprio 0\n"                                                                                \
                     "2:" ::"s"(tier_now), "s"(tier)                                                                \
                     : "scc");                                                                                      \
        tier_now = tier;                                                                                            \
    }
#define PRIO(n)                                                                                                     \
    asm volatile("s_cmp_lg_u32 %0, 0\n\t"                                                                           \
                 "s_cbranch_scc1 1f\n\t"                                                                            \
                 "s_setprio " PAGK_STR(n) "\n"                                                                      \
                 "1:" ::"s"(tier_now)                                                                               \
                 : "scc");
#define PAGK_PRIO_RESET __builtin_amdgcn_s_setprio(0);
#define PAGK_PRIO_N_CHAIN 2
#define PAGK_PRIO_N_SAMP 1
#define PAGK_PRIO_N_COST 1
#define PAGK_PRIO_N_REST 0
#endif
```

### pixel_aware_gyro_aided_klt_feature_tracker_amd/runtime.py

```python
from __future__ import annotations

import numpy as np
import torch

from . import capi, distributed


def _event_on(stream):
    ev = torch.cuda.Event()
    ev.record(stream)
    return ev


class GatherRing:

    def __init__(self, new_event):
        self.bufs = [None, None]
        self.prev = [None, None]
        self.turn = 0
        self.new_event = new_event

    def issue(self, side, tracked, gather):
        k = self.turn
        self.turn = 1 - k
# ... 14 lines not shown

class ResidentTracker:

    def __init__(self, params: capi.Params, device: int = 0, rank: int = 0, world: int = 1, concurrency: int = 1):
        if not torch.cuda.is_available():
            raise RuntimeError("ResidentTracker needs a HIP device (torch.cuda.is_available() is False)")
        self.params = params
        self.rank, self.world = rank, world
        self.dev = torch.device("cuda", device)
        torch.cuda.set_device(self.dev)
        self.ctx = capi.Context(device)
        if concurrency > 1:
            self.ctx.set_concurrency(concurrency)
        self.main = torch.cuda.Stream(device=self.dev)
        self.side = torch.cuda.Stream(device=self.dev)
        self.ctx.set_stream(self.main.cuda_stream)
        self.cur_slot = 1
        self._pyr_ready = None
        self._trk_done = {1: None, 2: None}
        self._graphs = {}
        self._graph_failed = False
        self.mode_used = "serial"
        self._gather_done = None
        self._last_gather = None
        self.n = 0

    def close(self):
        self.ctx.close()

    def load_pair(self, img_ref: np.ndarray, img_cur: np.ndarray):
        self.img_ref = torch.from_numpy(np.ascontiguousarray(img_ref)).to(self.dev)
        self.img_cur = torch.from_numpy(np.ascontiguousarray(img_cur)).to(self.dev)
        h, w = img_ref.shape
        self.w, self.h = w, h
        L = self.params.pyramids
        self.ctx.frame_set_device(0, self.img_ref.data_ptr(), w, h, w, L)
        self.ctx.frame_set_device(1, self.img_cur.data_ptr(), w, h, w, L)
        self.ctx.frame_set_device(2, self.img_cur.data_ptr(), w, h, w, L)
        self.cur_slot, self._pyr_ready = 1, None
        self._drop_graph()
        self._settle()

    def set_current_image(self, img_cur: np.ndarray):
        with torch.cuda.stream(self.main):
            self.img_cur.copy_(torch.from_numpy(np.ascontiguousarray(img_cur)).to(self.dev, non_blocking=False))

    def _settle(self):
        torch.cuda.synchronize(self.dev)

    def _drop_graph(self):
        for ids in self._graphs.values():
            for gid in ids:
                self.ctx.graph_destroy(gid)
        self._graphs = {}
        if getattr(self, "_live", None) is not None:
            self.ctx.graph_destroy(self._live[1])
            self._live = None

    @property
    def _graph(self):
        return self._graphs.get("graph")

    def set_features(self, pt_ref, pt_init, affine, status_in):
        self.n = int(pt_ref.shape[0])
        lo, hi = distributed.shard_range(self.n, self.rank, self.world)
        self.lo, self.hi = lo, hi
        m = distributed.shard_size(self.n, self.world)

        def up(a, width):
            t = torch.zeros((max(m, 1), width) if width > 1 else (max(m, 1),), dtype=torch.from_numpy(a).dtype,
                            device=self.dev)
            if hi > lo:
                t[:hi - lo] = torch.from_numpy(np.ascontiguousarray(a[lo:hi])).to(self.dev)
            return t

        same_shape = getattr(self, "d_pt_ref", None) is not None and self.d_pt_ref.shape[0] == max(m, 1) \
            and getattr(self, "_n_alloc", None) == self.n
        if same_shape:
            with torch.cuda.stream(self.main):
                for dst, a, width in ((self.d_pt_ref, pt_ref, 2), (self.d_pt_init, pt_init, 2),
                                      (self.d_affine, affine, 4), (self.d_status, status_in, 1)):
                    if hi > lo:
                        dst[:hi - lo].copy_(torch.from_numpy(np.ascontiguousarray(a[lo:hi])).to(self.dev))
            self._settle()
            return
        self.d_pt_ref = up(pt_ref, 2)
        self.d_pt_init = up(pt_init, 2)
        self.d_affine = up(affine, 4)
        self.d_status = up(status_in, 1)
        self.out = distributed.alloc_device_outputs(m, self.dev)
        self._n_alloc = self.n
        self._drop_graph()
        self._settle()

    def rebuild_current_pyramid(self, slot: int = 1):
        self.ctx.frame_set_device(slot, self.img_cur.data_ptr(), self.w, self.h, self.w, self.params.pyramids)

    def track_shard(self, slot: int = 1):
        self.ctx.track_device(self.params, 0, slot, self.hi - self.lo, self.d_pt_ref, self.d_pt_init, self.d_affine,
                              self.d_status, self.out)

    def _prefetch_pyramid(self, slot: int):
        with torch.cuda.stream(self.side):
            if self._trk_done[slot] is not None:
                self.side.wait_event(self._trk_done[slot])
            self.ctx.set_stream(self.side.cuda_stream)
            self.rebuild_current_pyramid(slot)
            ev = torch.cuda.Event()
            ev.record(self.side)
        self.ctx.set_stream(self.main.cuda_stream)
        return ev

    def step(self, gather: bool = True, mode: str = "graph"):
        gather = gather and not mode.endswith("-nogather")
        mode = mode.replace("-nogather", "")
        graph = {"graph": True, "fork": "fork", "fused": "fused"}.get(mode, False)
        overlap = mode == "streams"
        if mode not in ("graph", "fork", "fused", "serial", "streams"):
            raise ValueError(mode)
        collective = gather and (self.world > 1 or distributed.FORCE_COLLECTIVE)
        if collective:
            return self._sharded_step(mode)
        with torch.cuda.stream(self.main):
            if graph and not self._graph_failed:
                try:
                    self._graph_step(fork=(graph == "fork"), fused=(graph == "fused"))
                except capi.PagkError as e:
                    import sys
                    print(f"pagk: hipGraph capture failed ({e}); step() falls back to direct launches", file=sys.stderr)
                    self._graph_failed = True
                    self._drop_graph()
                    self.ctx.set_stream(self.main.cuda_stream)
                    self.mode_used = "serial"
                    self.rebuild_current_pyramid(1)
                    self.track_shard(1)
                else:
                    self.mode_used = mode
            elif graph:
                self.mode_used = "serial"
                self.rebuild_current_pyramid(1)
                self.track_shard(1)
            elif not overlap:
                self.mode_used = "serial"
                self.rebuild_current_pyramid(1)
                self.track_shard(1)
            else:
                self.mode_used = "streams"
                if self._pyr_ready is None:
                    self._pyr_ready = self._prefetch_pyramid(self.cur_slot)
                self.main.wait_event(self._pyr_ready)
                slot = self.cur_slot
                self.track_shard(slot)
                done = torch.cuda.Event()
                done.record(self.main)
                self._trk_done[slot] = done
                self.cur_slot = 3 - slot
                self._pyr_ready = self._prefetch_pyramid(self.cur_slot)
        return {name: self.out[name][:self.hi - self.lo] for name, _, _ in distributed.FIELDS}

    def _sharded_step(self, mode: str):
        with torch.cuda.stream(self.main):
            self.rebuild_current_pyramid(1)
            if self._gather_done is not None:
                self.main.wait_event(self._gather_done)
            if mode in ("graph", "fused", "fork") and not self._graph_failed:
                if "track" not in self._graphs:
                    self.track_shard(1)
                    self.main.synchronize()
                    try:
                        self.ctx.graph_begin()
                        try:
                            self.track_shard(1)
                        finally:
                            self._graphs["track"] = (self.ctx.graph_end(),)
                    except capi.PagkError:
# ... 410 lines not shown
```

Measured before the change: 12.53 million features/s.

## Boost wave priority for features that needed many iterations on the previous call

Each feature's final iteration count is written to a persistent per-context device buffer. On the next launch, features whose stored count exceeds a threshold (default 14, scaled by pyramid depth) start in the high s_setprio tier, so long-running blocks are favoured early. The hint buffer is carried through handover compaction, cleared on new uploads, and exposed through get/set/reset APIs. The intent is to cut the tail latency caused by slow features being scheduled late. In exchange it adds per-feature global reads and writes and state that lives across calls.

```diff
diff --git a/include/pagk.h b/include/pagk.h
--- a/include/pagk.h
+++ b/include/pagk.h
@@ -116,6 +116,11 @@
 int pagk_last_handover(pagk_ctx *ctx);
 
 int pagk_priority_threshold(pagk_ctx *ctx);
+
+int pagk_prio_hint_threshold(pagk_ctx *ctx);
+int pagk_prio_hint_reset(pagk_ctx *ctx);
+int pagk_prio_hint_get(pagk_ctx *ctx, int32_t n, int32_t *hints);
+int pagk_prio_hint_set(pagk_ctx *ctx, int32_t n, const int32_t *hints);
 
 int pagk_set_concurrency(pagk_ctx *ctx, int32_t streams);
 
diff --git a/pixel_aware_gyro_aided_klt_feature_tracker_amd/capi.py b/pixel_aware_gyro_aided_klt_feature_tracker_amd/capi.py
--- a/pixel_aware_gyro_aided_klt_feature_tracker_amd/capi.py
+++ b/pixel_aware_gyro_aided_klt_feature_tracker_amd/capi.py
@@ -394,6 +394,15 @@
         lib.pagk_selftest_divide.argtypes = [vp, i32, vp, vp, vp, vp, vp, vp]
         lib.pagk_selftest_solve.restype = C.c_int
         lib.pagk_selftest_solve.argtypes = [vp, i32, vp, vp, C.c_uint32, vp, vp, vp, vp]
+    if hasattr(lib, "pagk_prio_hint_reset"):
+        lib.pagk_prio_hint_threshold.restype = C.c_int
+        lib.pagk_prio_hint_threshold.argtypes = [vp]
+        lib.pagk_prio_hint_reset.restype = C.c_int
+        lib.pagk_prio_hint_reset.argtypes = [vp]
+        lib.pagk_prio_hint_get.restype = C.c_int
+        lib.pagk_prio_hint_get.argtypes = [vp, i32, vp]
+        lib.pagk_prio_hint_set.restype = C.c_int
+        lib.pagk_prio_hint_set.argtypes = [vp, i32, vp]
     if hasattr(lib, "pagk_priority_threshold"):
         lib.pagk_priority_threshold.restype = C.c_int
         lib.pagk_priority_threshold.argtypes = [vp]
@@ -451,6 +460,7 @@
     "pagk_multi_allgather", "pagk_track_sharded", "pagk_selftest_divide", "pagk_selftest_solve",
     "pagk_selftest_repeat_sum", "pagk_check_launch", "pagk_track_device_batch", "pagk_frame_set_device_batch", "pagk_priority_threshold",
     "pagk_multi_comm_count", "pagk_has_variant",
+    "pagk_prio_hint_threshold", "pagk_prio_hint_reset", "pagk_prio_hint_get", "pagk_prio_hint_set",
     "pagk_fit_params_default", "pagk_geometry_fit_device", "pagk_geometry_fit", "pagk_geometry_validation_device",
     "pagk_geometry_validation_fit", "pagk_selftest_fit_samples",
     "pagk_pose_params_default", "pagk_pose_params_check", "pagk_pose_2d2d_device", "pagk_pose_from_matches_device",
@@ -1404,6 +1414,22 @@
             self._check(rc, "pagk_priority_threshold")
         return rc
 
+    def prio_hint_threshold(self) -> int:
+        return int(self.lib.pagk_prio_hint_threshold(self.h))
+
+    def prio_hint_reset(self):
+        if hasattr(self.lib, "pagk_prio_hint_reset"):
+            self._check(self.lib.pagk_prio_hint_reset(self.h), "pagk_prio_hint_reset")
+
+    def prio_hint_get(self, n: int) -> np.ndarray:
+        out = np.zeros(max(n, 0), np.int32)
+        self._check(self.lib.pagk_prio_hint_get(self.h, n, out.ctypes.data_as(C.c_void_p)), "pagk_prio_hint_get")
+        return out
+
+    def prio_hint_set(self, hints) -> None:
+        h = np.ascontiguousarray(hints, np.int32)
+        self._check(self.lib.pagk_prio_hint_set(self.h, int(h.shape[0]), h.ctypes.data_as(C.c_void_p)), "pagk_prio_hint_set")
+
     def last_variant(self) -> int:
         return int(self.lib.pagk_last_variant(self.h))
 
diff --git a/pixel_aware_gyro_aided_klt_feature_tracker_amd/csrc/pagk_device.h b/pixel_aware_gyro_aided_klt_feature_tracker_amd/csrc/pagk_device.h
--- a/pixel_aware_gyro_aided_klt_feature_tracker_amd/csrc/pagk_device.h
+++ b/pixel_aware_gyro_aided_klt_feature_tracker_amd/csrc/pagk_device.h
@@ -73,6 +73,9 @@
     int prio_k;
     unsigned long long *prio_stats;
     const int *prio_kbuf;
+    const int *prio_hint_in;
+    int *prio_hint_out;
+    int prio_hint_t;
     int has_gyro, illum, use_affine, penalty, calc_ncc;
     uint32_t solver;
     float lam_invlog;
diff --git a/pixel_aware_gyro_aided_klt_feature_tracker_amd/csrc/pagk_handover_kernel.h b/pixel_aware_gyro_aided_klt_feature_tracker_amd/csrc/pagk_handover_kernel.h
--- a/pixel_aware_gyro_aided_klt_feature_tracker_amd/csrc/pagk_handover_kernel.h
+++ b/pixel_aware_gyro_aided_klt_feature_tracker_amd/csrc/pagk_handover_kernel.h
@@ -116,6 +116,8 @@
     int32_t *index_in_last;
     uint8_t *live, *mask;
     int32_t *state;
+    int32_t *prio_hint;
+    int32_t prio_hint_n;
 };
 
 __global__ void __launch_bounds__(256) k_handover_fill(uint8_t *mask, int64_t bytes)
@@ -181,6 +183,7 @@
     for (int c0 = 0; c0 < a.cap; c0 += 1024) {
         const int i = c0 + tid;
         const bool take = i < a.cap && a.status[i] != 0;
+        const int32_t hint = (take && i < a.prio_hint_n) ? a.prio_hint[i] : 0;
         int32_t tot;
         const int32_t o = m + handover_scan(take, wtot, lane, wave, tot);
         if (take) {
@@ -189,6 +192,7 @@
             a.keys_un[2 * o] = xu, a.keys_un[2 * o + 1] = yu;
             if (a.keys_normal) a.keys_normal[2 * o] = (xu - a.cx) * a.fx_inv, a.keys_normal[2 * o + 1] = (yu - a.cy) * a.fy_inv;
             a.index_in_last[o] = i;
+            if (o < a.prio_hint_n) a.prio_hint[o] = hint;
         }
         m += tot;
     }
@@ -229,6 +233,7 @@
     const int32_t added = topup ? (seen < n_new ? seen : n_new) : 0;
     const int32_t total = m + added;
     for (int i = tid; i < a.cap; i += 1024) {
+        if (i >= m && i < a.prio_hint_n) a.prio_hint[i] = 0;
         a.live[i] = i < total ? 1 : 0;
         if (i >= total) {
             a.keys[2 * i] = a.keys[2 * i + 1] = 0.0f;
diff --git a/pixel_aware_gyro_aided_klt_feature_tracker_amd/csrc/pagk_hip.hip b/pixel_aware_gyro_aided_klt_feature_tracker_amd/csrc/pagk_hip.hip
--- a/pixel_aware_gyro_aided_klt_feature_tracker_amd/csrc/pagk_hip.hip
+++ b/pixel_aware_gyro_aided_klt_feature_tracker_amd/csrc/pagk_hip.hip
@@ -16,6 +16,7 @@
 #include "pagk_pose_kernel.h"
 #include "pagk_layout.h"
 #include "pagk_select.h"
+#include "pagk_prio_env.h"
 
 using namespace pagk;
 
@@ -72,6 +73,7 @@
         QUAD_WS,
         SUSP,
         LV,
+        PRIO_HINT,
         kBufs
     };
     DevBuf buf[kBufs];
@@ -135,6 +137,7 @@
     int block5_min_features = 2500;
     int prio_k = 4;
     unsigned long long *prio_stats = nullptr;
+    int prio_hint_t = kPrioHintDefault;
     bool block5_window = true;
     int levels_min_features = 6000;
     int levels_shift = 0;
@@ -780,9 +783,32 @@
     return PAGK_OK;
 }
 
+int prio_hint_attach(pagk_ctx *ctx, int n, TrackArgs *a)
+{
+    DevBuf &hb = ctx->buf[pagk_ctx::PRIO_HINT];
+    const size_t need = (size_t)n * sizeof(int32_t);
+    if (need > hb.bytes) {
+        if (in_capture(ctx)) return PAGK_OK;
+        for (int k = 0; k < pagk_ctx::kGraphs; k++)
+            if (ctx->graph_execs[k]) return PAGK_OK;
+        if (int rc = reserve(ctx, hb, need, NOT_IN_CAPTURE_NOR_UNDER_GRAPH, "the priority hints", kLargestLaunchFirst)) return rc;
+        HIPCHK(ctx, hipMemsetAsync(hb.ptr, 0, hb.bytes, ctx->stream));
+    }
+    a->prio_hint_in = a->prio_hint_out = static_cast<int *>(hb.ptr);
+    return PAGK_OK;
+}
+
+int prio_hint_clear(pagk_ctx *ctx)
+{
+    DevBuf &hb = ctx->buf[pagk_ctx::PRIO_HINT];
+    if (hb.ptr) HIPCHK(ctx, hipMemsetAsync(hb.ptr, 0, hb.bytes, ctx->stream));
+    return PAGK_OK;
+}
+
 int launch_track(pagk_ctx *ctx, const pagk_params *p, const FrameSlot &sr, const FrameSlot &sc, int n,
                  const float *d_pt_ref, const float *d_pt_init, const float *d_affine, const uint8_t *d_status,
-                 const pagk_outputs *o, const PyrArgs *pyr = nullptr, int pyr_blocks = 0, bool *pyr_done = nullptr)
+                 const pagk_outputs *o, const PyrArgs *pyr = nullptr, int pyr_blocks = 0, bool *pyr_done = nullptr,
+                 bool hinted = true)
 {
     if (pyr_done) *pyr_done = false;
     TrackArgs a;
@@ -813,6 +839,7 @@
     a.prio_stats = ctx->prio_stats;
     a.prio_kbuf = ctx->prio_stats ? reinterpret_cast<const int *>(ctx->prio_stats + 2) : nullptr;
     a.lv_error = ctx->lv_error_dev;
+    a.prio_hint_t = n > ctx->cus ? (int)(((long long)ctx->prio_hint_t * p->pyramids + 2) / 3) : 0;
 
     if (ctx->ev_trk[0] && !in_capture(ctx)) HIPCHK(ctx, hipEventRecord(ctx->ev_trk[0], ctx->stream));
     if (n > 0) {
@@ -830,7 +857,10 @@
             case 5:
             case 7: rc = launch_quad(ctx, p, k, lean, variant == 7, n, a); break;
             case 6: rc = launch_rows(ctx, k, n, a); break;
-            default: rc = launch_block(ctx, k, lean, n, a, pyr, pyr_blocks, pyr_done); break;
+            default:
+                if (hinted && (rc = prio_hint_attach(ctx, n, &a))) break;
+                rc = launch_block(ctx, k, lean, n, a, pyr, pyr_blocks, pyr_done);
+                break;
         }
         if (rc) return rc;
         HIPCHK(ctx, e);
@@ -904,6 +934,7 @@
         memcpy(hb + offs[3], status_in, nn);
         HIPCHK(ctx, hipMemcpyAsync(db, hb, fp.in_bytes, hipMemcpyHostToDevice, ctx->stream));
     }
+    if ((rc = prio_hint_clear(ctx))) return rc;
     pagk_outputs dout = fp.out;
     if (!out->pt_dist) dout.pt_dist = nullptr;
     if (!out->pix_err) dout.pix_err = nullptr;
@@ -911,7 +942,7 @@
     if (!out->ncc) dout.ncc = nullptr;
     if (!out->iters) dout.iters = nullptr;
     rc = launch_track(ctx, p, sr, sc, n, fp.pt_ref, pt_init ? fp.pt_init : nullptr, affine ? fp.affine : nullptr,
-                      fp.status_in, &dout);
+                      fp.status_in, &dout, nullptr, 0, nullptr, false);
     if (rc) return rc;
     if (n > 0)
         HIPCHK(ctx, hipMemcpyAsync(hb + fp.in_bytes, db + fp.in_bytes, fp.lay.total - fp.in_bytes, hipMemcpyDeviceToHost,
@@ -1040,6 +1071,7 @@
     } else if (getenv("PAGK_PRIO_K")) {
         ctx->prio_k = atoi(getenv("PAGK_PRIO_K")) < 0 ? 0 : atoi(getenv("PAGK_PRIO_K"));
     }
+    if (getenv("PAGK_PRIO_HINT")) ctx->prio_hint_t = prio_hint_parse(getenv("PAGK_PRIO_HINT"), ctx->prio_hint_t);
     if (getenv("PAGK_LEVELS_XCD_SHIFT")) ctx->levels_shift = atoi(getenv("PAGK_LEVELS_XCD_SHIFT")) & 7;
     if (getenv("PAGK_LEVELS_SHARED")) ctx->levels_shared = atoi(getenv("PAGK_LEVELS_SHARED")) != 0;
     if (getenv("PAGK_QUAD_BUDGET")) ctx->quad_budget = atoi(getenv("PAGK_QUAD_BUDGET"));
@@ -1148,6 +1180,41 @@
     HIPCHK(ctx, hipStreamSynchronize(ctx->stream));
     if (int lr = lv_check(ctx)) return lr;
     return k;
+}
+
+int pagk_prio_hint_threshold(pagk_ctx *ctx) { return ctx ? ctx->prio_hint_t : PAGK_E_ARG; }
+
+int pagk_prio_hint_reset(pagk_ctx *ctx)
+{
+    if (!ctx) return PAGK_E_ARG;
+    HIPCHK(ctx, hipSetDevice(ctx->device));
+    return prio_hint_clear(ctx);
+}
+
+int pagk_prio_hint_get(pagk_ctx *ctx, int32_t n, int32_t *hints)
+{
+    if (!ctx || n < 0 || (n > 0 && !hints)) return PAGK_E_ARG;
+    NOT_WHILE_CAPTURING(ctx, "pagk_prio_hint_get");
+    HIPCHK(ctx, hipSetDevice(ctx->device));
+    const DevBuf &hb = ctx->buf[pagk_ctx::PRIO_HINT];
+    const size_t have = hb.bytes / sizeof(int32_t) < (size_t)n ? hb.bytes / sizeof(int32_t) : (size_t)n;
+    memset(hints, 0, (size_t)n * sizeof(int32_t));
+    if (have) HIPCHK(ctx, hipMemcpyAsync(hints, hb.ptr, have * sizeof(int32_t), hipMemcpyDeviceToHost, ctx->stream));
+    HIPCHK(ctx, hipStreamSynchronize(ctx->stream));
+    return PAGK_OK;
+}
+
+int pagk_prio_hint_set(pagk_ctx *ctx, int32_t n, const int32_t *hints)
+{
+    if (!ctx || n < 0 || (n > 0 && !hints)) return PAGK_E_ARG;
+    NOT_WHILE_CAPTURING(ctx, "pagk_prio_hint_set");
+    HIPCHK(ctx, hipSetDevice(ctx->device));
+    DevBuf &hb = ctx->buf[pagk_ctx::PRIO_HINT];
+    if (int rc = reserve(ctx, hb, (size_t)n * sizeof(int32_t), NOT_IN_CAPTURE_NOR_UNDER_GRAPH, "the priority hints", kLargestLaunchFirst)) return rc;
+    if (int rc = prio_hint_clear(ctx)) return rc;
+    if (n) HIPCHK(ctx, hipMemcpyAsync(hb.ptr, hints, (size_t)n * sizeof(int32_t), hipMemcpyHostToDevice, ctx->stream));
+    HIPCHK(ctx, hipStreamSynchronize(ctx->stream));
+    return PAGK_OK;
 }
 
 int pagk_check_launch(pagk_ctx *ctx)
@@ -1914,6 +1981,13 @@
            cap >= target_n && cand_cap >= 0 && !std::isnan(new_point_threshold);
 }
 
+void handover_hint_args(pagk_ctx *ctx, HandoverArgs *a)
+{
+    const DevBuf &hb = ctx->buf[pagk_ctx::PRIO_HINT];
+    a->prio_hint = static_cast<int32_t *>(hb.ptr);
+    a->prio_hint_n = (int32_t)(hb.bytes / sizeof(int32_t));
+}
+
 void handover_fill_args(HandoverArgs *out, const pagk_params *params, int32_t width, int32_t height, int32_t cap,
                         int32_t target_n, double new_point_threshold)
 {
@@ -2115,6 +2189,7 @@
     a.n_cand = d_n_cand, a.cand_un = d_cand_un;
     a.keys = d_keys, a.keys_un = d_keys_un, a.keys_normal = d_keys_normal;
     a.index_in_last = d_index_in_last, a.live = d_live, a.mask = mask, a.state = d_state;
+    handover_hint_args(ctx, &a);
     hipLaunchKernelGGL(k_handover_fill, dim3((unsigned)((bytes + 4095) / 4096)), dim3(256), 0, ctx->stream, mask, bytes);
     HIPCHK(ctx, hipGetLastError());
     hipLaunchKernelGGL(k_handover_holes, dim3((unsigned)(((int64_t)cap * 14 + 255) / 256)), dim3(256), 0, ctx->stream, cap,
@@ -2357,6 +2432,7 @@
     a.n_cand = d_info, a.cand_un = ws.cand;
     a.keys = d_keys, a.keys_un = d_keys_un, a.keys_normal = d_keys_normal;
     a.index_in_last = d_index_in_last, a.live = d_live, a.mask = mask, a.state = d_state;
+    handover_hint_args(ctx, &a);
     hipLaunchKernelGGL(k_handover_fill, dim3((unsigned)((bytes + 4095) / 4096)), dim3(256), 0, ctx->stream, mask, bytes);
     HIPCHK(ctx, hipGetLastError());
     hipLaunchKernelGGL(k_handover_holes, dim3((unsigned)(((int64_t)cap * 14 + 255) / 256)), dim3(256), 0, ctx->stream, cap,
diff --git a/pixel_aware_gyro_aided_klt_feature_tracker_amd/csrc/pagk_kernels.h b/pixel_aware_gyro_aided_klt_feature_tracker_amd/csrc/pagk_kernels.h
--- a/pixel_aware_gyro_aided_klt_feature_tracker_amd/csrc/pagk_kernels.h
+++ b/pixel_aware_gyro_aided_klt_feature_tracker_amd/csrc/pagk_kernels.h
@@ -489,8 +489,12 @@
 
     const float *init = a.has_gyro ? a.pt_init : a.pt_ref;
     float p2x = init[2 * i], p2y = init[2 * i + 1];
+    [[maybe_unused]] const bool hinted = !MFMA && !RELAXED && PIPE && !resume;
     if (!a.status_in[i]) {
-        if (tid == 0) write_outputs(a, i, p2x, p2y, 0, 0.0f, 0, 0.0f, 0);
+        if (tid == 0) {
+            write_outputs(a, i, p2x, p2y, 0, 0.0f, 0, 0.0f, 0);
+            if (hinted) prio_hint_store(a, i, 0);
+        }
         return;
     }
     float A00 = 1, A01 = 0, A10 = 0, A11 = 1;
@@ -563,7 +567,7 @@
 
     int succ = 1, iters = 0;
     [[maybe_unused]] constexpr bool kPrioByWork = NR > 1;
-    PAGK_PRIO_DECL
+    PAGK_PRIO_DECL(hinted)
     float lastCost = 0.0f;
 #ifdef PAGK_STAMPS
     unsigned long long st[14] = {0, 0, 0, 0, 0, 0, 0, 0, 0, 0, 0, 0, 0, 0};
@@ -976,6 +980,7 @@
         ncc = (float)((double)sh_f[2] / sqrt((double)(sh_f[3] * sh_f[4]) + 1e-10));
     }
     if (tid == 0) write_outputs(a, i, p2x, p2y, succ, lastCost, 1, ncc, iters);
+    if (tid == 0 && hinted) prio_hint_store(a, i, iters);
     if (tid == 0 && kPrioByWork && !resume) prio_account(a, i, iters, a.n_levels);
 #ifdef PAGK_STAMPS
     if (tid == 0 && a.dbg) {
diff --git a/pixel_aware_gyro_aided_klt_feature_tracker_amd/csrc/pagk_multi.h b/pixel_aware_gyro_aided_klt_feature_tracker_amd/csrc/pagk_multi.h
--- a/pixel_aware_gyro_aided_klt_feature_tracker_amd/csrc/pagk_multi.h
+++ b/pixel_aware_gyro_aided_klt_feature_tracker_amd/csrc/pagk_multi.h
@@ -349,9 +349,15 @@
         o.dist_pred = reinterpret_cast<double *>(sl + off[4]);
         o.ncc = reinterpret_cast<float *>(sl + off[5]);
         o.iters = reinterpret_cast<int32_t *>(sl + off[6]);
+        if ((rc = prio_hint_clear(c))) {
+            snprintf(pm->err, sizeof pm->err, "rank %d: %s", k, c->err);
+            drain(k);
+            return rc;
+        }
         rc = launch_track(c, params, c->slots[4], c->slots[5], nk, reinterpret_cast<float *>(db + in_off[0]),
                           pt_init_un ? reinterpret_cast<float *>(db + in_off[1]) : nullptr,
-                          affine ? reinterpret_cast<float *>(db + in_off[2]) : nullptr, db + in_off[3], &o);
+                          affine ? reinterpret_cast<float *>(db + in_off[2]) : nullptr, db + in_off[3], &o, nullptr, 0, nullptr,
+                          false);
         if (rc) {
             snprintf(pm->err, sizeof pm->err, "rank %d: %s", k, c->err);
             drain(k);
diff --git a/pixel_aware_gyro_aided_klt_feature_tracker_amd/csrc/pagk_pipe_kernel.h b/pixel_aware_gyro_aided_klt_feature_tracker_amd/csrc/pagk_pipe_kernel.h
--- a/pixel_aware_gyro_aided_klt_feature_tracker_amd/csrc/pagk_pipe_kernel.h
+++ b/pixel_aware_gyro_aided_klt_feature_tracker_amd/csrc/pagk_pipe_kernel.h
@@ -33,7 +33,10 @@
     const float *init = a.has_gyro ? a.pt_init : a.pt_ref;
     float p2x = init[2 * i], p2y = init[2 * i + 1];
     if (!a.status_in[i]) {
-        if (tid == 0) write_outputs(a, i, p2x, p2y, 0, 0.0f, 0, 0.0f, 0);
+        if (tid == 0) {
+            write_outputs(a, i, p2x, p2y, 0, 0.0f, 0, 0.0f, 0);
+            if (!resume) prio_hint_store(a, i, 0);
+        }
         return;
     }
     float A00 = 1, A01 = 0, A10 = 0, A11 = 1;
@@ -76,7 +79,7 @@
 
     int succ = 1, iters = 0, seq = 0;
     [[maybe_unused]] constexpr bool kPrioByWork = true;
-    PAGK_PRIO_DECL
+    PAGK_PRIO_DECL(!resume)
     float lastCost = 0.0f;
 #ifdef PAGK_STAMPS
     unsigned long long st[14] = {0, 0, 0, 0, 0, 0, 0, 0, 0, 0, 0, 0, 0, 0};
@@ -439,6 +442,7 @@
         ncc = (float)((double)sh_f[2] / sqrt((double)(sh_f[3] * sh_f[4]) + 1e-10));
     }
     if (tid == 0) write_outputs(a, i, p2x, p2y, succ, lastCost, 1, ncc, iters);
+    if (tid == 0 && !resume) prio_hint_store(a, i, iters);
     if (tid == 0 && kPrioByWork && !resume) prio_account(a, i, iters, a.n_levels);
 #ifdef PAGK_STAMPS
     if (lane == 0 && a.dbg) {
diff --git a/pixel_aware_gyro_aided_klt_feature_tracker_amd/csrc/pagk_prio.h b/pixel_aware_gyro_aided_klt_feature_tracker_amd/csrc/pagk_prio.h
--- a/pixel_aware_gyro_aided_klt_feature_tracker_amd/csrc/pagk_prio.h
+++ b/pixel_aware_gyro_aided_klt_feature_tracker_amd/csrc/pagk_prio.h
@@ -21,9 +21,15 @@
         }
     }
 }
+
+constexpr int kPrioBoost = 1 << 20;
+__device__ __forceinline__ void prio_hint_store(const TrackArgs &a, int i, int iters)
+{
+    if (a.prio_hint_out) a.prio_hint_out[i] = iters;
+}
 }
 #if PAGK_PRIO_MODE == 0
-#define PAGK_PRIO_DECL
+#define PAGK_PRIO_DECL(hinted)
 #define PAGK_PRIO_TIER
 #define PAGK_PRIO_RESET
 #define PRIO(n) __builtin_amdgcn_s_setprio(n);
@@ -32,14 +38,16 @@
 #define PAGK_PRIO_N_COST 1
 #define PAGK_PRIO_N_REST 0
 #else
-#define PAGK_PRIO_DECL   \
-    int tier_now = 0;    \
-    const int prio_kv = !kPrioByWork ? 0 : (a.prio_kbuf ? __builtin_amdgcn_readfirstlane(*a.prio_kbuf) : a.prio_k);
+#define PAGK_PRIO_DECL(hinted)                                                                                       \
+    int tier_now = 0;                                                                                                \
+    const int prio_kv = !kPrioByWork ? 0 : (a.prio_kbuf ? __builtin_amdgcn_readfirstlane(*a.prio_kbuf) : a.prio_k);  \
+    const int prio_boost = (kPrioByWork && (hinted) && a.prio_hint_t > 0 && a.prio_hint_in &&                        \
+                            __builtin_amdgcn_readfirstlane(a.prio_hint_in[i]) > a.prio_hint_t) ? kPrioBoost : 0;
 #define PAGK_STR2(x) #x
 #define PAGK_STR(x) PAGK_STR2(x)
 #define PAGK_PRIO_TIER                                                                                              \
     {                                                                                                               \
-        const int tier = (prio_kv > 0 && __builtin_amdgcn_readfirstlane(iters - prio_kv * (a.n_levels - level)) > 0) ? 3 : 0; \
+        const int tier = (prio_kv > 0 && __builtin_amdgcn_readfirstlane(iters + prio_boost - prio_kv * (a.n_levels - level)) > 0) ? 3 : 0; \
         asm volatile("s_cmp_eq_u32 %0, %1\n\t"                                                                      \
                      "s_cbranch_scc1 2f\n\t"                                                                        \
                      "s_cmp_eq_u32 %1, 0\n\t"                                                                       \
diff --git a/pixel_aware_gyro_aided_klt_feature_tracker_amd/csrc/pagk_prio_env.h b/pixel_aware_gyro_aided_klt_feature_tracker_amd/csrc/pagk_prio_env.h
--- /dev/null
+++ b/pixel_aware_gyro_aided_klt_feature_tracker_amd/csrc/pagk_prio_env.h
@@ -0,0 +1,19 @@
+#pragma once
+
+namespace pagk {
+
+constexpr int kPrioHintDefault = 14;
+
+inline int prio_hint_parse(const char *text, int fallback)
+{
+    if (!text || !*text) return fallback;
+    long v = 0;
+    for (const char *c = text; *c; c++) {
+        if (*c < '0' || *c > '9') return fallback;
+        v = v * 10 + (*c - '0');
+        if (v > 1000000) return fallback;
+    }
+    return (int)v;
+}
+
+}
diff --git a/pixel_aware_gyro_aided_klt_feature_tracker_amd/runtime.py b/pixel_aware_gyro_aided_klt_feature_tracker_amd/runtime.py
--- a/pixel_aware_gyro_aided_klt_feature_tracker_amd/runtime.py
+++ b/pixel_aware_gyro_aided_klt_feature_tracker_amd/runtime.py
@@ -120,6 +120,7 @@
                                       (self.d_affine, affine, 4), (self.d_status, status_in, 1)):
                     if hi > lo:
                         dst[:hi - lo].copy_(torch.from_numpy(np.ascontiguousarray(a[lo:hi])).to(self.dev))
+                self.ctx.prio_hint_reset()
             self._settle()
             return
         self.d_pt_ref = up(pt_ref, 2)
@@ -129,6 +130,8 @@
         self.out = distributed.alloc_device_outputs(m, self.dev)
         self._n_alloc = self.n
         self._drop_graph()
+        with torch.cuda.stream(self.main):
+            self.ctx.prio_hint_reset()
         self._settle()
 
     def rebuild_current_pyramid(self, slot: int = 1):
```

After: 12.75 million features/s (median of 6 runs). 1.8% higher.
